# peterhpark/neuroclear

Hardware: AMD Instinct MI355X
Metric: voxels/sec (higher is better)
Workload: dtype f32

## Files before the change

include/nc_hip.h:

```cpp
#ifndef NC_HIP_H
#define NC_HIP_H

#include <stddef.h>
#include <stdint.h>

#ifdef __cplusplus
extern "C" {
#endif

#define NC_OK 0
#define NC_ERR_SHAPE (-1)
#define NC_ERR_WS (-2)
#define NC_ERR_HIP (-3)
#define NC_ERR_ARG (-4)

const char* nc_last_error(void);
int nc_version(void);
int nc_conv_fwd_path(int C, int K, int kd, int kh, int kw, int stride, int pad);
int nc_conv_wgrad_path(int C, int K, int kd, int kh, int kw, int stride, int pad);
void nc_prof_begin(double min_flop);
int nc_prof_end(int max, int* cls, double* flop, float* ms);
int nc_prof_end2(int max, int* cls, double* flop, float* ms, double* abytes);
void nc_set_force_direct(int on);
void nc_sconv_set_cfg(int cfg);
// ... 72 lines not shown

int nc_slice_fwd(const float* vol, float* out, int NC, int D, int H, int W, int axis, int index, void* stream);
int nc_slice_bwd(const float* dout, float* dvol, int NC, int D, int H, int W, int axis, int index, void* stream);
int nc_mip_fwd(const float* vol, float* out, int32_t* arg, int NC, int D, int H, int W, int axis, int start, int depth,
               void* stream);
int nc_mip_bwd(const float* dout, const int32_t* arg, float* dvol, int NC, int D, int H, int W, int axis,
               void* stream);

int nc_volume_slices(const float* src, float* dst, int N, int C, int D, int H, int W, int axis, int to_volume,
                     void* stream);

size_t nc_loss_ws_bytes(long n);
int nc_mse_const_fwd(const float* pred, long n, float target, float* out, void* ws, size_t ws_bytes, void* stream);
int nc_mse_const_bwd(const float* pred, long n, float target, const float* gscale, float* dpred, void* stream);
int nc_bce_logits_const_fwd(const float* pred, long n, float target, float* out, void* ws, size_t ws_bytes, void* stream);
int nc_bce_logits_const_bwd(const float* pred, long n, float target, const float* gscale, float* dpred, void* stream);
int nc_mean_fwd(const float* pred, long n, float* out, void* ws, size_t ws_bytes, void* stream);
int nc_mean_bwd(long n, const float* gscale, float* dpred, void* stream);
int nc_l1_fwd(const float* a, const float* b, long n, float* out, void* ws, size_t ws_bytes, void* stream);
int nc_l1_bwd(const float* a, const float* b, long n, const float* gscale, float* da, void* stream);

int nc_adam_step(float* p, const float* g, float* m, float* v, long n, float lr, float beta1, float beta2, float eps,
                 int step, void* stream);

int nc_dice_cut_cube(const void* vol, int is_u16, int L0, int L1, int L2, int roi, int overlap, int border, int index,
                     float* cube, void* stream);
int nc_rotate_crop(const void* vol, int is_u16, int D, int H, int W, int z0, int y0, int x0, int cz, int cy, int cx,
                   const double* inv_affine, float* out, void* stream);
int nc_assemble_scatter_add(const float* cube, float* acc, int P0, int P1, int P2, int roi, int overlap, int border,
                            int index, void* stream);
int nc_assemble_finalize(const float* acc, void* out, int out_is_u16, int P0, int P1, int P2, int L0, int L1, int L2,
                         int roi, int overlap, void* stream);
int nc_assemble_finalize_slab(const float* acc_slab, void* out, int out_is_u16, int P0, int P1, int P2, int L0, int L1, int L2, int roi,
                              int overlap, int z0, int nz, int za, void* stream);

int nc_assemble_merge(const float* acc, float* merged, int L0, int L1, int L2, int roi, int overlap, void* stream);
int nc_radix_hist(const float* x, long n, int pass, unsigned prefix, unsigned* hist4096, void* stream);
int nc_assemble_rescale_finalize(const float* merged, void* out, int out_is_u16, int L0, int L1, int L2, int roi,
                                 int overlap, float lo, float hi, float range, void* stream);

size_t nc_match_histograms_ws_bytes(long n);
int nc_match_histograms(const float* source, const float* tmpl, float* out, long n, void* ws, size_t ws_bytes,
                        void* stream);

int nc_spectral_norm_fwd(const float* w_orig, float* u, float* v, float* w_out, float* sigma, float* scratch_k, int K, int M,
                         int power_iteration, float eps, void* stream);
int nc_spectral_norm_bwd(const float* g, const float* w_sn, const float* u, const float* v, const float* sigma, float* dw_orig, int K,
                         int M, void* stream);

size_t nc_patchgan_param_floats(int n_layers, int ndf, int nd);
size_t nc_patchgan_saved_floats(int B, int D, int H, int W, int n_layers, int ndf, int nd);
size_t nc_patchgan_ws_bytes(int B, int D, int H, int W, int n_layers, int ndf, int nd);
int nc_patchgan_out_shape(int B, int D, int H, int W, int n_layers, int ndf, int nd, int* oD, int* oH, int* oW);
int nc_patchgan_fwd(const float* params, const float* x, float* y, float* saved, int B, int D, int H, int W,
                    int n_layers, int ndf, int nd, void* ws, size_t ws_bytes, void* stream);
int nc_patchgan_bwd(const float* params, const float* x, const float* saved, const float* dy, float* dx, float* dparams,
                    int B, int D, int H, int W, int n_layers, int ndf, int nd, void* ws, size_t ws_bytes, void* stream);
int nc_patchgan_fwd_part(const float* params, const float* x, float* y, float* saved, int Btot, int b0, int B, int D, int H,
                         int W, int n_layers, int ndf, int nd, void* ws, size_t ws_bytes, void* stream);
int nc_patchgan_bwd_part(const float* params, const float* x, const float* saved, const float* dy, float* dx, int Btot, int b0,
                         int B, int D, int H, int W, int n_layers, int ndf, int nd, void* ws, size_t ws_bytes, void* stream);
size_t nc_patchgan_gp_saved_floats(int B, int D, int H, int W, int n_layers, int ndf, int nd);
size_t nc_patchgan_gp_ws_bytes(int B, int D, int H, int W, int n_layers, int ndf, int nd);
int nc_patchgan_gp_fwd(const float* params, const float* x, float* g, float* pen, float* saved, int B, int D, int H, int W, int n_layers,
                       int ndf, int nd, float constant, float lambda_gp, void* ws, size_t ws_bytes, void* stream);
int nc_patchgan_gp_bwd(const float* params, const float* x, const float* saved, const float* g, const float* dpen, float* dparams, float* dx,
                       int B, int D, int H, int W, int n_layers, int ndf, int nd, float constant, float lambda_gp, void* ws, size_t ws_bytes,
                       void* stream);

size_t nc_unet_deconv_fwd_ws_bytes(int N, int S0, int S1, int S2);
int nc_unet_deconv_fwd(const float* params, const float* x, float* y, int N, int S0, int S1, int S2, void* ws,
                       size_t ws_bytes, void* stream);


size_t nc_unet_deconv_param_floats(void);
size_t nc_unet_deconv_saved_floats(int N, int S0, int S1, int S2);
size_t nc_unet_deconv_train_ws_bytes(int N, int S0, int S1, int S2);
int nc_unet_deconv_train_fwd(const float* params, const float* x, float* y, float* saved, int N, int S0, int S1, int S2,
                             void* ws, size_t ws_bytes, void* stream, unsigned* kept);
int nc_unet_deconv_bwd(const float* params, const float* x, const float* y, const float* saved, const float* dy, float* dx,
                       float* dparams, int N, int S0, int S1, int S2, void* ws, size_t ws_bytes, void* stream, unsigned kept);
void nc_set_unet_lean(int on);
int nc_get_unet_lean(void);
size_t nc_deep_linear_param_floats(void);
size_t nc_deep_linear_saved_floats(int N, int S0, int S1, int S2);
size_t nc_deep_linear_ws_bytes(int N, int S0, int S1, int S2);
int nc_deep_linear_fwd(const float* params, const float* x, float* y, float* saved , int N, int S0, int S1,
                       int S2, void* ws, size_t ws_bytes, void* stream, unsigned* kept );
void nc_set_dl_collapse(int on);
int nc_get_dl_collapse(void);
int nc_deep_linear_bwd(const float* params, const float* x, const float* saved, const float* dy, float* dx, float* dparams,
                       int N, int S0, int S1, int S2, void* ws, size_t ws_bytes, void* stream, unsigned kept);

int nc_conv_fwd_c8(const void* xh, const float* w, const float* bias, void* yh, int out_ctot, int out_c0, int N, int C, int D, int H,
                   int W, int K, int kd, int kh, int kw, int stride, int pad, int dtype, void* ws, size_t ws_bytes, void* stream);
int nc_conv_dgrad_c8(const void* dyh, const float* w, void* dxh, int N, int C, int D, int H, int W, int K, int kd, int kh, int kw,
                     int stride, int pad, int dtype, void* ws, size_t ws_bytes, void* stream);
size_t nc_conv_c1_c8_ws_bytes(int N, int D, int H, int W, int ks);
int nc_conv_c1_fwd_c8(const float* x, const float* w, const float* bias, void* yh, int out_ctot, int out_c0, int N, int D, int H, int W,
                      int ks, int dtype, void* ws, size_t ws_bytes, void* stream);
int nc_conv_c1_dgrad_c8(const void* dyh, const float* w, float* dx, int N, int D, int H, int W, int ks, void* ws, size_t ws_bytes,
                        void* stream);
size_t nc_conv_c1_wgrad_c8_ws_bytes(int N, int D, int H, int W, int ks);
int nc_conv_c1_wgrad_c8(const float* x, const void* dyh, float* dw, int N, int D, int H, int W, int ks, void* ws, size_t ws_bytes,
                        void* stream);
size_t nc_c8_instnorm_ws_bytes(int N, int C, long S);
int nc_c8_instnorm_stats(const void* xh, int N, int C, long S, float eps, float* mean, float* rstd, int dtype, void* ws,
                         size_t ws_bytes, void* stream);
int nc_c8_instnorm_act_fwd(const void* xh, const float* mean, const float* rstd, float slope, void* yh, int out_ctot, int out_c0,
                           int N, int C, long S, int dtype, void* stream);
int nc_c8_instnorm_act_bwd(const void* gh, int g_ctot, int g_c0, const void* xh, const float* mean, const float* rstd, float slope,
                           void* dxh, float* dbias , int N, int C, long S, int dtype, void* ws, size_t ws_bytes,
                           void* stream);
int nc_c8_maxpool2_fwd(const void* xh, int x_ctot, int x_c0, void* yh, int N, int C, int D, int H, int W, int dtype, void* stream);
int nc_c8_maxpool2_bwd_add(const void* dph, const void* xh, int x_ctot, int x_c0, const void* skiph, int s_ctot, int s_c0, void* dxh,
                           int N, int C, int D, int H, int W, int dtype, void* stream);
int nc_from_c8(const void* xh, int x_ctot, int x_c0, float* y, int N, int C, long S, int dtype, void* stream);
size_t nc_convT_c8_ws_bytes(int N, int C, int D, int H, int W, int K);
int nc_convT_k2s2_fwd_c8(const void* xh, const float* w, const float* bias, void* yh, int out_ctot, int out_c0, int N, int C, int D,
                         int H, int W, int K, int dtype, void* ws, size_t ws_bytes, void* stream);
int nc_convT_k2s2_dgrad_c8(const void* dyh, int dy_ctot, int dy_c0, const float* w, void* dxh, int N, int C, int D, int H, int W, int K,
                           void* ws, size_t ws_bytes, void* stream);
int nc_convT_k2s2_wgrad_c8(const void* xh, const void* dyh, int dy_ctot, int dy_c0, float* dw, float* dbias , int N,
                           int C, int D, int H, int W, int K, void* ws, size_t ws_bytes, void* stream);

int nc_unet_deconv_lp_supported(int N, int S0, int S1, int S2, int dtype);
size_t nc_unet_deconv_lp_saved_bytes(int N, int S0, int S1, int S2);
size_t nc_unet_deconv_lp_ws_bytes(int N, int S0, int S1, int S2);
int nc_unet_deconv_lp_fwd(const float* params, const float* x, float* y, void* saved, int N, int S0, int S1, int S2, int dtype,
                          void* ws, size_t ws_bytes, void* stream);
int nc_unet_deconv_lp_bwd(const float* params, const float* x, const float* y, const void* saved, const float* dy, float* dx,
                          float* dparams, int N, int S0, int S1, int S2, int dtype, void* ws, size_t ws_bytes, void* stream);
int nc_deep_linear_lp_supported(int N, int S0, int S1, int S2, int dtype);
size_t nc_deep_linear_lp_saved_bytes(int N, int S0, int S1, int S2);
size_t nc_deep_linear_lp_ws_bytes(int N, int S0, int S1, int S2);
int nc_deep_linear_lp_fwd(const float* params, const float* x, float* y, void* saved, int N, int S0, int S1, int S2, int dtype,
                          void* ws, size_t ws_bytes, void* stream, unsigned* kept);
int nc_deep_linear_lp_bwd(const float* params, const float* x, const void* saved, const float* dy, float* dx, float* dparams,
                          int N, int S0, int S1, int S2, int dtype, void* ws, size_t ws_bytes, void* stream, unsigned kept);

void nc_set_conv_split(int on);
int nc_get_conv_split(void);
void nc_set_split_terms(int terms);
int nc_get_split_terms(void);
void nc_set_p2d_terms(int mode);
int nc_get_p2d_terms(void);
void nc_set_h2_guard(int on);
int nc_get_h2_guard(void);
int nc_h2_guard_stats(unsigned long long* out4, int reset);
void nc_set_epi_stats(int on);
int nc_get_epi_stats(void);
void nc_set_s3x_w64(int on);
int nc_get_s3x_w64(void);
int nc_unet_deconv_fwd_terms(int S0, int S1, int S2);
void nc_set_c8x_mode(int mode);
int nc_get_c8x_mode(void);
int nc_conv_lp_uses_c8x(int what , int fp32_out, int N, int C, int D, int H, int W, int K, int ks);
void nc_set_s3_fusion(int on);
int nc_conv_split_supported(int what, int N, int C, int D, int H, int W, int K, int kd, int kh, int kw, int stride, int pad);
size_t nc_conv_split_ws_bytes(int N, int C, int D, int H, int W, int K, int ks);
size_t nc_s3_bytes(int N, int C, long S);
int nc_to_s3(const float* x, void* xs, int N, int C, long S, void* stream);
int nc_conv_fwd_split(const float* x, const void* xs, const float* w, const float* bias, float* y, int N, int C, int D, int H, int W,
                      int K, int ks , void* ws, size_t ws_bytes, void* stream);
int nc_conv_dgrad_split(const float* dy, const void* dys, const float* w, float* dx, int N, int C, int D, int H, int W, int K, int ks,
                        void* ws, size_t ws_bytes, void* stream);
// ... 30 lines not shown
```

neuroclear_amd/_lib.py:

```python
import ctypes
import os
import re

_HERE = os.path.dirname(os.path.abspath(__file__))
LIB_PATH = os.environ.get('NC_HIP_LIB') or os.path.join(_HERE, 'csrc', 'libnc_hip.so')
HEADER_PATH = os.path.join(os.path.dirname(_HERE), 'include', 'nc_hip.h')

_lib = None


class NcError(RuntimeError):
    pass


def header_symbols():
    src = open(HEADER_PATH).read()
    src = re.sub(r'/\*.*?\*/', '', src, flags=re.S)
    return sorted(set(re.findall(r'\b(nc_[a-zA-Z0-9_]+)\s*\(', src)))


def lib():
    global _lib
    if _lib is None:
        if not os.path.exists(LIB_PATH):
            raise NcError('libnc_hip.so is not built (%s): run `python -c "import __graft_entry__ as g; g.build()"` '
                          'or `make -C neuroclear_amd/csrc`; there is no CPU fallback' % LIB_PATH)
        L = ctypes.CDLL(LIB_PATH)
        for name in header_symbols():
            fn = getattr(L, name)
            if name.endswith('_bytes') or name.endswith('_floats'):
                fn.restype = ctypes.c_size_t
            elif name == 'nc_last_error':
                fn.restype = ctypes.c_char_p
            elif name in ('nc_set_force_direct', 'nc_prof_begin', 'nc_sconv_set_cfg', 'nc_sconv_set_tune', 'nc_set_conv_split', 'nc_set_s3_fusion', 'nc_set_c8x_mode', 'nc_set_split_terms', 'nc_set_h2_guard', 'nc_set_epi_stats', 'nc_set_dl_collapse', 'nc_set_p2d_terms', 'nc_set_s3x_w64', 'nc_set_unet_lean'):
                fn.restype = None
            else:
                fn.restype = ctypes.c_int
        _lib = L
    return _lib


def check(code, what=''):
    if code != 0:
        raise NcError('%s failed (%d): %s' % (what, code, lib().nc_last_error().decode()))


P = ctypes.c_void_p
I = ctypes.c_int
L_ = ctypes.c_long
F = ctypes.c_float
Z = ctypes.c_size_t
```

neuroclear_amd/csrc/api.hip:

```cpp
#include <cstdlib>
#include <cstring>
#include <vector>

#include <atomic>
#include <mutex>
#include <set>
#include <utility>

#include "common.hpp"

namespace nc {

static thread_local char g_err[512] = "";
int g_force_direct = 0;

void set_error(const char* fmt, ...) {
  va_list ap;
  va_start(ap, fmt);
  vsnprintf(g_err, sizeof(g_err), fmt, ap);
  va_end(ap);
}

int raise_dyn_lds(const void* kernel, int bytes, const char* who) {
  static std::mutex mu;
// ... 303 lines not shown
int nc_conv_dgrad_lp(const float* dy, const void* dyh, const float* w, float* dx, int N, int C, int D, int H, int W, int K,
                     int kd, int kh, int kw, int stride, int pad, int dtype, void* ws, size_t ws_bytes, void* stream) {
  ConvDims d;
  if (int e = lp_args("conv_dgrad_lp", d, dy, dyh, w, dx, N, C, D, H, W, K, kd, kh, kw, stride, pad, dtype)) return e;
  if (!h_dgrad_supported(d)) { set_error("conv_dgrad_lp: shape not covered by the 16-bit kernels"); return NC_ERR_SHAPE; }
  ProfScope ps(1, 1, d, 1, (hipStream_t)stream);
  return conv_dgrad_h(dy, dyh, w, dx, d, dtype, ws, ws_bytes, (hipStream_t)stream);
}

int nc_conv_wgrad_lp(const float* x, const void* xh, const float* dy, const void* dyh, float* dw, float* dbias, int N, int C,
                     int D, int H, int W, int K, int kd, int kh, int kw, int stride, int pad, int dtype, void* ws,
                     size_t ws_bytes, void* stream) {
  ConvDims d;
  if (int e = lp_args("conv_wgrad_lp", d, x, xh, dw, dw, N, C, D, H, W, K, kd, kh, kw, stride, pad, dtype)) return e;
  if (!dy && !dyh) { set_error("conv_wgrad_lp: null pointer"); return NC_ERR_ARG; }
  if (dbias && !dy) { set_error("conv_wgrad_lp: the bias gradient needs the fp32 dy"); return NC_ERR_ARG; }
  if (!h_wgrad_supported(d)) { set_error("conv_wgrad_lp: shape not covered by the 16-bit kernels"); return NC_ERR_SHAPE; }
  hipStream_t s = (hipStream_t)stream;
  {
    ProfScope ps(2, 1, d, 1, s);
    if (int e = conv_wgrad_h(x, xh, dy, dyh, dw, d, dtype, ws, ws_bytes, s)) return e;
  }
  if (dbias) return bias_grad(dy, dbias, d.N, d.K, (long)d.Do * d.Ho * d.Wo, ws, ws_bytes, s);
  return NC_OK;
}

int nc_conv_wgrad(const float* x, const float* dy, float* dw, float* dbias, int N, int C, int D, int H, int W, int K,
                  int kd, int kh, int kw, int stride, int pad, void* ws, size_t ws_bytes, void* stream) {
  ConvDims d;
  if (int e = conv_args("conv_wgrad", d, x, dy, dw, N, C, D, H, W, K, kd, kh, kw, stride, pad)) return e;
  hipStream_t s = (hipStream_t)stream;
  int e;
  {
  const int path = wgrad_path(d);
  ProfScope ps(2, path, d, 0, s);
  if (path == 9) e = conv_wgrad_s3(x, nullptr, dy, nullptr, dw, d, ws, ws_bytes, s);
  else if (path == 10) e = conv_wgrad_p2d(x, dy, dw, d, ws, ws_bytes, s);
  else if (!g_force_direct && mfma_wgrad_supported(d)) e = conv_wgrad_mfma(x, dy, dw, d, ws, ws_bytes, s);
  else if (!g_force_direct && wgrad_1x1_supported(d)) e = conv_wgrad_1x1(x, dy, dw, d, ws, ws_bytes, s);
  else if (!g_force_direct && c1_wgrad_supported(d)) e = conv_wgrad_c1(x, dy, dw, d, ws, ws_bytes, s);
  else if (!g_force_direct && k1_wgrad_supported(d)) e = conv_wgrad_k1(x, dy, dw, d, s);
  else if (!g_force_direct && wgrad_path(d) == 8) {
    e = conv_wgrad_pg1(x, dy, nullptr, 1.f, dw, dbias, d, ws, ws_bytes, s);
    dbias = nullptr;
  }
  else if (!g_force_direct && sconv_wgrad_on(d)) e = conv_wgrad_sconv(x, dy, dw, d, ws, ws_bytes, s);
  else if (!g_force_direct && gemm_wgrad_supported(d)) e = conv_wgrad_gemm(x, dy, dw, d, ws, ws_bytes, s);
  else e = conv_wgrad_direct(x, dy, dw, d, s);
  }
  if (e) return e;
  if (dbias) return bias_grad(dy, dbias, d.N, d.K, (long)d.Do * d.Ho * d.Wo, ws, ws_bytes, s);
  return NC_OK;
}

int nc_conv_bwd(const float* x, const float* dy, const float* w, float* dx, float* dw, float* dbias, int N, int C, int D, int H, int W,
                int K, int kd, int kh, int kw, int stride, int pad, void* ws, size_t ws_bytes, void* stream) {
  ConvDims d;
  if (int e = conv_args("conv_bwd", d, x, dy, dw, N, C, D, H, W, K, kd, kh, kw, stride, pad)) return e;
  if (!w) { set_error("conv_bwd: null pointer"); return NC_ERR_ARG; }
  hipStream_t s = (hipStream_t)stream;
  SwitchScope switches_;
  if (dx && dgrad_path(d) == 9 && wgrad_path(d) == 9 && ws && s3_bwd_ws_bytes(d) && ws_bytes >= s3_bwd_ws_bytes(d)) {
    {
      ProfScope ps(1, 9, d, 0, s);
      if (int e = conv_bwd_s3(x, dy, w, dx, dw, d, ws, ws_bytes, s, 0)) return e;
      if (int e = conv_bwd_s3(x, dy, w, dx, dw, d, ws, ws_bytes, s, 1)) return e;
    }
    {
      ProfScope ps(2, 9, d, 0, s);
      if (int e = conv_bwd_s3(x, dy, w, dx, dw, d, ws, ws_bytes, s, 2)) return e;
    }
    if (dbias) return bias_grad(dy, dbias, d.N, d.K, (long)d.Do * d.Ho * d.Wo, ws, ws_bytes, s);
    return NC_OK;
  }
  if (dx)
    if (int e = nc_conv_dgrad(dy, w, dx, N, C, D, H, W, K, kd, kh, kw, stride, pad, ws, ws_bytes, stream)) return e;
  return nc_conv_wgrad(x, dy, dw, dbias, N, C, D, H, W, K, kd, kh, kw, stride, pad, ws, ws_bytes, stream);
}

}

namespace nc {
int conv_fwd_keep(const float* x, const float* w, const float* bias, float* y, int N, int C, int D, int H, int W, int K, int ks,
                  void* ws, size_t ws_bytes, void* stream, void* xs_keep, bool* kept) {
  ConvDims d;
  *kept = false;
  if (xs_keep && make_dims(d, N, C, D, H, W, K, ks, ks, ks, 1, ks / 2) && fwd_path(d) == 9 && wgrad_path(d) == 9) {
    if (!x || !w || !y) { set_error("conv_fwd: null pointer"); return NC_ERR_ARG; }
    ProfScope ps(0, 9, d, 0, (hipStream_t)stream);
    *kept = true;
    return conv_fwd_s3(x, nullptr, w, bias, y, d, ws, ws_bytes, (hipStream_t)stream, xs_keep);
  }
  return nc_conv_fwd(x, w, bias, y, N, C, D, H, W, K, ks, ks, ks, 1, ks / 2, ws, ws_bytes, stream);
}

bool conv_keep_supported(int N, int C, int D, int H, int W, int K, int ks) {
  ConvDims d;
  return make_dims(d, N, C, D, H, W, K, ks, ks, ks, 1, ks / 2) && fwd_path(d) == 9 && wgrad_path(d) == 9;
}

int conv_fwd_pre(const void* xs, const float* w, const float* bias, float* y, int N, int C, int D, int H, int W, int K, int ks, void* ws,
                 size_t ws_bytes, void* stream, float* stats_part) {
  ConvDims d;
  if (!xs || !w || !y) { set_error("conv_fwd_pre: null pointer"); return NC_ERR_ARG; }
  if (!make_dims(d, N, C, D, H, W, K, ks, ks, ks, 1, ks / 2) || fwd_path(d) != 9) { set_error("conv_fwd_pre: layer not on the split-operand kernels"); return NC_ERR_SHAPE; }
  ProfScope ps(0, 9, d, 0, (hipStream_t)stream);
  if (stats_part && !(conv_layer_h2(d) && ks == 3)) { set_error("conv_fwd_pre: epilogue statistics exist for the two-term 3^3 layers only"); return NC_ERR_ARG; }
  return conv_fwd_s3(nullptr, xs, w, bias, y, d, ws, ws_bytes, (hipStream_t)stream, nullptr, stats_part);
}

bool conv_bwd_pre_supported(int N, int C, int D, int H, int W, int K, int ks, bool want_dx, size_t ws_bytes) {
  ConvDims d;
  return make_dims(d, N, C, D, H, W, K, ks, ks, ks, 1, ks / 2) && wgrad_path(d) == 9 && s3_bwd_ws_bytes(d) && ws_bytes >= s3_bwd_ws_bytes(d) &&
         (!want_dx || dgrad_path(d) == 9);
}
int conv_bwd_pre(const float* x, const void* xs, const float* w, float* dx, float* dw, int N, int C, int D, int H, int W, int K, int ks,
                 void* ws, size_t ws_bytes, void* stream, bool dy_guarded) {
  ConvDims d;
  hipStream_t s = (hipStream_t)stream;
  if (!conv_bwd_pre_supported(N, C, D, H, W, K, ks, dx != nullptr, ws_bytes) || !make_dims(d, N, C, D, H, W, K, ks, ks, ks, 1, ks / 2)) {
    set_error("conv_bwd_pre: layer not on the split-operand kernels");
    return NC_ERR_SHAPE;
  }
  if ((!x && !xs) || !w || !dw || !ws) { set_error("conv_bwd_pre: null pointer"); return NC_ERR_ARG; }
  if (dx) {
    ProfScope ps(1, 9, d, 0, s);
    if (int e = conv_bwd_s3(x, nullptr, w, dx, dw, d, ws, ws_bytes, s, 1, nullptr, dy_guarded)) return e;
  }
  ProfScope ps(2, 9, d, 0, s);
  return conv_bwd_s3(x, nullptr, w, dx, dw, d, ws, ws_bytes, s, 2, xs, dy_guarded);
}

int conv_bwd_keep(const float* x, const void* xs, const float* dy, const float* w, float* dx, float* dw, int N, int C, int D, int H,
                  int W, int K, int ks, void* ws, size_t ws_bytes, void* stream) {
  ConvDims d;
  hipStream_t s = (hipStream_t)stream;
  if (xs && make_dims(d, N, C, D, H, W, K, ks, ks, ks, 1, ks / 2) && wgrad_path(d) == 9 && ws && s3_bwd_ws_bytes(d) &&
      ws_bytes >= s3_bwd_ws_bytes(d) &&
      (!dx || dgrad_path(d) == 9)) {
    if (!x || !dy || !w || !dw) { set_error("conv_bwd: null pointer"); return NC_ERR_ARG; }
    {
      ProfScope ps(1, 9, d, 0, s);
      if (int e = conv_bwd_s3(x, dy, w, dx, dw, d, ws, ws_bytes, s, 0)) return e;
      if (dx)
        if (int e = conv_bwd_s3(x, dy, w, dx, dw, d, ws, ws_bytes, s, 1)) return e;
    }
    ProfScope ps(2, 9, d, 0, s);
    return conv_bwd_s3(x, dy, w, dx, dw, d, ws, ws_bytes, s, 2, xs);
  }
  return nc_conv_bwd(x, dy, w, dx, dw, nullptr, N, C, D, H, W, K, ks, ks, ks, 1, ks / 2, ws, ws_bytes, stream);
}
}

extern "C" {

namespace {
struct UnetOff {
  size_t w[14], b[14];
  size_t total;
};
UnetOff unet_offsets() {
  struct L { int id; size_t wn, bn; };
  const L order[14] = {{0, 64 * 1 * 27, 64},       {1, 64 * 64 * 27, 64},     {2, 128 * 64 * 27, 128},
                       {3, 128 * 128 * 27, 128},   {4, 256 * 128 * 27, 256},  {5, 256 * 256 * 27, 256},
                       {6, 256 * 256 * 27, 256},   {10, 256 * 128 * 8, 128},  {7, 128 * 256 * 27, 128},
                       {8, 128 * 128 * 27, 128},   {11, 128 * 64 * 8, 64},    {9, 64 * 128 * 27, 64},
                       {12, 64, 1},                {13, 1, 1}};
  UnetOff o{};
  size_t off = 0;
  for (const L& l : order) {
    o.w[l.id] = off; off += l.wn;
    o.b[l.id] = off; off += l.bn;
  }
  o.total = off;
  return o;
}
struct UnetWs {
  size_t raw, cat1, a1, p1, cat2, a2, a2b, p2, b1, b2, t1, t2, mean, rstd, in_ws, conv_ws, total;
  size_t s_a1, s_cat1, s_a2, s_cat2, s_b1, s_b2;
  size_t cells;
  size_t stats;
  size_t in_ws_bytes, conv_ws_bytes;
};
UnetWs unet_ws(int S0, int S1, int S2, int NB = 1) {
  const size_t S1v = (size_t)S0 * S1 * S2;
  const size_t S = S1v * NB, Sh = S / 8, Sq = S / 64;
  UnetWs u{};
  size_t off = 0;
  auto take = [&](size_t n) { size_t r = off; off += (n + 63) & ~(size_t)63; return r; };
  u.raw = take(64 * S); u.cat1 = take(128 * S); u.a1 = take(64 * S); u.p1 = take(64 * Sh); u.cat2 = take(256 * Sh);
  u.a2 = take(128 * Sh); u.a2b = take(128 * Sh); u.p2 = take(128 * Sq); u.b1 = take(256 * Sq); u.b2 = take(256 * Sq);
  u.t1 = take(S); u.t2 = take(S); u.mean = take(256 * (size_t)NB); u.rstd = take(256 * (size_t)NB);
  u.in_ws_bytes = nc_instnorm_ws_bytes(256, (long)S1v);
  u.in_ws = take(u.in_ws_bytes / 4);
  size_t cw = 0;
  auto upd = [&](int C, int D, int H, int W, int K) {
    size_t b = nc_conv_ws_bytes(1, C, D, H, W, K, 3, 3, 3, 1, 1);
    if (b > cw) cw = b;
  };
  upd(64, S0, S1, S2, 64); upd(128, S0, S1, S2, 64);
  upd(64, S0 / 2, S1 / 2, S2 / 2, 128); upd(128, S0 / 2, S1 / 2, S2 / 2, 128); upd(256, S0 / 2, S1 / 2, S2 / 2, 128);
  upd(128, S0 / 4, S1 / 4, S2 / 4, 256); upd(256, S0 / 4, S1 / 4, S2 / 4, 256);
  u.conv_ws_bytes = cw;
  u.conv_ws = take(cw / 4 + 64);
  auto take3 = [&](size_t elems) { return take((elems * 6 + 3) / 4); };
  u.s_a1 = take3(64 * S); u.s_cat1 = take3(128 * S); u.s_a2 = take3(128 * Sh); u.s_cat2 = take3(256 * Sh);
  u.s_b1 = take3(256 * Sq); u.s_b2 = take3(256 * Sq);
  u.cells = take(64);
  {
    size_t sb = 0;
// ... 260 lines not shown
```

neuroclear_amd/csrc/common.hpp:

```cpp
#pragma once
#include <hip/hip_runtime.h>

#include <cstdarg>
#include <cstdio>

#include "../../include/nc_hip.h"

namespace nc {

void set_error(const char* fmt, ...);

inline int check_launch(const char* what) {
  hipError_t e = hipGetLastError();
  if (e != hipSuccess) {
    set_error("%s: %s", what, hipGetErrorString(e));
    return NC_ERR_HIP;
  }
  return NC_OK;
}

inline long cdiv(long a, long b) { return (a + b - 1) / b; }

int raise_dyn_lds(const void* kernel, int bytes, const char* who);
template <typename K>
// ... 71 lines not shown
bool gemm_fwd_supported(const ConvDims& d);
bool gemm_dgrad_supported(const ConvDims& d);
bool gemm_wgrad_supported(const ConvDims& d);
size_t gemm_ws_bytes(const ConvDims& d);
int conv_fwd_gemm(const float* x, const float* w, const float* b, float* y, const ConvDims& d, void* ws, size_t wsb,
                  hipStream_t s);
int conv_dgrad_gemm(const float* dy, const float* w, float* dx, const ConvDims& d, void* ws, size_t wsb,
                    hipStream_t s);
int conv_wgrad_gemm(const float* x, const float* dy, float* dw, const ConvDims& d, void* ws, size_t wsb,
                    hipStream_t s);

bool sconv_fwd_supported(const ConvDims& d);
bool sconv_dgrad_supported(const ConvDims& d);
size_t sconv_ws_bytes(const ConvDims& d);
void p2d_set_terms(int m);
int p2d_get_terms();
bool p2d_fwd_supported(const ConvDims& d);
bool p2d_dgrad_supported(const ConvDims& d);
size_t p2d_ws_bytes(const ConvDims& d);
int conv_fwd_p2d(const float* x, const float* w, const float* bias, float* y, const ConvDims& d, void* ws, size_t wsb, hipStream_t s);
int conv_dgrad_p2d(const float* dy, const float* w, float* dx, const ConvDims& d, void* ws, size_t wsb, hipStream_t s);
bool p2d_wgrad_supported(const ConvDims& d);
size_t p2d_wgrad_ws_bytes(const ConvDims& d);
int conv_wgrad_p2d(const float* x, const float* dy, float* dw, const ConvDims& d, void* ws, size_t wsb, hipStream_t s);
int conv_fwd_sconv(const float* x, const float* w, const float* bias, float* y, const ConvDims& d, void* ws, size_t wsb, hipStream_t s);
int conv_dgrad_sconv(const float* dy, const float* w, float* dx, const ConvDims& d, void* ws, size_t wsb, hipStream_t s);
void sconv_set_cfg(int cfg);
void sconv_set_tune(int on);
bool sconv_wgrad_supported(const ConvDims& d);
size_t sconv_wgrad_ws_bytes(const ConvDims& d);
int conv_wgrad_sconv(const float* x, const float* dy, float* dw, const ConvDims& d, void* ws, size_t wsb, hipStream_t s);

bool pg1_supported(const ConvDims& d);
size_t pg1_ws_bytes(const ConvDims& d);
int conv_fwd_pg1(const float* x, const float* w, const float* bias, float* y, const ConvDims& d, float slope, hipStream_t s);
int conv_wgrad_pg1(const float* x, const float* g, const float* act, float slope, float* dw, float* db, const ConvDims& d,
                   void* ws, size_t wsb, hipStream_t s);
int conv_dgrad_pg1(const float* g, const float* act, float slope, const float* w, float* dx, const ConvDims& d, hipStream_t s);

bool wgrad_1x1_supported(const ConvDims& d);
size_t wgrad_1x1_ws_bytes(const ConvDims& d);
int conv_wgrad_1x1(const float* x, const float* dy, float* dw, const ConvDims& d, void* ws, size_t wsb, hipStream_t s);
bool flat_1x1_supported(const ConvDims& d);
int conv_fwd_1x1(const float* x, const float* w, const float* b, float* y, const ConvDims& d, void* ws, size_t wsb,
                 hipStream_t s);
int conv_dgrad_1x1(const float* dy, const float* w, float* dx, const ConvDims& d, void* ws, size_t wsb,
                   hipStream_t s);

size_t conv_fwd_to1_k3_ws_bytes(int N, int D, int H, int W);
int conv_fwd_to1_k3(const float* x, const float* w, float* y, int N, int C, int D, int H, int W, void* ws, size_t wsb, hipStream_t s);
bool to1_dgrad_supported(const ConvDims& d);
int conv_dgrad_to1(const float* dy, const float* w, float* dx, const ConvDims& d, hipStream_t s);
bool to1_mfma_supported(const ConvDims& d);
size_t to1_mfma_ws_bytes(const ConvDims& d);
int conv_dgrad_to1_mfma(const float* dy, const float* w, float* dx, const ConvDims& d, void* ws, size_t wsb,
                        hipStream_t s);
bool k1_fwd_supported(const ConvDims& d);
bool k1_wgrad_supported(const ConvDims& d);
int conv_fwd_k1(const float* x, const float* w, const float* b, float* y, const ConvDims& d, hipStream_t s);
int conv_wgrad_k1(const float* x, const float* dy, float* dw, const ConvDims& d, hipStream_t s);
bool c1_wgrad_supported(const ConvDims& d);
size_t c1_wgrad_ws_bytes(const ConvDims& d);
int conv_wgrad_c1(const float* x, const float* dy, float* dw, const ConvDims& d, void* ws, size_t wsb, hipStream_t s);

bool s3_fwd_supported(const ConvDims& d);
bool s3_dgrad_supported(const ConvDims& d);
size_t s3_ws_bytes(const ConvDims& d);
size_t s3_tensor_bytes(int N, int C, long S);
int split3_to(const float* x, void* xs, int N, int C, long S, hipStream_t s);
int split3_into(const float* x, long xstride, void* xs, int N, int C, long S, int ctot, int c0, hipStream_t s, const unsigned* guard = nullptr);
bool conv_layer_h2(const ConvDims& d);
struct ForceThreeTerm { ForceThreeTerm(); ~ForceThreeTerm(); };
struct NetworkScope { NetworkScope(); ~NetworkScope(); };
struct SwitchScope { SwitchScope(); ~SwitchScope(); };
struct ForceTwoTerm { ForceTwoTerm(); ~ForceTwoTerm(); int prev_terms, prev_depth; };
int frozen_terms();
int frozen_guard();
bool h2_guard_can_flip();
int operand_into(const ConvDims& d, const float* x, long xstride, void* xs, int N, int C, long S, int ctot, int c0, hipStream_t s);
int act_operand(const ConvDims& d, const float* x, const float* mean, const float* rstd, float slope, float* y, long ystride, void* ys, int N, int C,
                long S, int ctot, int c0, hipStream_t s);
int act_split3(const float* x, const float* mean, const float* rstd, float slope, float* y, long ystride, void* ys, int N, int C, long S,
               int ctot, int c0, hipStream_t s);
int conv_fwd_s3(const float* x, const void* xs, const float* w, const float* b, float* y, const ConvDims& d, void* ws, size_t wsb,
                hipStream_t s, void* xs_keep = nullptr, float* stats_part = nullptr);
bool epi_stats_on();
void epi_stats_set(int on);
int epi_stats_mode();
void s3x_w64_set(int on);
int s3x_w64_get();
int conv_dgrad_s3(const float* dy, const void* dys, const float* w, float* dx, const ConvDims& d, void* ws, size_t wsb, hipStream_t s);
size_t s3_bwd_ws_bytes(const ConvDims& d);
int conv_bwd_s3(const float* x, const float* dy, const float* w, float* dx, float* dw, const ConvDims& d, void* ws, size_t wsb,
                hipStream_t s, int phase, const void* xs = nullptr, bool dy_guarded = false);
int conv_fwd_keep(const float* x, const float* w, const float* bias, float* y, int N, int C, int D, int H, int W, int K, int ks,
                  void* ws, size_t ws_bytes, void* stream, void* xs_keep, bool* kept);
int conv_bwd_keep(const float* x, const void* xs, const float* dy, const float* w, float* dx, float* dw, int N, int C, int D, int H,
                  int W, int K, int ks, void* ws, size_t ws_bytes, void* stream);
bool s3x_supported(int N, int Cin, int D, int H, int W, int Kout, int KS);
size_t s3x_packed_bytes(int Cin, int Kout, int KS, int NT = 3);
void s3x_set_terms(int t);
int s3x_get_terms();
int conv_s3x_h2(const void* xs, const unsigned* cell_a, const unsigned* cell_b, int split_c, const float* w, const float* bias, float* y, int N,
                int Cin, int D, int H, int W, int Kout, int KS, long so, long si, int flip, unsigned* wcell, void* wp_ws, hipStream_t s,
                const unsigned* guard = nullptr, float* stats_part = nullptr);
size_t s3x_stats_bytes(int N, int D, int H, int W, int Kout, int KS);
int s3x_stats_finalize(const float* stats_part, const float* bias, int N, int D, int H, int W, int Kout, int KS, float eps, float* mean, float* rstd,
                       hipStream_t s);
bool c1k7_h2_supported(const ConvDims& d);
size_t c1k7_h2_ws_bytes(const ConvDims& d);
int conv_c1k7_h2(const float* x, const float* w, const float* bias, float* y, const ConvDims& d, void* ws, size_t wsb, hipStream_t s);
size_t c1k7_h2_dgrad_ws_bytes(const ConvDims& d);
bool dl_typed_supported(int N, int D, int H, int W);
size_t dl_typed_bytes(int N, int D, int H, int W);
const float* dl_typed_wp(const char* scratch, int N, int D, int H, int W);
float* dl_typed_dwsw(char* scratch, int N, int D, int H, int W);
int dl_typed_compose(const float* F, char* scratch, int N, int D, int H, int W, hipStream_t s);
int dl_typed_fwd_boundary(const float* act0, float* y, char* scratch, int N, int D, int H, int W, hipStream_t s);
int dl_typed_dgrad_boundary(const float* act0, const float* dy, float* g, char* scratch, int N, int D, int H, int W, hipStream_t s);
int dl_typed_p(const float* act0, const float* dy, float* Pq, char* scratch, int N, int D, int H, int W, hipStream_t s);
int conv_c1k7_h2_dgrad(const float* dy, const float* w, float* dx, const ConvDims& d, void* ws, size_t wsb, hipStream_t s);
inline size_t h2_cells_offset(size_t elems) { return (elems * 4 + 255) & ~(size_t)255; }
inline unsigned* h2_cells_of(const void* t, size_t elems) { return (unsigned*)((char*)const_cast<void*>(t) + h2_cells_offset(elems)); }
int instnorm_relu_tail_sigmoid(const float* x, const float* mean, const float* rstd, const float* w1, const float* b1, const float* w2,
                               const float* b2, float* y, int C, long S, hipStream_t s);
int instnorm_act_bwd_dbias_h2(const float* dy, const float* x, const float* mean, const float* rstd, float slope, void* dxs,
                              float* dbias, int N, int C, long S, void* ws, size_t ws_bytes, void* stream, unsigned* guard = nullptr);
int instnorm_act_bwd_dbias_h2_rank1(const float* dy1, const float* w1, const float* x, const float* mean, const float* rstd, float slope, void* dxs,
                                    float* dbias, int C, long S, void* ws, size_t ws_bytes, void* stream, unsigned* guard);
unsigned* conv_bwd_guard_words(void* ws, int N, int K, long S);
int maxpool2_h2(const void* in, void* out, int N, int C, int ctot, int D, int H, int W, hipStream_t s);
int h2_zero_cells(unsigned* cells, int n, hipStream_t s);
int h2_set_cell(unsigned* cell, float bound, hipStream_t s);
int h2_absmax(const float* x, long n, unsigned* cell, hipStream_t s, unsigned* cell2 = nullptr);
int split2h_into(const float* x, long xstride, void* xs, int N, int C, long S, int ctot, int c0, const unsigned* cell, hipStream_t s,
                 unsigned* guard = nullptr);
constexpr int kGuardLow = 0, kGuardAll = 1, kGuardFlag = 2;
constexpr unsigned kGuardDrop = 17u << 23;
constexpr unsigned long long kGuardShare = 64;
#if defined(__HIP_DEVICE_COMPILE__)
__device__ __forceinline__ bool guard_skip(const unsigned* guard, int want) {
  return guard && (int)(__builtin_nontemporal_load(guard + kGuardFlag) != 0) != want;
}
#else
__device__ bool guard_skip(const unsigned* guard, int want);
#endif
bool h2_guard_on();
int h2_guard_mode();
void h2_guard_set(int on);
int h2_guard_read(unsigned long long* out4, int reset);
int h2_guard_zero(unsigned* g, hipStream_t s, int nwords = 8);
int h2_guard_decide(unsigned* ga, unsigned* gb, unsigned* prior, unsigned* flag, bool can_flip, hipStream_t s, unsigned long long total_a = 0);
int h2_to_s3_if(const void* xh, void* xs, int N, int C, long S, const unsigned* cells, const unsigned* guard, hipStream_t s);
int act_split2h(const float* x, const float* mean, const float* rstd, float slope, float* y, long ystride, void* ys, int N, int C, long S, int ctot,
                int c0, float bound, unsigned* cell, unsigned* cell2, hipStream_t s);
int act_split2h_pool(const float* x, const float* mean, const float* rstd, float slope, void* ys, void* pooled, int N, int C, int D, int H, int W,
                     int ctot, int c0, float bound, unsigned* cell, hipStream_t s);
int conv_s3x(const void* xs, const float* w, const float* bias, float* y, int N, int Cin, int D, int H, int W, int Kout, int KS, long so,
             long si, int flip, void* wp_ws, hipStream_t s, const unsigned* guard = nullptr);
bool conv_keep_supported(int N, int C, int D, int H, int W, int K, int ks);
int conv_fwd_pre(const void* xs, const float* w, const float* bias, float* y, int N, int C, int D, int H, int W, int K, int ks, void* ws,
                 size_t ws_bytes, void* stream, float* stats_part = nullptr);
bool conv_bwd_pre_supported(int N, int C, int D, int H, int W, int K, int ks, bool want_dx, size_t ws_bytes);
int conv_bwd_pre(const float* x, const void* xs, const float* w, float* dx, float* dw, int N, int C, int D, int H, int W, int K, int ks,
                 void* ws, size_t ws_bytes, void* stream, bool dy_guarded = false);
bool instnorm_bwd_s3_supported(int N, int C, long S);
int instnorm_act_bwd_dbias_s3(const float* dy, const float* x, const float* mean, const float* rstd, float slope, void* dxs,
                              float* dbias, int N, int C, long S, void* ws, size_t ws_bytes, void* stream);
bool convT_fwd_s3_supported(int N, int C, int D, int H, int W, int K);
size_t c8x_packed_bytes(int Cin, int Kout, int KS);
void c8x_set_mode(int m);
int c8x_get_mode();
bool c8x_supported(int N, int Cin, int D, int H, int W, int Kout, int KS, bool fp32_out);
int conv_c8x(const void* xh, const float* w, const float* bias, float* y, void* yh, int ctot, int c0, int N, int Cin, int D, int H, int W,
             int Kout, int KS, long so, long si, int flip, int diffuse, int dt, void* wp_ws, hipStream_t s);
bool convT_s3x_supported(int N, int C, int D, int H, int W, int K);
size_t convT_s3x_ws_bytes(int C, int K);
int convT_fwd_s3x(const void* xs, const float* w, const float* bias, float* y, void* ys, int ctot, int c0, int N, int C, int D, int H, int W,
                  int K, void* ws, size_t wsb, hipStream_t s, const unsigned* h2cell = nullptr, const unsigned* xcell = nullptr);
int convT_h2_bound(const float* w, const float* bias, int C, int K, float in_bound, unsigned* cell, hipStream_t s);
int convT_fwd_split_h2(const float* x, const float* w, const float* bias, float* y, void* ys, int ys_ctot, int ys_c0, int N, int C, int D, int H,
                       int W, int K, const unsigned* out_cell, void* ws, size_t ws_bytes, hipStream_t s);
int convT_fwd_s3(const float* x, const float* w, const float* bias, float* y, void* ys, int ctot, int c0, int N, int C, int D, int H,
                 int W, int K, void* stream);
bool s3_wgrad_supported(const ConvDims& d);
bool c8x_wgrad_supported(const ConvDims& d);
size_t c8x_wgrad_part_bytes(const ConvDims& d);
int conv_wgrad_c8x(const void* xh, const void* dyh, float* dw, const ConvDims& d, int dtype, void* ws, size_t wsb, hipStream_t s);
size_t s3_wgrad_ws_bytes(const ConvDims& d);
int conv_wgrad_s3(const float* x, const void* xs, const float* dy, const void* dys, float* dw, const ConvDims& d, void* ws, size_t wsb,
                  hipStream_t s);
bool s3x_k32_supported(int N, int D, int H, int W);
bool conv_fwd_h2_k32_supported(const ConvDims& d);
int conv_fwd_h2_k32_keep(const float* x, const float* w, float* y, const ConvDims& d, void* ws, size_t wsb, hipStream_t s, void* xs_keep);
bool conv_fwd_h2_c32_supported(const ConvDims& d);
size_t conv_fwd_h2_c32_ws_bytes(const ConvDims& d);
int conv_fwd_h2_c32(const float* x, const float* w, float* y, const ConvDims& d, void* ws, size_t wsb, hipStream_t s);
bool wgrad_h2_supported(const ConvDims& d);
int conv_wgrad_h2(const float* x, const void* xs, const float* dy, const void* dys, float* dw, const ConvDims& d, void* ws, size_t wsb, hipStream_t s);
bool h_fwd_supported(const ConvDims& d);
bool h_dgrad_supported(const ConvDims& d);
bool h_wgrad_supported(const ConvDims& d);
size_t h_ws_bytes(const ConvDims& d);
int to_c8(const float* x, void* xh, int N, int C, long S, int dt, hipStream_t s);
int conv_fwd_h(const float* x, const void* xh, const float* w, const float* b, float* y, const ConvDims& d, int dt,
               void* ws, size_t wsb, hipStream_t s);
int conv_dgrad_h(const float* dy, const void* dyh, const float* w, float* dx, const ConvDims& d, int dt, void* ws,
                 size_t wsb, hipStream_t s);
int conv_wgrad_h(const float* x, const void* xh, const float* dy, const void* dyh, float* dw, const ConvDims& d, int dt,
                 void* ws, size_t wsb, hipStream_t s);
int conv_fwd_h_c8(const void* xh, const float* w, const float* b, void* yh, int ctot, int c0, const ConvDims& d, int dt,
                  void* ws, size_t wsb, hipStream_t s);
int conv_fwd_h_na1(const void* xh, const float* w, float* y, const ConvDims& d, int dt, void* ws, size_t wsb, hipStream_t s);
int conv_dgrad_h_c8(const void* dyh, const float* w, void* dxh, int ctot, int c0, const ConvDims& d, int dt, void* ws,
                    size_t wsb, hipStream_t s);
bool dl_collapse_on();
size_t dl_tail_bytes();
const float* dl_tail_E(const char* tail);
const float* dl_tail_Ef(const char* tail);
float* dl_tail_q(char* tail);
int dl_tail_compose(const float* w2, const float* w3, const float* w4, const float* w5, char* tail, hipStream_t s);
int dl_tail_grads(const float* w2, const float* w3, const float* w4, const float* w5, char* tail, float* dw2, float* dw3, float* dw4, float* dw5,
                  hipStream_t s);
float* dl_tail_P(char* tail);
const float* dl_w1_fold(char* tail, const float* w1, hipStream_t s);
int dl_w1_contract(const char* tail, float* dw1, hipStream_t s);
int dl_q_from_p(char* tail, const float* w1, hipStream_t s);
const float* dl_fold_fwd64(char* tail, const float* w1, hipStream_t s);
int dl_combine27(const float* Z, float* y, int N, int D, int H, int W, int zch, hipStream_t s);
bool c1_h_supported(int D, int H, int W, int KS);
size_t c1_h_ws_bytes(int N, int D, int H, int W, int KS);
int conv_c1_fwd_h(const float* x, const float* w, const float* bias, void* yh, int ctot, int c0, int N, int D, int H, int W, int KS,
                  int dt, void* ws, size_t wsb, hipStream_t s);
int conv_c1_dgrad_h(const void* dyh, const float* w, float* dx, int N, int D, int H, int W, int KS, void* ws, size_t wsb,
                    hipStream_t s);

void h_set_weight_diffusion(int on);

bool c1_wgrad_h_supported(int N, int D, int H, int W, int KS);
size_t c1_wgrad_h_ws_bytes(int N, int D, int H, int W, int KS);
int conv_c1_wgrad_h(const float* x, const void* dyh, float* dw, int N, int D, int H, int W, int KS, void* ws, size_t wsb,
                    hipStream_t s);

static constexpr size_t kPackSlackBytes = 128 * 1024;

extern int g_force_direct;

struct ProfScope {
// ... 8 lines not shown
```

neuroclear_amd/csrc/conv_s3x.hip:

```cpp
#include <atomic>
#include <cstdlib>
#include <type_traits>

#include "common.hpp"
#include "s3_common.hpp"

namespace nc {
namespace {

typedef float f32x4 __attribute__((ext_vector_type(4)));
typedef __bf16 bf16x8 __attribute__((ext_vector_type(8)));
typedef _Float16 f16x8 __attribute__((ext_vector_type(8)));
typedef unsigned u32x4 __attribute__((ext_vector_type(4)));
typedef unsigned long long u64x2 __attribute__((ext_vector_type(2)));
typedef const __attribute__((address_space(1))) void* gptr_t;
typedef __attribute__((address_space(3))) void* lptr_t;
typedef const volatile __attribute__((address_space(3))) unsigned long long* lds64_t;

constexpr int kWaves = 8;
constexpr int kThreads = kWaves * 64;
constexpr int kLdsMax = 160 * 1024;
#ifndef NC_S3X_DMAW
#define NC_S3X_DMAW 4
#endif
#ifndef NC_S3X_BDEPTH
#define NC_S3X_BDEPTH 1
#endif
constexpr int kDmaWaves = NC_S3X_DMAW;
constexpr int kMaxPieces = 56;

__device__ __forceinline__ unsigned fdiv(unsigned n, unsigned m) { return __umulhi(n, m); }
unsigned magic(unsigned d) { return (unsigned)(((1ull << 32) + d - 1) / d); }

__device__ __forceinline__ void split3(float v, unsigned short (&t)[3]) { s3_split(v, t); }

template <int NT>
__global__ void __launch_bounds__(256) k_pack_w_s3x(const float* __restrict__ w, unsigned short* __restrict__ wp, int NCH, int KS, int NS,
                                                    long so, long si, int flip, long total, const unsigned* __restrict__ amax, int split_c,
                                                    const unsigned* __restrict__ cell_a, const unsigned* __restrict__ cell_b) {
  const long i = (long)blockIdx.x * 256 + threadIdx.x;
  if (i >= total) return;
  const int T2 = KS * KS, T3 = T2 * KS, NB = NCH * KS;
  const int j = (int)(i & 7);
  long q = i >> 3;
  const int lane = (int)(q & 63); q >>= 6;
  const int f = (int)(q % (2 * NT)); q /= 2 * NT;
  const int s = (int)(q % NS); q /= NS;
  const int half = (int)(q & 1);
  const int cot = (int)(q >> 1);
  const int rb = f / NT, term = f % NT;
  const int g = lane >> 4, m = lane & 15;
  const int T = 4 * s + g;
  const int bi = T / T2, tp = T % T2;
  unsigned short t[3] = {0, 0, 0};
  if (bi < NB) {
    const int chunk = bi / KS, dz = bi % KS;
#ifdef NC_S3X_B128
    const int jj = j;
#else
    const int jj = (g & 1) ? ((j + 4) & 7) : j;
#endif
    const long co = cot * 64 + half * 32 + rb * 16 + m, ci = chunk * 8 + jj;
    const int tap = dz * T2 + tp;
    const float v = w[co * so + ci * si + (flip ? T3 - 1 - tap : tap)];
    if constexpr (NT == 3) split3(v, t);
    else h2_split(v * (ci >= split_c ? h2_group_factor(*cell_a, *cell_b) : 1.f) * h2_scale(*amax), t);
  }
  wp[i] = t[term];
}

__global__ void __launch_bounds__(256) k_absmax_w(const float* __restrict__ w, long n, int T3, int C, int split_c, const unsigned* __restrict__ cell_a,
                                                  const unsigned* __restrict__ cell_b, unsigned* __restrict__ out) {
  unsigned m = 0;
  const float gf = split_c < C ? h2_group_factor(*cell_a, *cell_b) : 1.f;
  for (long i = (long)blockIdx.x * 256 + threadIdx.x; i < n; i += (long)gridDim.x * 256) {
    const int ci = (int)((i / T3) % C);
    const unsigned b = __float_as_uint(w[i] * (ci >= split_c ? gf : 1.f)) & 0x7fffffffu;
    if (b < 0x7f800000u && b > m) m = b;
  }
#pragma unroll
  for (int o = 32; o > 0; o >>= 1) {
    const unsigned q = (unsigned)__shfl_xor((int)m, o);
    m = q > m ? q : m;
  }
  __shared__ unsigned wm[4];
  if ((threadIdx.x & 63) == 0) wm[threadIdx.x >> 6] = m;
  __syncthreads();
  if (threadIdx.x == 0) {
    unsigned b = wm[0];
    for (int k = 1; k < 4; ++k) b = wm[k] > b ? wm[k] : b;
    if (b) atomicMax(out, b);
  }
}

__global__ void __launch_bounds__(256) k_pack_w_c1k7(const float* __restrict__ w, unsigned short* __restrict__ wp, int NS, long total,
                                                     const unsigned* __restrict__ amax) {
  const long i = (long)blockIdx.x * 256 + threadIdx.x;
  if (i >= total) return;
  const int j = (int)(i & 7);
  long q = i >> 3;
  const int lane = (int)(q & 63); q >>= 6;
  const int f = (int)(q & 3); q >>= 2;
  const int s = (int)(q % NS); q /= NS;
  const int half = (int)(q & 1);
  const int rb = f >> 1, term = f & 1;
  const int g = lane >> 4, m = lane & 15;
  const int T = 4 * s + g;
  unsigned short t[3] = {0, 0, 0};
  const int jj = (g & 1) ? ((j + 4) & 7) : j;
  const int dz = T >> 3, dy = T & 7;
  if (dz < 7 && dy < 7 && jj < 7) {
    const int co = half * 32 + rb * 16 + m;
    h2_split(w[(long)co * 343 + (dz * 7 + dy) * 7 + jj] * h2_scale(*amax), t);
  }
  wp[i] = t[term];
}

__global__ void __launch_bounds__(256) k_build_x8_h2(const float* __restrict__ x, uint4* __restrict__ out, long S, int W, const unsigned* __restrict__ cell,
                                                     unsigned* __restrict__ guard) {
  const unsigned cb_bits = *cell;
  const float sc = h2_scale(cb_bits);
  const int n = blockIdx.y;
  unsigned n_all = 0, n_low = 0;
  for (long v0 = (long)blockIdx.x * 256; v0 < S; v0 += (long)gridDim.x * 256) {
    const long v = v0 + threadIdx.x;
    unsigned m = 0;
    if (v < S) {
      const int xx = (int)(v % W);
      const float* row = x + (long)n * S + (v - xx);
      unsigned short e[8][3];
#pragma unroll
      for (int j = 0; j < 8; ++j) {
        const int xs = xx + j - 3;
        const float f = (j < 7 && (unsigned)xs < (unsigned)W) ? row[xs] : 0.f;
        if (j == 3) { const unsigned b = __float_as_uint(f) & 0x7fffffffu; if (b < 0x7f800000u) m = b; }
        h2_split(f * sc, e[j]);
      }
#pragma unroll
      for (int t = 0; t < 2; ++t) out[((long)n * 2 + t) * S + v] = s3_unit(e, t);
    }
    if (guard) {
      const unsigned thr = cb_bits > kGuardDrop ? cb_bits - kGuardDrop : 0u;
      const bool any_hi = __builtin_amdgcn_ballot_w64(m >= thr && m != 0) != 0;
      const bool any_nz = __builtin_amdgcn_ballot_w64(m != 0) != 0;
      if (any_nz) {
        ++n_all;
        if (!any_hi) ++n_low;
      }
    }
  }
  if (!guard) return;
  __shared__ unsigned cnt[2];
  if (threadIdx.x < 2) cnt[threadIdx.x] = 0;
  __syncthreads();
  if ((threadIdx.x & 63) == 0) {
    if (n_all) atomicAdd(&cnt[kGuardAll], n_all);
    if (n_low) atomicAdd(&cnt[kGuardLow], n_low);
  }
  __syncthreads();
  if (threadIdx.x < 2 && cnt[threadIdx.x]) atomicAdd(guard + threadIdx.x, cnt[threadIdx.x]);
}

__global__ void __launch_bounds__(256) k_pack_w_c1k7d(const float* __restrict__ w, unsigned short* __restrict__ wp, int NS, long total,
                                                      const unsigned* __restrict__ amax) {
  const long i = (long)blockIdx.x * 256 + threadIdx.x;
  if (i >= total) return;
  const int j = (int)(i & 7);
  long q = i >> 3;
  const int lane = (int)(q & 63); q >>= 6;
  const int f = (int)(q & 3); q >>= 2;
  const int s = (int)(q % NS); q /= NS;
  const int half = (int)(q & 1);
  const int rb = f >> 1, term = f & 1;
  const int g = lane >> 4, m = lane & 15;
  const int T = 4 * s + g;
// ... 918 lines not shown
__global__ void __launch_bounds__(256) k_s3x_stats_partial(const float2* __restrict__ part, XStatsPlan pl, double2* __restrict__ chunk_sums) {
  const int slice = blockIdx.x, n = blockIdx.y, ch = blockIdx.z;
  const int cot = slice >> 1, half = slice & 1;
  const int l = threadIdx.x & 31, grp = threadIdx.x >> 5;
  const long per_n = (long)pl.TPP * pl.D;
  double s = 0.0, q = 0.0;
  const long nrec = per_n * 4, per = (nrec + kStatChunks - 1) / kStatChunks;
  const long r1 = (ch + 1) * per < nrec ? (ch + 1) * per : nrec;
#pragma unroll 4
  for (long r = ch * per + grp; r < r1; r += 8) {
    const long u = r >> 2;
    const int pg = (int)(r & 3);
    const long t = ((long)n * per_n + u) * pl.KT + cot;
    if (t < pl.main_count) {
      const float2 v = part[((t * kWaves) + pg * 2 + half) * 32 + l];
      s += (double)v.x; q += (double)v.y;
    } else {
      const int full_g = (pl.TPP / kXGroup) * kXGroup * pl.D;
      int tp;
      if (u < full_g) { const long g4 = u / (kXGroup * pl.D), rem = u - g4 * (kXGroup * pl.D); tp = (int)(g4 * kXGroup + (rem % kXGroup)); }
      else { const int L = pl.TPP % kXGroup; const long v2 = u - full_g; tp = (pl.TPP / kXGroup) * kXGroup + (int)(v2 % L); }
      for (int sub = 0; sub < pl.fsub; ++sub) {
        if ((long)(tp * pl.fsub + sub) * pl.PTsub >= pl.HP) continue;
        const long ti = pl.main_count + (t - pl.full) * pl.fsub + sub;
        const float2 v = part[((ti * kWaves) + pg * 2 + half) * 32 + l];
        s += (double)v.x; q += (double)v.y;
      }
    }
  }
  __shared__ double rs[8][32], rq[8][32];
  rs[grp][l] = s; rq[grp][l] = q;
  __syncthreads();
  if (grp == 0) {
    for (int g = 1; g < 8; ++g) { s += rs[g][l]; q += rq[g][l]; }
    chunk_sums[(((long)n * gridDim.x + slice) * kStatChunks + ch) * 32 + l] = make_double2(s, q);
  }
}
__global__ void __launch_bounds__(256) k_s3x_stats_final(const double2* __restrict__ chunk_sums, int K, const float* __restrict__ bias, long S, float eps,
                                                         float* __restrict__ mean, float* __restrict__ rstd) {
  const int i = blockIdx.x * 256 + threadIdx.x, n = blockIdx.y;
  if (i >= K) return;
  const int slice = i >> 5, l = i & 31;
  double s = 0.0, q = 0.0;
  for (int ch = 0; ch < kStatChunks; ++ch) {
    const double2 v = chunk_sums[(((long)n * (K / 32) + slice) * kStatChunks + ch) * 32 + l];
    s += v.x; q += v.y;
  }
  const int g4 = l >> 3, m = l & 7;
  const int c = (slice >> 1) * 64 + (slice & 1) * 32 + 4 * g4 + 16 * (m >> 2) + (m & 3);
  const double m0 = s / (double)S;
  double var = q / (double)S - m0 * m0;
  if (var < 0.0) var = 0.0;
  mean[(long)n * K + c] = (float)(m0 + (bias ? (double)bias[c] : 0.0));
  rstd[(long)n * K + c] = (float)(1.0 / sqrt(var + (double)eps));
}

}

static std::atomic<int> g_epi_stats{getenv("NC_EPI_STATS") ? atoi(getenv("NC_EPI_STATS")) : 1};
bool epi_stats_on() { return g_epi_stats.load(std::memory_order_relaxed) != 0; }
int epi_stats_mode() { return g_epi_stats.load(std::memory_order_relaxed); }
void epi_stats_set(int on) { g_epi_stats.store(on < 0 ? 0 : on > 2 ? 2 : on, std::memory_order_relaxed); }

int s3x_ksteps(int Cin, int KS) { return (KS * KS * KS * (Cin / 8) / 4 + 1) & ~1; }
size_t s3x_packed_bytes(int Cin, int Kout, int KS, int NT) {
  const int NS = s3x_ksteps(Cin, KS);
  return (size_t)(Kout / 32) * NS * 2 * NT * 1024;
}

static std::atomic<int> g_terms{getenv("NC_SPLIT_TERMS") ? atoi(getenv("NC_SPLIT_TERMS")) : 2};
void s3x_set_terms(int t) { g_terms = (t == 0 || t == 3) ? t : 2; }
int s3x_get_terms() { const int f = frozen_terms(); return f >= 0 ? f : g_terms.load(); }

bool s3x_k32_supported(int N, int D, int H, int W) { return x_plan(N, D, H, W, 1, 5, 2, true).ok && (long)32 * D * H * W * 4 < (1l << 31); }
bool s3x_supported(int N, int Cin, int D, int H, int W, int Kout, int KS) {
  if (KS != 3 && KS != 5) return false;
  if (Cin % 64 || Kout % 64) return false;
  if ((long)Kout * D * H * W * 4 >= (1l << 31)) return false;
  if ((long)D * H * W * 48 >= (1l << 31)) return false;
  if ((long)H * (W + KS - 1) + 4096 >= (1l << 31)) return false;
  return x_plan(N, D, H, W, Kout / 64, KS).ok;
}

int conv_s3x_h2(const void* xs, const unsigned* cell_a, const unsigned* cell_b, int split_c, const float* w, const float* bias, float* y, int N,
                int Cin, int D, int H, int W, int Kout, int KS, long so, long si, int flip, unsigned* wcell, void* wp_ws, hipStream_t s,
                const unsigned* guard, float* stats_part) {
  const bool k32 = Kout == 32;
  if (k32 && (KS != 5 || stats_part || guard)) { set_error("conv_s3x_h2: 32 output channels for unguarded 5^3 launches only"); return NC_ERR_SHAPE; }
  const XPlan pl = x_plan(N, D, H, W, k32 ? 1 : Kout / 64, KS, 2, k32);
  if (!pl.ok) { set_error("conv_s3x_h2: shape not covered"); return NC_ERR_SHAPE; }
  if (split_c < Cin && (flip || !cell_b || split_c % 8)) { set_error("conv_s3x_h2: scale groups only for the forward weight layout"); return NC_ERR_ARG; }
  if (stats_part && KS != 3) { set_error("conv_s3x_h2: epilogue statistics exist for the 3^3 layers only (the layers in front of an InstanceNorm)"); return NC_ERR_ARG; }
  const int NCH = Cin / 8, NS = s3x_ksteps(Cin, KS), T3 = KS * KS * KS;
  if (Cin % 32) { set_error("conv_s3x_h2: channels must be a multiple of 32"); return NC_ERR_SHAPE; }
  if (int e = h2_zero_cells(wcell, 1, s)) return e;
  const long nw = (long)Kout * Cin * T3;
  if (!cell_b) cell_b = cell_a;
  hipLaunchKernelGGL(k_absmax_w, dim3((unsigned)(cdiv(nw, 256 * 8) < 256 ? cdiv(nw, 256 * 8) : 256)), dim3(256), 0, s, w, nw, T3, Cin,
                     flip ? Cin : split_c, cell_a, cell_b, wcell);
  const long total = (long)(s3x_packed_bytes(Cin, Kout, KS, 2) / 2);
  hipLaunchKernelGGL(k_pack_w_s3x<2>, dim3((unsigned)cdiv(total, 256)), dim3(256), 0, s, w, (unsigned short*)wp_ws, NCH, KS, NS, so, si, flip, total,
                     (const unsigned*)wcell, flip ? Cin : split_c, cell_a, cell_b);
  if (int e = check_launch("conv_s3x_h2 pack")) return e;
  XParams p{};
  p.xs = (const uint4*)xs; p.wp = (const uint4*)wp_ws; p.bias = bias; p.y = y; p.amax_x = cell_a; p.amax_w = wcell; p.guard = guard;
  p.N = N; p.NCH = NCH; p.D = D; p.H = H; p.W = W; p.K = Kout;
  p.P = pl.P; p.HP = pl.HP; p.TPP = pl.TPP; p.KT = k32 ? 1 : Kout / 64;
  p.NS = NS; p.mP = magic(pl.P);
  static const int flush = getenv("NC_S3X_FLUSH") ? atoi(getenv("NC_S3X_FLUSH")) : 4;
  p.flush = flush >= 4 ? flush : flush > 0 ? 4 : 1 << 30;
  if (KS == 3 && !k32 && s3x_w64_get()) p.flush = 1 << 30;
  const bool one = pl.rem && pl.fsub == 1;
  if (pl.full || one) {
    p.fsub = 1; p.UB = pl.UB; p.npb = pl.npb; p.mUB = magic(pl.UB);
    p.t_begin = 0; p.t_count = (int)(pl.full + (one ? pl.rem : 0)); p.tiles_per_xcd = (int)cdiv(p.t_count, 8);
    p.stats = (float2*)stats_part;
    const int e = !k32 && w64_applies(KS, pl.NCB, NS, pl.lds) ? (stats_part ? launch_w64<true>(p, pl.lds, s) : launch_w64<false>(p, pl.lds, s))
                  : k32 ? (pl.NCB == 4 ? launch_x<5, 4, 2, false, true>(p, pl.lds + kOffTab, s) : launch_x<5, 2, 2, false, true>(p, pl.lds + kOffTab, s))
                  : stats_part ? (KS == 3 ? launch_x_ncb<3, 2, true>(pl.NCB, p, pl.lds + kOffTab, s) : launch_x_ncb<5, 2>(pl.NCB, p, pl.lds + kOffTab, s))
                             : (KS == 3 ? launch_x_ncb<3, 2>(pl.NCB, p, pl.lds + kOffTab, s) : launch_x_ncb<5, 2>(pl.NCB, p, pl.lds + kOffTab, s));
    if (e) return e;
  }
  if (pl.rem && !one) {
    p.fsub = pl.fsub; p.UB = pl.UBt; p.npb = pl.npbt; p.mUB = magic(pl.UBt);
    p.t_begin = (int)pl.full; p.t_count = (int)(pl.rem * pl.fsub); p.tiles_per_xcd = (int)cdiv(p.t_count, 8);
    p.stats = stats_part ? (float2*)stats_part + pl.full * kWaves * 32 : nullptr;
    const int e = k32 ? (pl.NCB / pl.fsub == 4 ? launch_x<5, 4, 2, false, true>(p, pl.ldst + kOffTab, s) : launch_x<5, 2, 2, false, true>(p, pl.ldst + kOffTab, s))
                  : stats_part ? (KS == 3 ? launch_x_ncb<3, 2, true>(pl.NCB / pl.fsub, p, pl.ldst + kOffTab, s)
                                        : launch_x_ncb<5, 2>(pl.NCB / pl.fsub, p, pl.ldst + kOffTab, s))
                             : (KS == 3 ? launch_x_ncb<3, 2>(pl.NCB / pl.fsub, p, pl.ldst + kOffTab, s)
                                        : launch_x_ncb<5, 2>(pl.NCB / pl.fsub, p, pl.ldst + kOffTab, s));
    if (e) return e;
  }
  return NC_OK;
}

static size_t c1k7_al(size_t b) { return (b + 255) & ~(size_t)255; }
static constexpr int kC1k7Steps = 14;
static size_t c1k7_packed_bytes() { return (size_t)2 * kC1k7Steps * 4 * 1024; }
bool c1k7_h2_supported(const ConvDims& d) {
  static const int on = getenv("NC_C1K7_H2") ? atoi(getenv("NC_C1K7_H2")) : 1;
  if (!on || s3x_get_terms() != 2) return false;
  if (d.C != 1 || d.K != 64 || d.kd != 7 || d.kh != 7 || d.kw != 7 || d.sd != 1 || d.sh != 1 || d.sw != 1 || d.pd != 3 || d.ph != 3 || d.pw != 3) return false;
  const long S = (long)d.D * d.H * d.W;
  if (d.W < 4 || (long)64 * S * 4 >= (1l << 31) || S * 32 >= (1l << 31)) return false;
  return x_plan(d.N, d.D, d.H, d.W, 1, 7, 2, false, true).ok;
}
size_t c1k7_h2_ws_bytes(const ConvDims& d) {
  if (!c1k7_h2_supported(d)) return 0;
  return 512 + c1k7_al((size_t)d.N * d.D * d.H * d.W * 32) + c1k7_al(c1k7_packed_bytes());
}
template <int NCB>
static int launch_pc(const XParams& p, int lds, hipStream_t s) { return launch_x<7, NCB, 2, false, false, 1>(p, lds, s); }
static int launch_pc_ncb(int NCB, const XParams& p, int lds, hipStream_t s) {
  if (NCB == 8) return launch_pc<8>(p, lds, s);
  if (NCB == 7) return launch_pc<7>(p, lds, s);
  if (NCB == 6) return launch_pc<6>(p, lds, s);
  if (NCB == 4) return launch_pc<4>(p, lds, s);
  return launch_pc<2>(p, lds, s);
}
int conv_c1k7_h2(const float* x, const float* w, const float* bias, float* y, const ConvDims& d, void* ws, size_t wsb, hipStream_t s) {
  if (!c1k7_h2_supported(d)) { set_error("conv_c1k7_h2: shape not covered"); return NC_ERR_SHAPE; }
  if (!ws || wsb < c1k7_h2_ws_bytes(d)) { set_error("conv_c1k7_h2: workspace too small"); return NC_ERR_WS; }
  const XPlan pl = x_plan(d.N, d.D, d.H, d.W, 1, 7, 2, false, true);
  const long S = (long)d.D * d.H * d.W;
  unsigned* cells = (unsigned*)ws;
  unsigned* gw = (unsigned*)((char*)ws + 256);
  uint4* x8 = (uint4*)((char*)ws + 512);
  void* wp = (char*)x8 + c1k7_al((size_t)d.N * S * 32);
  if (int e = h2_zero_cells(cells, 2, s)) return e;
  if (int e = h2_absmax(x, (long)d.N * S, cells, s)) return e;
  if (int e = h2_absmax(w, (long)64 * 343, cells + 1, s)) return e;
  const bool guard = h2_guard_on();
  if (guard) if (int e = h2_guard_zero(gw, s, 4)) return e;
  {
    long bx = cdiv(S, 256);
    if (guard && bx * d.N > 4096) bx = cdiv(4096, d.N);
    hipLaunchKernelGGL(k_build_x8_h2, dim3((unsigned)bx, (unsigned)d.N), dim3(256), 0, s, x, x8, S, d.W, (const unsigned*)cells, guard ? gw : nullptr);
  }
  if (guard) if (int e = h2_guard_decide(gw, nullptr, nullptr, gw + kGuardFlag, false, s)) return e;
  const long total = (long)(c1k7_packed_bytes() / 2);
  hipLaunchKernelGGL(k_pack_w_c1k7, dim3((unsigned)cdiv(total, 256)), dim3(256), 0, s, w, (unsigned short*)wp, kC1k7Steps, total, (const unsigned*)(cells + 1));
  if (int e = check_launch("conv_c1k7_h2 prep")) return e;
  XParams p{};
  p.xs = x8; p.wp = (const uint4*)wp; p.bias = bias; p.y = y; p.amax_x = cells; p.amax_w = cells + 1; p.guard = nullptr;
  p.N = d.N; p.NCH = 1; p.D = d.D; p.H = d.H; p.W = d.W; p.K = 64;
// ... 138 lines not shown
```

neuroclear_amd/csrc/conv_split.hip:

```cpp
#include <cstdlib>
#include <type_traits>

#include "common.hpp"
#include "s3_common.hpp"

namespace nc {
NC_ZERO_PAGE()
namespace {

typedef float f32x16 __attribute__((ext_vector_type(16)));
typedef __bf16 bf16x8 __attribute__((ext_vector_type(8)));
typedef int i32x4 __attribute__((ext_vector_type(4)));
typedef const __attribute__((address_space(1))) void* gptr_t;
typedef __attribute__((address_space(3))) void* lptr_t;

constexpr int kWaves = 8;
constexpr int kThreads = kWaves * 64;
constexpr int kLdsMax = 160 * 1024;
#ifndef NC_S3_ABLATE
#define NC_S3_ABLATE 0
#endif
template <int KS> struct Sub;
template <> struct Sub<3> { static constexpr int NP = 5, NSUB = 1, MAXP = 5; static constexpr int q0[2] = {0, 5}; };
template <> struct Sub<5> { static constexpr int NP = 13, NSUB = 4, MAXP = 4; static constexpr int q0[5] = {0, 4, 7, 10, 13}; };
// ... 332 lines not shown
      for (int v = 0; v < VB; ++v) {
        const unsigned f = (unsigned)(cur.q0 + qb + v * 32);
        const unsigned yy = fdiv(f, p.mP);
        const unsigned xx = f - yy * p.P;
        yo[v] = ((int)yy < p.H && (int)xx < p.W) ? (long)yy * p.W + xx : -1;
      }
#pragma unroll
      for (int a = 0; a < 2; ++a) {
        float bv[16];
#pragma unroll
        for (int e = 0; e < 16; ++e) bv[e] = p.bias ? p.bias[cob + a * 32 + (e & 3) + 8 * (e >> 2) + 4 * h] : 0.f;
#pragma unroll
        for (int v = 0; v < VB; ++v)
          if (yo[v] >= 0) {
            float* yv = yn + yo[v];
#pragma unroll
            for (int e = 0; e < 16; ++e) yv[(long)(a * 32 + (e & 3) + 8 * (e >> 2)) * S] = acc[a][v][e] + bv[e];
          }
      }
    }
    if (!more_tiles) break;
    cur = nxt;
    tcur = tnext;
    lo = dz_lo(cur);
    nv = dz_hi(cur) - lo + 1;
  }
}

struct SPlan {
  int PT, VB, P, R, RP, TPP, npb, lds;
  bool ok;
};

SPlan s_plan(int H, int W, int KS) {
  SPlan pl{};
  pl.P = W + KS - 1;
  const long plane = (long)H * pl.P;
  const int wbytes = (KS == 3 ? Sub<3>::MAXP : Sub<5>::MAXP) * kPairPieces * 1024;
  double best = 0;
  for (int VB : {2, 1}) {
    const int PT = VB * 256;
    const int rows = (pl.P - 1 + PT - 1) / pl.P + 1;
    const int R = rows + KS - 1;
    const int RP = R * pl.P;
    const int npb = (3 * RP + 4 + 63) / 64;
    const int lds = 2 * npb * 1024 + 2 * wbytes;
    if (npb > 8 * 7 || lds > kLdsMax) continue;
    const int TPP = (int)((plane + PT - 1) / PT);
    const double eff = (double)H * W / ((double)TPP * PT) * (VB == 2 ? 1.0 : 0.85);
    if (eff > best) {
      best = eff;
      pl.PT = PT; pl.VB = VB; pl.R = R; pl.RP = RP; pl.npb = npb; pl.lds = lds; pl.TPP = TPP;
      pl.ok = true;
    }
  }
  return pl;
}

bool s_shape_ok(const ConvDims& d, int Cin, int Kout) {
  if (d.kd != d.kh || d.kd != d.kw || (d.kd != 3 && d.kd != 5)) return false;
  if (d.sd != 1 || d.sh != 1 || d.sw != 1 || d.pd != d.kd / 2 || d.ph != d.pd || d.pw != d.pd) return false;
  if (Cin % 8 || Kout % 64) return false;
  if ((long)d.D * d.H * d.W * 3 >= (1l << 31)) return false;
  return s_plan(d.H, d.W, d.kd).ok;
}

size_t s_packed_bytes(int Cin, int Kout, int KS) {
  return (size_t)(Kout / 64) * (Cin / 8) * KS * ((KS * KS + 1) / 2) * kPairPieces * 1024;
}
size_t align256(size_t b) { return (b + 255) & ~(size_t)255; }

template <int KS, int VB>
int launch_s3(const SParams& p, int lds, hipStream_t s) {
  auto kern = k_conv_s3<KS, VB>;
  if (int e = raise_dyn_lds(kern, kLdsMax, "conv_s3")) return e;
  hipLaunchKernelGGL(kern, dim3(256), dim3(kThreads), lds, s, p);
  return check_launch("conv_s3");
}

bool s3_layer_h2(const ConvDims& d);

int run_s3(const float* x, const void* xs_pre, const float* w, const float* bias, float* y, const ConvDims& d, int Cin, int Kout,
           long so, long si, int flip, void* ws, size_t wsb, hipStream_t s, void* xs_keep = nullptr, bool h2 = false, unsigned* guard_pre = nullptr,
           float* stats_part = nullptr) {
  const int KS = d.kd;
  const SPlan pl = s_plan(d.H, d.W, KS);
  const long S = (long)d.D * d.H * d.W;
  if (h2) {
    const size_t ex = (size_t)d.N * Cin * S;
    const bool internal = !xs_pre && !xs_keep;
    const size_t p2 = s3x_packed_bytes(Cin, Kout, KS, 2), p3 = s3x_packed_bytes(Cin, Kout, KS, 3);
    const size_t xb6 = align256(ex * 6), xb4 = h2_cells_offset(ex) + 256;
    bool dual = guard_pre || (internal && x && h2_guard_can_flip() && wsb >= xb6 + 256 + p3 + 256);
    if (guard_pre && wsb < 256 + p3 + 256) { set_error("conv_s3 (two-term, guarded operand): workspace too small"); return NC_ERR_WS; }
    const size_t xb = !internal ? 0 : dual ? xb6 : xb4;
    if (!ws || wsb < xb + 256 + p2 + 256) { set_error("conv_s3 (two-term): workspace too small"); return NC_ERR_WS; }
    void* xs = xs_pre ? const_cast<void*>(xs_pre) : xs_keep ? xs_keep : ws;
    unsigned* cells = h2_cells_of(xs, ex);
    unsigned* gw = (unsigned*)((char*)ws + xb);
    unsigned* guard = guard_pre ? guard_pre : gw;
    if (!xs_pre) {
      if (int e = h2_guard_zero(gw, s)) return e;
      if (int e = h2_zero_cells(cells, 2, s)) return e;
      if (int e = h2_absmax(x, (long)ex, cells, s, cells + 1)) return e;
      if (int e = split2h_into(x, (long)Cin * S, xs, d.N, Cin, S, Cin, 0, cells, s, gw)) return e;
      if (int e = h2_guard_decide(gw, nullptr, nullptr, gw + kGuardFlag, dual, s)) return e;
      if (dual)
        if (int e = split3_into(x, (long)Cin * S, xs, d.N, Cin, S, Cin, 0, s, gw)) return e;
    }
    if (stats_part && dual) { set_error("conv_s3 (two-term): epilogue statistics need an operand that cannot fall back"); return NC_ERR_ARG; }
    if (int e = conv_s3x_h2(xs, cells, cells + 1, flip ? Cin : Cin / 2, w, bias, y, d.N, Cin, d.D, d.H, d.W, Kout, KS, so, si, flip, gw + 16,
                            (char*)ws + xb + 256, s, dual ? guard : nullptr, stats_part)) return e;
    if (dual) return conv_s3x(xs, w, bias, y, d.N, Cin, d.D, d.H, d.W, Kout, KS, so, si, flip, (char*)ws + xb + 256, s, guard);
    return NC_OK;
  }
  const size_t xb = (xs_pre || xs_keep) ? 0 : align256((size_t)d.N * Cin * S * 6);
  const size_t wb = align256(s_packed_bytes(Cin, Kout, KS));
  if (!ws || wsb < xb + wb + 256) { set_error("conv_s3: workspace too small"); return NC_ERR_WS; }
  uint4* xs = xs_pre ? (uint4*)xs_pre : xs_keep ? (uint4*)xs_keep : (uint4*)ws;
  unsigned short* wp = (unsigned short*)((char*)ws + xb);
  const uint4* zeros = reinterpret_cast<const uint4*>(nc_zero_page());
  if (!zeros) { set_error("conv_s3: no zero page"); return NC_ERR_HIP; }
  if (!xs_pre) {
    hipLaunchKernelGGL(k_split3, dim3((unsigned)cdiv(S, 256), (unsigned)(d.N * Cin / 8)), dim3(256), 0, s, x, xs, S, Cin / 8, Cin / 8, 0,
                       (long)Cin * S, (const unsigned*)nullptr);
    if (int e = check_launch("split3")) return e;
  }
  static const int use_x = getenv("NC_S3X") ? atoi(getenv("NC_S3X")) : 1;
  if (use_x && s3x_supported(d.N, Cin, d.D, d.H, d.W, Kout, KS) && s3x_packed_bytes(Cin, Kout, KS) <= wb)
    return conv_s3x(xs, w, bias, y, d.N, Cin, d.D, d.H, d.W, Kout, KS, so, si, flip, wp, s);
  const long total = (long)(s_packed_bytes(Cin, Kout, KS) / 2);
  hipLaunchKernelGGL(k_pack_w_s3, dim3((unsigned)cdiv(total, 256)), dim3(256), 0, s, w, wp, Cin / 8, KS, so, si, flip, total);
  if (int e = check_launch("pack_w_s3")) return e;
  SParams p{};
  p.xs = xs; p.wp = (const uint4*)wp; p.bias = bias; p.y = y; p.zeros = zeros;
  p.N = d.N; p.NCH = Cin / 8; p.D = d.D; p.H = d.H; p.W = d.W; p.K = Kout;
  p.P = pl.P; p.R = pl.R; p.RP = pl.RP; p.PT = pl.PT; p.TPP = pl.TPP; p.KT = Kout / 64;
  p.mP = magic(pl.P); p.mRP = magic(pl.RP);
  p.npb = pl.npb;
  p.ntiles = (long)d.N * d.D * pl.TPP * p.KT;
  p.tiles_per_xcd = (int)cdiv(p.ntiles, 8);
  static const int flush = 1;
  p.flush = flush;
  if (KS == 3) return pl.VB == 2 ? launch_s3<3, 2>(p, pl.lds, s) : launch_s3<3, 1>(p, pl.lds, s);
  return pl.VB == 2 ? launch_s3<5, 2>(p, pl.lds, s) : launch_s3<5, 1>(p, pl.lds, s);
}

typedef short s16x4 __attribute__((ext_vector_type(4)));
typedef __attribute__((address_space(3))) s16x4* ltr_t;

struct WsParams {
  const uint4* xs;
  const uint4* dys;
  float* part;
  const uint4* zeros;
  int N, C, K, D, H, W;
  int Ty, Tx, YB, XB;
  int F, NF;
  int Xp, XU, XUp;
  int PT, PTp, NK;
  int npx, npd;
  int xslot, dybuf;
  int nct;
  int npairs, nwp;
  long steps;
  unsigned mTx, mXp, mXUp, mPTp;
  const unsigned* guard;
};

__device__ __forceinline__ i32x4 tr_frag(const unsigned char* lds, unsigned a0, unsigned a1) {
  const s16x4 lo = __builtin_amdgcn_ds_read_tr16_b64_v4i16((ltr_t)(lds + a0));
  const s16x4 hi = __builtin_amdgcn_ds_read_tr16_b64_v4i16((ltr_t)(lds + a1));
  return __builtin_bit_cast(i32x4, __builtin_shufflevector(lo, hi, 0, 1, 2, 3, 4, 5, 6, 7));
}

template <int KS>
__global__ void __launch_bounds__(kThreads, 1) k_wgrad_s3(const WsParams p) {
  extern __shared__ __attribute__((aligned(1024))) unsigned char lds_raw[];
  if (guard_skip(p.guard, 1)) return;
  constexpr int PAD = KS / 2, T2 = KS * KS;
  constexpr int ZR = KS == 3 ? 3 : 1, NS = ZR + 1, NDG = KS / ZR, TW = ZR * T2;
  constexpr int TG = (TW + 3) / 4;
  const int tid = threadIdx.x, lane = tid & 63;
  const int wave = __builtin_amdgcn_readfirstlane(tid >> 6);
  const int mt = wave & 1, tg = wave >> 1;
  const int t0 = tg * (TW / 4) + (tg < TW % 4 ? tg : TW % 4);
  const int ntap = TW / 4 + (tg < TW % 4 ? 1 : 0);
  const long HW = (long)p.H * p.W, S = (long)p.D * HW;

  const int G = gridDim.x, xcd = blockIdx.x & 7;
  const int wg = (G >> 3) * xcd + ((G & 7) < xcd ? (G & 7) : xcd) + (blockIdx.x >> 3);
  const int pair = wg % p.npairs, wi = wg / p.npairs;
  if (wi >= p.nwp) return;
  const int dzg = pair % NDG, kc = pair / NDG;
  const int kt = kc / p.nct, ct = kc % p.nct;
// ... 739 lines not shown
}

bool c8x_wgrad_supported(const ConvDims& d) {
  static const int on = getenv("NC_HX_WGRAD") ? atoi(getenv("NC_HX_WGRAD")) : 1;
  return on && wsx_shape_ok(d);
}
size_t c8x_wgrad_part_bytes(const ConvDims& d) {
  const int T3 = d.kd * d.kh * d.kw, TW = d.kd == 3 ? 27 : 25;
  const int npairs = (d.K / 64) * (d.C / 32) * (T3 / TW);
  return (size_t)npairs * ws_nwp(d, ws_plan(d, 1), npairs) * TW * 64 * 32 * 4;
}
int conv_wgrad_c8x(const void* xh, const void* dyh, float* dw, const ConvDims& d, int dtype, void* ws, size_t wsb, hipStream_t s) {
  return dtype == NC_DT_F16 ? run_wsx<NC_DT_F16>(xh, dyh, dw, d, ws, wsb, s) : run_wsx<NC_DT_BF16>(xh, dyh, dw, d, ws, wsb, s);
}

bool s3_fwd_supported(const ConvDims& d) { return s_shape_ok(d, d.C, d.K); }
bool s3_dgrad_supported(const ConvDims& d) { return s_shape_ok(d, d.K, d.C); }
size_t s3_ws_bytes(const ConvDims& d) {
  const long S = (long)d.D * d.H * d.W;
  const int cmax = d.C > d.K ? d.C : d.K;
  const int c64 = (d.C + 63) / 64 * 64, k64 = (d.K + 63) / 64 * 64;
  size_t pk = align256(s_packed_bytes(c64, k64, d.kd));
  const size_t p3 = align256(s3x_packed_bytes(c64, k64, d.kd, 3));
  if (p3 > pk) pk = p3;
  return align256((size_t)d.N * cmax * S * 6) + pk + 768;
}
size_t s3_tensor_bytes(int N, int C, long S) { return (size_t)N * C * S * 6; }
bool s3_wgrad_supported(const ConvDims& d) { return ws_shape_ok(d); }
size_t s3_wgrad_ws_bytes(const ConvDims& d) {
  if (!ws_shape_ok(d)) return 0;
  const long S = (long)d.D * d.H * d.W;
  size_t pb = ws_part_bytes(d, 3);
  if (ws_kv(d, 2) == 32 && ws_plan(d, 2).ok) { const size_t p2 = ws_part_bytes(d, 2); if (p2 > pb) pb = p2; }
  return align256((size_t)d.N * d.C * S * 6) + align256((size_t)d.N * d.K * S * 6) + pb + 768;
}
int conv_wgrad_s3(const float* x, const void* xs, const float* dy, const void* dys, float* dw, const ConvDims& d, void* ws, size_t wsb,
                  hipStream_t s) {
  return run_ws(x, xs, dy, dys, dw, d, ws, wsb, s);
}
bool conv_fwd_h2_c32_supported(const ConvDims& d) {
  if (s3x_get_terms() != 2 || d.C % 32 || d.K % 64 || d.kd != d.kh || d.kd != d.kw || (d.kd != 3 && d.kd != 5)) return false;
  if (d.sd != 1 || d.sh != 1 || d.sw != 1 || d.pd != d.kd / 2 || d.ph != d.pd || d.pw != d.pd) return false;
  return s3x_supported(d.N, 64, d.D, d.H, d.W, d.K, d.kd);
}
size_t conv_fwd_h2_c32_ws_bytes(const ConvDims& d) {
  const size_t ex = (size_t)d.N * d.C * d.D * d.H * d.W;
  return align256(ex * 6) + 256 + s3x_packed_bytes(d.C, d.K, d.kd, 3) + 512;
}
int conv_fwd_h2_c32(const float* x, const float* w, float* y, const ConvDims& d, void* ws, size_t wsb, hipStream_t s) {
  if (!conv_fwd_h2_c32_supported(d)) { set_error("conv_fwd_h2_c32: shape not covered"); return NC_ERR_SHAPE; }
  const int T3 = d.kd * d.kh * d.kw;
  return run_s3(x, nullptr, w, nullptr, y, d, d.C, d.K, (long)d.C * T3, T3, 0, ws, wsb, s, nullptr, true);
}
bool conv_fwd_h2_k32_supported(const ConvDims& d) {
  if (s3x_get_terms() != 2 || d.C % 64 || d.K != 32 || d.kd != 5 || d.kh != 5 || d.kw != 5 || d.sd != 1 || d.sh != 1 || d.sw != 1 || d.pd != 2 || d.ph != 2 || d.pw != 2)
    return false;
  return s3x_k32_supported(d.N, d.D, d.H, d.W);
}
int conv_fwd_h2_k32_keep(const float* x, const float* w, float* y, const ConvDims& d, void* ws, size_t wsb, hipStream_t s, void* xs_keep) {
  if (!conv_fwd_h2_k32_supported(d) || !xs_keep) { set_error("conv_fwd_h2_k32_keep: shape not covered"); return NC_ERR_SHAPE; }
  return run_s3(x, nullptr, w, nullptr, y, d, d.C, d.K, (long)d.C * 125, 125, 0, ws, wsb, s, xs_keep, true);
}
bool wgrad_h2_supported(const ConvDims& d) { return s3x_get_terms() == 2 && ws_shape_ok(d) && ws_kv(d, 2) == 32 && ws_plan(d, 2).ok && ws_part_bytes(d, 2) != 0; }
int conv_wgrad_h2(const float* x, const void* xs, const float* dy, const void* dys, float* dw, const ConvDims& d, void* ws, size_t wsb, hipStream_t s) {
  if (!wgrad_h2_supported(d)) { set_error("conv_wgrad_h2: shape not covered"); return NC_ERR_SHAPE; }
  return run_ws_h2(x, xs, dy, dys, dw, d, ws, wsb, s, nullptr);
}
size_t s3_bwd_ws_bytes(const ConvDims& d) {
  if (!ws_shape_ok(d)) return 0;
  const long S = (long)d.D * d.H * d.W;
  const size_t A = align256((size_t)d.N * d.K * S * 6) + 256;
  size_t dg = 0;
  if (s_shape_ok(d, d.K, d.C)) {
    dg = align256(s_packed_bytes(d.K, d.C, d.kd));
    const size_t p3 = align256(s3x_packed_bytes(d.K, d.C, d.kd, 3));
    if (p3 > dg) dg = p3;
    dg += 768;
  }
  const size_t wg = s3_wgrad_ws_bytes(d) - align256((size_t)d.N * d.K * S * 6);
  return A + (dg > wg ? dg : wg);
}
unsigned* conv_bwd_guard_words(void* ws, int N, int K, long S) { return (unsigned*)((char*)ws + align256((size_t)N * K * S * 6)); }
int conv_bwd_s3(const float* x, const float* dy, const float* w, float* dx, float* dw, const ConvDims& d, void* ws, size_t wsb,
                hipStream_t s, int phase, const void* xs, bool dy_guarded) {
  const long S = (long)d.D * d.H * d.W;
  const size_t A = align256((size_t)d.N * d.K * S * 6) + 256;
  if (!ws || wsb < s3_bwd_ws_bytes(d)) { set_error("conv_bwd_s3: workspace too small"); return NC_ERR_WS; }
  unsigned* yg = (unsigned*)((char*)ws + A - 256);
  const bool h2 = s3_layer_h2(d);
  const bool guarded = h2 && h2_guard_can_flip() && (dy || dy_guarded);
  if (phase == 0) {
    if (h2) {
      const size_t ey = (size_t)d.N * d.K * S;
      unsigned* yc = h2_cells_of(ws, ey);
      if (int e = h2_guard_zero(yg, s)) return e;
      if (int e = h2_zero_cells(yc, 2, s)) return e;
      if (int e = h2_absmax(dy, (long)ey, yc, s, yc + 1)) return e;
      if (int e = split2h_into(dy, (long)d.K * S, ws, d.N, d.K, S, d.K, 0, yc, s, yg)) return e;
      if (!guarded) return h2_guard_decide(yg, nullptr, nullptr, yg + kGuardFlag, false, s);
      if (int e = h2_guard_decide(yg, nullptr, nullptr, yg + kGuardFlag, true, s)) return e;
      return split3_into(dy, (long)d.K * S, ws, d.N, d.K, S, d.K, 0, s, yg);
    }
    return split3_to(dy, ws, d.N, d.K, S, s);
  }
  if (phase == 1) {
    ConvDims t = d;
    t.C = d.K; t.K = d.C;
    const int T3 = d.kd * d.kh * d.kw;
    return run_s3(dy, ws, w, nullptr, dx, t, d.K, d.C, T3, (long)d.C * T3, 1, (char*)ws + A, wsb - A, s, nullptr, h2, guarded ? yg : nullptr);
  }
  return run_ws(x, xs, dy, ws, dw, d, (char*)ws + A, wsb - A, s, guarded ? yg : nullptr);
}

int split3_to(const float* x, void* xs, int N, int C, long S, hipStream_t s) { return split3_into(x, (long)C * S, xs, N, C, S, C, 0, s); }

int split3_into(const float* x, long xstride, void* xs, int N, int C, long S, int ctot, int c0, hipStream_t s, const unsigned* guard) {
  if (C % 8 || ctot % 8 || c0 % 8) { set_error("split3: channels must be multiples of 8"); return NC_ERR_SHAPE; }
  long bx = cdiv(S, 256);
  const long ny = (long)N * C / 8;
  if (guard && bx * ny > 2048) bx = cdiv(2048, ny) < bx ? cdiv(2048, ny) : bx;
  hipLaunchKernelGGL(k_split3, dim3((unsigned)bx, (unsigned)ny), dim3(256), 0, s, x, (uint4*)xs, S, C / 8, ctot / 8, c0 / 8,
                     xstride, guard);
  return check_launch("split3");
}

int act_split3(const float* x, const float* mean, const float* rstd, float slope, float* y, long ystride, void* ys, int N, int C, long S,
               int ctot, int c0, hipStream_t s) {
  if (C % 8 || ctot % 8 || c0 % 8) { set_error("act_split3: channels must be multiples of 8"); return NC_ERR_SHAPE; }
  hipLaunchKernelGGL(k_act_split3, dim3((unsigned)cdiv(S, 256), (unsigned)(N * C / 8)), dim3(256), 0, s, x, mean, rstd, slope, y, ystride,
                     (uint4*)ys, S, C / 8, ctot / 8, c0 / 8);
  return check_launch("act_split3");
}

int operand_into(const ConvDims& d, const float* x, long xstride, void* xs, int N, int C, long S, int ctot, int c0, hipStream_t s) {
  if (!s3_layer_h2(d)) return split3_into(x, xstride, xs, N, C, S, ctot, c0, s);
  if (C != ctot && 2 * C != ctot) { set_error("operand_into: a part must be the whole tensor or a half"); return NC_ERR_SHAPE; }
  unsigned* cells = h2_cells_of(xs, (size_t)N * ctot * S);
  unsigned* mine = cells + (c0 ? 1 : 0);
  if (int e = h2_zero_cells(mine, C == ctot ? 2 : 1, s)) return e;
  for (int n = 0; n < N; ++n)
    if (int e = h2_absmax(x + (long)n * xstride, (long)C * S, mine, s, C == ctot ? cells + 1 : nullptr)) return e;
  unsigned* g = cells + (c0 ? 16 : 8);
  if (int e = h2_guard_zero(g, s)) return e;
  if (int e = split2h_into(x, xstride, xs, N, C, S, ctot, c0, mine, s, g)) return e;
  return h2_guard_decide(g, nullptr, nullptr, g + kGuardFlag, false, s);
}
int act_operand(const ConvDims& d, const float* x, const float* mean, const float* rstd, float slope, float* y, long ystride, void* ys, int N, int C,
                long S, int ctot, int c0, hipStream_t s) {
  if (!s3_layer_h2(d)) return act_split3(x, mean, rstd, slope, y, ystride, ys, N, C, S, ctot, c0, s);
  if (C != ctot && 2 * C != ctot) { set_error("act_operand: a part must be the whole tensor or a half"); return NC_ERR_SHAPE; }
  unsigned* cells = h2_cells_of(ys, (size_t)N * ctot * S);
  unsigned* mine = cells + (c0 ? 1 : 0);
  return act_split2h(x, mean, rstd, slope, y, ystride, ys, N, C, S, ctot, c0, sqrtf((float)S), mine, C == ctot ? cells + 1 : nullptr, s);
}
bool conv_layer_h2(const ConvDims& d) { return s3_layer_h2(d); }
static thread_local int tl_net_depth = 0;
static thread_local int tl_sw_depth = 0, tl_sw_terms = -1, tl_sw_guard = -1;
SwitchScope::SwitchScope() {
  if (tl_sw_depth++ == 0) { tl_sw_terms = s3x_get_terms(); tl_sw_guard = h2_guard_mode(); }
}
SwitchScope::~SwitchScope() {
  if (--tl_sw_depth == 0) { tl_sw_terms = -1; tl_sw_guard = -1; }
}
ForceTwoTerm::ForceTwoTerm() : prev_terms(tl_sw_terms), prev_depth(tl_sw_depth) { tl_sw_terms = 2; ++tl_sw_depth; }
ForceTwoTerm::~ForceTwoTerm() { tl_sw_terms = prev_terms; --tl_sw_depth; if (tl_sw_depth == 0) { tl_sw_terms = -1; tl_sw_guard = -1; } }
int frozen_terms() { return tl_sw_terms; }
int frozen_guard() { return tl_sw_guard; }
NetworkScope::NetworkScope() { ++tl_net_depth; if (tl_sw_depth++ == 0) { tl_sw_terms = s3x_get_terms(); tl_sw_guard = h2_guard_mode(); } }
NetworkScope::~NetworkScope() { --tl_net_depth; if (--tl_sw_depth == 0) { tl_sw_terms = -1; tl_sw_guard = -1; } }
bool h2_guard_can_flip() { return h2_guard_mode() == 2 || (h2_guard_mode() == 1 && tl_net_depth == 0); }
ForceThreeTerm::ForceThreeTerm() { ++tl_force3; }
ForceThreeTerm::~ForceThreeTerm() { --tl_force3; }

int conv_fwd_s3(const float* x, const void* xs, const float* w, const float* b, float* y, const ConvDims& d, void* ws, size_t wsb,
                hipStream_t s, void* xs_keep, float* stats_part) {
  const int T3 = d.kd * d.kh * d.kw;
  return run_s3(x, xs, w, b, y, d, d.C, d.K, (long)d.C * T3, T3, 0, ws, wsb, s, xs_keep, s3_layer_h2(d), nullptr, stats_part);
}

int conv_dgrad_s3(const float* dy, const void* dys, const float* w, float* dx, const ConvDims& d, void* ws, size_t wsb, hipStream_t s) {
  ConvDims t = d;
  t.C = d.K; t.K = d.C;
  const int T3 = d.kd * d.kh * d.kw;
  return run_s3(dy, dys, w, nullptr, dx, t, d.K, d.C, T3, (long)d.C * T3, 1, ws, wsb, s, nullptr, s3_layer_h2(d));
}

}
```

neuroclear_amd/csrc/convt_s3.hip:

```cpp
#include <cstdlib>

#include "common.hpp"
#include "s3_common.hpp"

namespace nc {
namespace {

typedef float f32x4 __attribute__((ext_vector_type(4)));
typedef __bf16 bf16x8 __attribute__((ext_vector_type(8)));
typedef _Float16 f16x8 __attribute__((ext_vector_type(8)));
typedef int i32x4 __attribute__((ext_vector_type(4)));

constexpr int kTWaves = 8;
constexpr int kTThreads = kTWaves * 64;
constexpr int kTCB = 4;

template <int NT>
__global__ void __launch_bounds__(256) k_pack_wT_s3(const float* __restrict__ w, unsigned short* __restrict__ wp, int C, int K, int QN, long total,
                                                    const unsigned* __restrict__ wcell) {
  const long i = (long)blockIdx.x * 256 + threadIdx.x;
  if (i >= total) return;
  const int j = (int)(i & 7);
  long r = i >> 3;
  const int lane = (int)(r & 63); r >>= 6;
  const int term = (int)(r % NT); r /= NT;
  const int ql = (int)(r % QN); r /= QN;
  const int NS = C / 32;
  const int s = (int)(r % NS); r /= NS;
  const int nqg = 8 / QN;
  const int qg = (int)(r % nqg);
  const int kg = (int)(r / nqg);
  const int m = lane & 15, g = lane >> 4;
  const int ci = (4 * s + g) * 8 + j, k = kg * 16 + m, q = qg * QN + ql;
  unsigned short t[3];
  if constexpr (NT == 3) s3_split(w[((long)ci * K + k) * 8 + q], t);
  else h2_split(w[((long)ci * K + k) * 8 + q] * h2_scale(*wcell), t);
  wp[i] = t[term];
}

struct TParams3 {
  const uint4* xs;
  const uint4* wp;
  const float* bias;
  float* y;
  uint2* ys;
  int N, C, K, D, H, W;
  int oblocks, ob0;
  const unsigned *xcell, *wcell;
  const unsigned* h2cell;
  int ngroups;
  long ntiles;
};

template <int QN, int NT = 3>
__global__ void __launch_bounds__(kTThreads, 1) k_convT_s3(const TParams3 p) {
  extern __shared__ __attribute__((aligned(1024))) unsigned char lds_raw[];
  const int tid = threadIdx.x, lane = tid & 63;
  const int wave = __builtin_amdgcn_readfirstlane(tid >> 6);
  const int m16 = lane & 15, g = lane >> 4;
  const long S = (long)p.D * p.H * p.W;
  const int NS = p.C / 32;
  constexpr int NQG = 8 / QN;
  const int xcd = blockIdx.x & 7, jx = blockIdx.x >> 3;
  const int grp = jx % p.ngroups;
  const long slot = (long)(jx / p.ngroups) * 8 + xcd;
  const long nslots = (long)(gridDim.x / (8 * p.ngroups)) * 8;
  const int kg = grp / NQG, qg = grp % NQG;

  {
    const uint4* src = p.wp + (long)grp * NS * QN * NT * 64;
    uint4* dst = reinterpret_cast<uint4*>(lds_raw);
    for (int i = tid; i < NS * QN * NT * 64; i += kTThreads) dst[i] = src[i];
  }
  __syncthreads();
  const i32x4* const wl = reinterpret_cast<const i32x4*>(lds_raw) + lane;

  const long tiles_per_n = (S + 511) / 512;
  const int H2 = 2 * p.H, W2 = 2 * p.W;
  const long S2 = 8 * S;
  float bb[4];
#pragma unroll
  for (int e = 0; e < 4; ++e) bb[e] = p.bias ? p.bias[kg * 16 + 4 * g + e] : 0.f;
  float oscx = 1.f, oscw = 1.f;
  if constexpr (NT == 2) { const float2 f = h2_unscale2(*p.xcell, *p.wcell); oscx = f.x; oscw = f.y; }

  for (long tile = slot; tile < p.ntiles; tile += nslots) {
// ... 15 lines not shown
    i32x4 B[kTCB][NT];
    auto load_b = [&](int s) __attribute__((always_inline)) {
      const uint4* xc = xn + (long)(4 * s + g) * NT * S;
#pragma unroll
      for (int cb = 0; cb < kTCB; ++cb)
#pragma unroll
        for (int t = 0; t < NT; ++t) B[cb][t] = __builtin_bit_cast(i32x4, xc[(long)t * S + vv[cb]]);
    };
    load_b(0);
#pragma unroll 1
    for (int s = 0; s < NS; ++s) {
      i32x4 Bc[kTCB][NT];
#pragma unroll
      for (int cb = 0; cb < kTCB; ++cb)
#pragma unroll
        for (int t = 0; t < NT; ++t) Bc[cb][t] = B[cb][t];
      if (s + 1 < NS) load_b(s + 1);
      const i32x4* ws = wl + (long)s * QN * NT * 64;
#pragma unroll
      for (int q = 0; q < QN; ++q) {
        i32x4 A[NT];
#pragma unroll
        for (int t = 0; t < NT; ++t) A[t] = ws[(q * NT + t) * 64];
        constexpr int NP = NT == 3 ? 6 : 3;
        constexpr int TA[6] = {NT - 1, NT == 3 ? 1 : 0, 0, 1, 0, 0};
        constexpr int TB[6] = {0, 1, NT == 3 ? 2 : 0, 0, 1, 0};
#pragma unroll
        for (int m = 0; m < NP; ++m)
#pragma unroll
          for (int cb = 0; cb < kTCB; ++cb) {
            if constexpr (NT == 3)
              acc[q][cb] = __builtin_amdgcn_mfma_f32_16x16x32_bf16(__builtin_bit_cast(bf16x8, A[TA[m]]), __builtin_bit_cast(bf16x8, Bc[cb][TB[m]]),
                                                                   acc[q][cb], 0, 0, 0);
            else
              acc[q][cb] = __builtin_amdgcn_mfma_f32_16x16x32_f16(__builtin_bit_cast(f16x8, A[TA[m]]), __builtin_bit_cast(f16x8, Bc[cb][TB[m]]),
                                                                  acc[q][cb], 0, 0, 0);
          }
      }
    }
#pragma unroll
    for (int cb = 0; cb < kTCB; ++cb) {
      const long v = v0 + cb * 16 + m16;
      if (v >= S) continue;
      const int ix = (int)(v % p.W), iy = (int)((v / p.W) % p.H), iz = (int)(v / ((long)p.W * p.H));
#pragma unroll
      for (int q = 0; q < QN; ++q) {
        const int qq = qg * QN + q;
        const long o = ((long)(2 * iz + (qq >> 2)) * H2 + (2 * iy + ((qq >> 1) & 1))) * W2 + 2 * ix + (qq & 1);
        float val[4];
#pragma unroll
        for (int e = 0; e < 4; ++e) val[e] = NT == 2 ? acc[q][cb][e] * oscx * oscw + bb[e] : acc[q][cb][e] + bb[e];
        if (p.y) {
          float* yk = p.y + ((long)n * p.K + kg * 16 + 4 * g) * S2 + o;
#pragma unroll
          for (int e = 0; e < 4; ++e) yk[(long)e * S2] = val[e];
        }
        if (p.ys && p.h2cell) {
          unsigned short t3[4][3];
          const float sc = h2_scale(*p.h2cell);
#pragma unroll
          for (int e = 0; e < 4; ++e) h2_split(val[e] * sc, t3[e]);
          const long blk = ((long)n * p.oblocks + p.ob0 + kg * 2 + (g >> 1)) * 2;
#pragma unroll
          for (int t = 0; t < 2; ++t)
            p.ys[((blk + t) * S2 + o) * 2 + (g & 1)] = make_uint2(t3[0][t] | ((unsigned)t3[1][t] << 16), t3[2][t] | ((unsigned)t3[3][t] << 16));
        } else if (p.ys) {
          unsigned short t3[4][3];
#pragma unroll
          for (int e = 0; e < 4; ++e) s3_split(val[e], t3[e]);
          const long blk = ((long)n * p.oblocks + p.ob0 + kg * 2 + (g >> 1)) * 3;
#pragma unroll
          for (int t = 0; t < 3; ++t)
            p.ys[((blk + t) * S2 + o) * 2 + (g & 1)] = make_uint2(t3[0][t] | ((unsigned)t3[1][t] << 16), t3[2][t] | ((unsigned)t3[3][t] << 16));
        }
      }
    }
  }
}

__global__ void __launch_bounds__(256) k_convT_bound(const float* __restrict__ w, const float* __restrict__ bias, int C, int K, float in_bound,
                                                     unsigned* __restrict__ cell) {
  __shared__ float part[4][64];
  __shared__ float red[64];
  const int col = threadIdx.x & 63, sl = threadIdx.x >> 6;
  const int kq = blockIdx.x * 64 + col;
  float sabs = 0.f;
  if (kq < K * 8) {
#pragma unroll 8
    for (int ci = sl; ci < C; ci += 4) sabs += fabsf(w[(long)ci * K * 8 + kq]);
  }
  part[sl][col] = sabs;
  __syncthreads();
  if (sl == 0) {
    const float t = (part[0][col] + part[1][col]) + (part[2][col] + part[3][col]);
    red[col] = kq < K * 8 ? t * in_bound + (bias ? fabsf(bias[kq >> 3]) : 0.f) : 0.f;
  }
  __syncthreads();
  for (int o = 32; o > 0; o >>= 1) {
    if ((int)threadIdx.x < o) red[threadIdx.x] = red[threadIdx.x + o] > red[threadIdx.x] ? red[threadIdx.x + o] : red[threadIdx.x];
    __syncthreads();
  }
  if (threadIdx.x == 0) atomicMax(cell, __float_as_uint(red[0] * 1.001f) & 0x7fffffffu);
}

int qn_for(int C) { return (C / 32) * 8 * 3 * 1024 <= 128 * 1024 ? 8 : 4; }

}

bool convT_s3x_supported(int N, int C, int D, int H, int W, int K) {
  static const bool on = !(getenv("NC_CONVT_S3X") && atoi(getenv("NC_CONVT_S3X")) == 0);
  const long S = (long)D * H * W;
  if (!on || C % 32 || K % 16 || C > 256 || N < 1) return false;
  if ((C / 32) * qn_for(C) * 3 * 1024 > 128 * 1024) return false;
  return (long)N * K * 8 * S < (1L << 40) && S * 16 * 3 * (C / 8) < (1L << 40);
}
size_t convT_s3x_ws_bytes(int C, int K) { return (size_t)C * K * 8 * 3 * 2 + 256; }

int convT_h2_bound(const float* w, const float* bias, int C, int K, float in_bound, unsigned* cell, hipStream_t s) {
  hipLaunchKernelGGL(k_convT_bound, dim3((unsigned)cdiv((long)K * 8, 64)), dim3(256), 0, s, w, bias, C, K, in_bound, cell);
  return check_launch("convT_h2_bound");
}

int convT_fwd_s3x(const void* xs, const float* w, const float* bias, float* y, void* ys, int ctot, int c0, int N, int C, int D, int H, int W,
                  int K, void* ws, size_t wsb, hipStream_t s, const unsigned* h2cell, const unsigned* xcell) {
  if (!xs || !w || (!y && !ys) || !ws) { set_error("convT_fwd_s3x: null pointer"); return NC_ERR_ARG; }
  if (!convT_s3x_supported(N, C, D, H, W, K) || ctot % 8 || c0 % 8) { set_error("convT_fwd_s3x: shape not covered"); return NC_ERR_SHAPE; }
  if (wsb < convT_s3x_ws_bytes(C, K)) { set_error("convT_fwd_s3x: workspace too small"); return NC_ERR_WS; }
  const int QN = qn_for(C);
  const int NT = xcell ? 2 : 3;
  const long total = (long)C * K * 8 * NT;
  unsigned* wcell = (unsigned*)((char*)ws + (size_t)C * K * 8 * 3 * 2);
  if (NT == 2) {
    if (int e = h2_zero_cells(wcell, 1, s)) return e;
    if (int e = h2_absmax(w, (long)C * K * 8, wcell, s)) return e;
    hipLaunchKernelGGL(k_pack_wT_s3<2>, dim3((unsigned)cdiv(total, 256)), dim3(256), 0, s, w, (unsigned short*)ws, C, K, QN, total, (const unsigned*)wcell);
  } else {
    hipLaunchKernelGGL(k_pack_wT_s3<3>, dim3((unsigned)cdiv(total, 256)), dim3(256), 0, s, w, (unsigned short*)ws, C, K, QN, total, (const unsigned*)nullptr);
  }
  if (int e = check_launch("pack_wT_s3")) return e;
  const long S = (long)D * H * W;
  TParams3 p{};
  p.xs = (const uint4*)xs; p.wp = (const uint4*)ws; p.bias = bias; p.y = y; p.ys = (uint2*)ys;
  p.N = N; p.C = C; p.K = K; p.D = D; p.H = H; p.W = W;
  p.oblocks = ctot / 8; p.ob0 = c0 / 8; p.h2cell = ys ? h2cell : nullptr; p.xcell = xcell; p.wcell = wcell;
  p.ngroups = (K / 16) * (8 / QN);
  p.ntiles = (long)N * cdiv(S, 512);
  int per_xcd = 32 / p.ngroups;
  if (per_xcd < 1) per_xcd = 1;
  const unsigned grid = (unsigned)(8 * p.ngroups * per_xcd);
  const size_t lds = (size_t)(C / 32) * QN * NT * 1024;
  auto launch = [&](auto kern) -> int {
    if (int e = raise_dyn_lds(kern, 160 * 1024, "convT_fwd_s3x")) return e;
    hipLaunchKernelGGL(kern, dim3(grid), dim3(kTThreads), lds, s, p);
    return check_launch("convT_s3");
  };
  if (NT == 2) return QN == 8 ? launch(k_convT_s3<8, 2>) : launch(k_convT_s3<4, 2>);
  return QN == 8 ? launch(k_convT_s3<8, 3>) : launch(k_convT_s3<4, 3>);
}

}
```

neuroclear_amd/csrc/gen_nets.hip:

```cpp

#include <atomic>
#include <cstdlib>

#include "common.hpp"

using namespace nc;

#define NC_TRY(expr) do { int e_ = (expr); if (e_) return e_; } while (0)

namespace {

size_t up64(size_t n) { return (n + 63) & ~(size_t)63; }

size_t s3_floats(size_t elems) { return up64((elems * 6 + 3) / 4); }
size_t align256(size_t b) { return (b + 255) & ~(size_t)255; }

std::atomic<int> g_unet_lean{getenv("NC_UNET_LEAN") ? (atoi(getenv("NC_UNET_LEAN")) != 0) : 1};
constexpr int kLeanBit0 = 10;
constexpr int kLeanBlocks[5] = {1, 3, 5, 6, 8};
int lean_index(int consumer) {
  for (int j = 0; j < 5; ++j) if (kLeanBlocks[j] == consumer) return j;
  return -1;
}

struct UBlock { int C, K, lvl; };
const UBlock kUB[10] = {{1, 64, 0},    {64, 64, 0},    {64, 128, 1},  {128, 128, 1}, {128, 256, 2},
                        {256, 256, 2}, {256, 256, 2}, {256, 128, 1}, {128, 128, 1}, {128, 64, 0}};

struct UPlan {
  int N, d[3][3];
  long S[3];
  size_t a1, cat1, p1, a2, cat2, p2, b1, b2, b3, e2a, e2b, e1, t1, raw[10], mean[10], rstd[10], saved;
  size_t xs3[10];
  size_t G1, G2, G3, H1, H2, H3, Q1, Q2, s1, s2, T, grads;
  size_t conv_ws, in_ws, convT_ws;
};

bool u_plan(UPlan& p, int N, int S0, int S1, int S2) {
  if (N < 1 || S0 < 4 || S1 < 4 || S2 < 4 || (S0 & 3) || (S1 & 3) || (S2 & 3)) return false;
  p = UPlan{};
  p.N = N;
  for (int l = 0; l < 3; ++l) {
    p.d[l][0] = S0 >> l; p.d[l][1] = S1 >> l; p.d[l][2] = S2 >> l;
    p.S[l] = (long)p.d[l][0] * p.d[l][1] * p.d[l][2];
  }
  const size_t n = (size_t)N, S = (size_t)p.S[0], Sh = (size_t)p.S[1], Sq = (size_t)p.S[2];
  size_t off = 0;
  auto take = [&](size_t k) { size_t r = off; off += up64(k); return r; };
  p.a1 = take(n * 64 * S); p.cat1 = take(n * 128 * S); p.p1 = take(n * 64 * Sh); p.a2 = take(n * 128 * Sh);
  p.cat2 = take(n * 256 * Sh); p.p2 = take(n * 128 * Sq); p.b1 = take(n * 256 * Sq); p.b2 = take(n * 256 * Sq);
  p.b3 = take(n * 256 * Sq); p.e2a = take(n * 128 * Sh); p.e2b = take(n * 128 * Sh); p.e1 = take(n * 64 * S);
  p.t1 = take(n * S);
  for (int i = 0; i < 10; ++i) {
    p.raw[i] = take(n * kUB[i].K * (size_t)p.S[kUB[i].lvl]);
    p.mean[i] = take(n * kUB[i].K);
    p.rstd[i] = take(n * kUB[i].K);
  }
  for (int i = 1; i < 10; ++i) { p.xs3[i] = off; off += s3_floats(n * kUB[i].C * (size_t)p.S[kUB[i].lvl]); }
  p.saved = off;
  off = 0;
  p.G1 = take(n * 64 * S); p.G2 = take(n * 64 * S); p.G3 = take(n * 128 * S);
  p.H1 = take(n * 128 * Sh); p.H2 = take(n * 128 * Sh); p.H3 = take(n * 256 * Sh);
  p.Q1 = take(n * 256 * Sq); p.Q2 = take(n * 256 * Sq); p.s1 = take(n * S); p.s2 = take(n * S);
  p.T = take(n * 64 * S);
  p.grads = off;
  auto upd = [&](int C, int K, int l, int k) {
    const size_t b = nc_conv_ws_bytes(N, C, p.d[l][0], p.d[l][1], p.d[l][2], K, k, k, k, 1, k / 2);
    if (b > p.conv_ws) p.conv_ws = b;
  };
  for (int i = 0; i < 10; ++i) upd(kUB[i].C, kUB[i].K, kUB[i].lvl, 3);
  upd(64, 1, 0, 1); upd(1, 1, 0, 1);
  p.in_ws = nc_instnorm_bwd_dbias_ws_bytes(N * 256, (long)S);
  for (int i = 1; i < 10; ++i) {
    const size_t b = s3x_stats_bytes(N, p.d[kUB[i].lvl][0], p.d[kUB[i].lvl][1], p.d[kUB[i].lvl][2], kUB[i].K, 3);
    if (b > p.in_ws) p.in_ws = b;
  }
  p.convT_ws = nc_convT_ws_bytes(N, 256, p.d[2][0], p.d[2][1], p.d[2][2], 128);
  const size_t c2 = nc_convT_ws_bytes(N, 128, p.d[1][0], p.d[1][1], p.d[1][2], 64);
  if (c2 > p.convT_ws) p.convT_ws = c2;
  return true;
}

struct UOff { size_t w[14], b[14], total; };
UOff u_offsets() {
  struct L { int id; size_t wn, bn; };
  const L order[14] = {{0, 64 * 1 * 27, 64},     {1, 64 * 64 * 27, 64},    {2, 128 * 64 * 27, 128},  {3, 128 * 128 * 27, 128},
                       {4, 256 * 128 * 27, 256}, {5, 256 * 256 * 27, 256}, {6, 256 * 256 * 27, 256}, {10, 256 * 128 * 8, 128},
                       {7, 128 * 256 * 27, 128}, {8, 128 * 128 * 27, 128}, {11, 128 * 64 * 8, 64},   {9, 64 * 128 * 27, 64},
                       {12, 64, 1},              {13, 1, 1}};
  UOff o{};
  size_t off = 0;
  for (const L& l : order) {
    o.w[l.id] = off; off += l.wn;
    o.b[l.id] = off; off += l.bn;
  }
  o.total = off;
  return o;
}

int gather_half(const float* src, float* dst, int N, int Ctot, int c0, int C, long S, hipStream_t s) {
  if (hipMemcpy2DAsync(dst, (size_t)C * S * 4, src + (size_t)c0 * S, (size_t)Ctot * S * 4, (size_t)C * S * 4, N,
                       hipMemcpyDeviceToDevice, s) != hipSuccess) {
    set_error("gather_half: hipMemcpy2DAsync failed");
    return NC_ERR_HIP;
  }
  return NC_OK;
}

size_t u_ws_bytes(const UPlan& p, bool bwd) {
  return align256(p.conv_ws) + align256(p.in_ws) + align256(p.convT_ws) + (bwd ? p.grads * sizeof(float) : 0) + 256;
}

}

extern "C" {

void nc_set_unet_lean(int on) { g_unet_lean.store(on != 0, std::memory_order_relaxed); }
int nc_get_unet_lean(void) { return g_unet_lean.load(std::memory_order_relaxed); }

size_t nc_unet_deconv_param_floats(void) { return u_offsets().total; }

size_t nc_unet_deconv_saved_floats(int N, int S0, int S1, int S2) {
  UPlan p;
  return u_plan(p, N, S0, S1, S2) ? p.saved : 0;
}

size_t nc_unet_deconv_train_ws_bytes(int N, int S0, int S1, int S2) {
  UPlan p;
  return u_plan(p, N, S0, S1, S2) ? u_ws_bytes(p, true) : 0;
}

int nc_unet_deconv_train_fwd(const float* params, const float* x, float* y, float* saved, int N, int S0, int S1, int S2,
                             void* ws, size_t ws_bytes, void* stream, unsigned* kept) {
  NetworkScope net_scope;
  if (!params || !x || !y || !saved) { set_error("unet_deconv_train_fwd: null pointer"); return NC_ERR_ARG; }
  UPlan p;
  if (!u_plan(p, N, S0, S1, S2)) {
    set_error("unet_deconv_train_fwd: every edge must be a positive multiple of 4 (got %d,%d,%d)", S0, S1, S2);
    return NC_ERR_SHAPE;
  }
  if (!ws || ws_bytes < u_ws_bytes(p, false)) { set_error("unet_deconv_train_fwd: workspace too small"); return NC_ERR_WS; }
  const UOff o = u_offsets();
  void* cws = ws;
  void* iws = (char*)ws + align256(p.conv_ws);
  float* V = saved;
  const float* P = params;
  if (kept) *kept = 0;
  hipStream_t hs = (hipStream_t)stream;
  static const bool fuse_on = !(getenv("NC_S3_TRAIN_FUSE") && atoi(getenv("NC_S3_TRAIN_FUSE")) == 0);
  const bool lean = g_unet_lean.load(std::memory_order_relaxed) != 0;
  bool use[10], pre[10], h2l[10];
  ConvDims cd[10];
  for (int i = 0; i < 10; ++i) {
    const UBlock& b = kUB[i];
    const int* d = p.d[b.lvl];
    use[i] = fuse_on && i >= 1 && conv_keep_supported(N, b.C, d[0], d[1], d[2], b.K, 3);
    pre[i] = false;
    h2l[i] = make_dims(cd[i], N, b.C, d[0], d[1], d[2], b.K, 3, 3, 3, 1, 1) && use[i] && conv_layer_h2(cd[i]);
  }
  unsigned kept_mask = 0;
  auto block = [&](int i, const float* in, float* out, size_t out_stride, int to, int to_ctot) -> int {
    const UBlock& b = kUB[i];
    const int* d = p.d[b.lvl];
    const long S = p.S[b.lvl];
    const bool epi = pre[i] && h2l[i] && epi_stats_mode() == 2 && s3x_stats_bytes(N, d[0], d[1], d[2], b.K, 3) && s3x_stats_bytes(N, d[0], d[1], d[2], b.K, 3) <= p.in_ws;
    if (pre[i]) {
      NC_TRY(conv_fwd_pre(V + p.xs3[i], P + o.w[i], P + o.b[i], V + p.raw[i], N, b.C, d[0], d[1], d[2], b.K, 3, cws, p.conv_ws, stream,
                          epi ? (float*)iws : nullptr));
      kept_mask |= 1u << i;
      if (h2l[i]) kept_mask |= 1u << (16 + i);
    } else {
      bool kept1 = false;
      NC_TRY(conv_fwd_keep(in, P + o.w[i], P + o.b[i], V + p.raw[i], N, b.C, d[0], d[1], d[2], b.K, 3, cws, p.conv_ws, stream,
                           i >= 1 ? (void*)(V + p.xs3[i]) : nullptr, &kept1));
      if (kept1) kept_mask |= 1u << i;
      if (kept1 && i >= 1 && conv_layer_h2(cd[i])) kept_mask |= 1u << (16 + i);
    }
    if (epi) NC_TRY(s3x_stats_finalize((const float*)iws, P + o.b[i], N, d[0], d[1], d[2], b.K, 3, 1e-5f, V + p.mean[i], V + p.rstd[i], hs));
    else NC_TRY(nc_instnorm_stats(V + p.raw[i], N * b.K, S, 1e-5f, V + p.mean[i], V + p.rstd[i], iws, p.in_ws, stream));
    if (to >= 0 && use[to]) {
      const int lj = lean && h2l[to] && to_ctot == b.K ? lean_index(to) : -1;
      if (lj >= 0) { out = nullptr; kept_mask |= 1u << (kLeanBit0 + lj); }
      NC_TRY(act_operand(cd[to], V + p.raw[i], V + p.mean[i], V + p.rstd[i], 0.f, out, (long)out_stride, V + p.xs3[to], N, b.K, S, to_ctot, 0, hs));
      if (to_ctot == b.K) pre[to] = true;
      return NC_OK;
    }
    if (out_stride == (size_t)b.K * S || N == 1)
      return nc_instnorm_act_fwd(V + p.raw[i], V + p.mean[i], V + p.rstd[i], 0.f, out, N * b.K, S, stream);
    for (int n = 0; n < N; ++n)
      NC_TRY(nc_instnorm_act_fwd(V + p.raw[i] + (size_t)n * b.K * S, V + p.mean[i] + n * b.K, V + p.rstd[i] + n * b.K, 0.f,
                                 out + n * out_stride, b.K, S, stream));
    return NC_OK;
  };
  const long S = p.S[0], Sh = p.S[1], Sq = p.S[2];
  const int *d0 = p.d[0], *d1 = p.d[1], *d2 = p.d[2];
  NC_TRY(block(0, x, V + p.a1, (size_t)64 * S, 1, 64));
  NC_TRY(block(1, V + p.a1, V + p.cat1, (size_t)128 * S, 9, 128));
  for (int n = 0; n < N; ++n)
    NC_TRY(nc_maxpool2_fwd(V + p.cat1 + (size_t)n * 128 * S, V + p.p1 + (size_t)n * 64 * Sh, 64, d0[0], d0[1], d0[2], stream));
  NC_TRY(block(2, V + p.p1, V + p.a2, (size_t)128 * Sh, 3, 128));
  NC_TRY(block(3, V + p.a2, V + p.cat2, (size_t)256 * Sh, 7, 256));
  for (int n = 0; n < N; ++n)
    NC_TRY(nc_maxpool2_fwd(V + p.cat2 + (size_t)n * 256 * Sh, V + p.p2 + (size_t)n * 128 * Sq, 128, d1[0], d1[1], d1[2], stream));
  NC_TRY(block(4, V + p.p2, V + p.b1, (size_t)256 * Sq, 5, 256));
  NC_TRY(block(5, V + p.b1, V + p.b2, (size_t)256 * Sq, 6, 256));
  NC_TRY(block(6, V + p.b2, V + p.b3, (size_t)256 * Sq, -1, 0));
  const bool ct2 = nc_convT_k2s2_split_active(1, 256, d2[0], d2[1], d2[2], 128) &&
                   p.conv_ws >= nc_convT_k2s2_split_ws_bytes(1, 256, d2[0], d2[1], d2[2], 128);
  static const bool ct_h2 = !(getenv("NC_CONVT_H2") && atoi(getenv("NC_CONVT_H2")) == 0);
  const bool ct2h = ct2 && h2l[7] && ct_h2;
  unsigned* cell7 = h2_cells_of(V + p.xs3[7], (size_t)N * 256 * Sh) + 1;
  if (ct2h) {
    NC_TRY(h2_zero_cells(cell7, 1, hs));
    NC_TRY(convT_h2_bound(P + o.w[10], P + o.b[10], 256, 128, sqrtf((float)Sq), cell7, hs));
  }
  for (int n = 0; n < N; ++n) {
    if (ct2h)
      NC_TRY(convT_fwd_split_h2(V + p.b3 + (size_t)n * 256 * Sq, P + o.w[10], P + o.b[10], V + p.cat2 + ((size_t)n * 256 + 128) * Sh,
                                (char*)(V + p.xs3[7]) + (size_t)n * 256 * Sh * 4, 256, 128, 1, 256, d2[0], d2[1], d2[2], 128, cell7, cws, p.conv_ws, hs));
    else if (ct2)
      NC_TRY(nc_convT_k2s2_fwd_split(V + p.b3 + (size_t)n * 256 * Sq, nullptr, P + o.w[10], P + o.b[10], V + p.cat2 + ((size_t)n * 256 + 128) * Sh,
                                     use[7] && !h2l[7] ? (char*)(V + p.xs3[7]) + (size_t)n * 256 * Sh * 6 : nullptr, 256, 128, 1, 256, d2[0], d2[1], d2[2], 128, cws,
                                     p.conv_ws, stream));
    else
      NC_TRY(nc_convT_k2s2_fwd(V + p.b3 + (size_t)n * 256 * Sq, P + o.w[10], P + o.b[10], V + p.cat2 + ((size_t)n * 256 + 128) * Sh,
                               1, 256, d2[0], d2[1], d2[2], 128, stream));
  }
  if (use[7]) {
    if (!ct2 || (h2l[7] && !ct2h)) NC_TRY(operand_into(cd[7], V + p.cat2 + (size_t)128 * Sh, (long)256 * Sh, V + p.xs3[7], N, 128, Sh, 256, 128, hs));
    pre[7] = true;
  }
  NC_TRY(block(7, V + p.cat2, V + p.e2a, (size_t)128 * Sh, 8, 128));
  NC_TRY(block(8, V + p.e2a, V + p.e2b, (size_t)128 * Sh, -1, 0));
  const bool ct1 = nc_convT_k2s2_split_active(1, 128, d1[0], d1[1], d1[2], 64) &&
                   p.conv_ws >= nc_convT_k2s2_split_ws_bytes(1, 128, d1[0], d1[1], d1[2], 64);
  const bool ct_s3 = use[9] && !h2l[9] && (ct1 || convT_fwd_s3_supported(1, 128, d1[0], d1[1], d1[2], 64));
  const bool ct1h = ct1 && h2l[9] && ct_h2;
  unsigned* cell9 = h2_cells_of(V + p.xs3[9], (size_t)N * 128 * S) + 1;
  if (ct1h) {
    NC_TRY(h2_zero_cells(cell9, 1, hs));
    NC_TRY(convT_h2_bound(P + o.w[11], P + o.b[11], 128, 64, sqrtf((float)Sh), cell9, hs));
  }
  for (int n = 0; n < N; ++n) {
    if (ct1h)
      NC_TRY(convT_fwd_split_h2(V + p.e2b + (size_t)n * 128 * Sh, P + o.w[11], P + o.b[11], V + p.cat1 + ((size_t)n * 128 + 64) * S,
                                (char*)(V + p.xs3[9]) + (size_t)n * 128 * S * 4, 128, 64, 1, 128, d1[0], d1[1], d1[2], 64, cell9, cws, p.conv_ws, hs));
    else if (ct1)
      NC_TRY(nc_convT_k2s2_fwd_split(V + p.e2b + (size_t)n * 128 * Sh, nullptr, P + o.w[11], P + o.b[11], V + p.cat1 + ((size_t)n * 128 + 64) * S,
                                     use[9] && !h2l[9] ? (char*)(V + p.xs3[9]) + (size_t)n * 128 * S * 6 : nullptr, 128, 64, 1, 128, d1[0], d1[1], d1[2], 64, cws,
                                     p.conv_ws, stream));
    else if (ct_s3)
      NC_TRY(convT_fwd_s3(V + p.e2b + (size_t)n * 128 * Sh, P + o.w[11], P + o.b[11], V + p.cat1 + ((size_t)n * 128 + 64) * S,
                          (char*)(V + p.xs3[9]) + (size_t)n * 128 * S * 6, 128, 64, 1, 128, d1[0], d1[1], d1[2], 64, stream));
    else
      NC_TRY(nc_convT_k2s2_fwd(V + p.e2b + (size_t)n * 128 * Sh, P + o.w[11], P + o.b[11], V + p.cat1 + ((size_t)n * 128 + 64) * S,
                               1, 128, d1[0], d1[1], d1[2], 64, stream));
  }
  if (use[9]) {
    if (!ct_s3 && !ct1h) NC_TRY(operand_into(cd[9], V + p.cat1 + (size_t)64 * S, (long)128 * S, V + p.xs3[9], N, 64, S, 128, 64, hs));
    pre[9] = true;
  }
  NC_TRY(block(9, V + p.cat1, V + p.e1, (size_t)64 * S, -1, 0));
  NC_TRY(nc_conv_fwd(V + p.e1, P + o.w[12], P + o.b[12], V + p.t1, N, 64, d0[0], d0[1], d0[2], 1, 1, 1, 1, 1, 0, cws, p.conv_ws, stream));
  NC_TRY(nc_conv_fwd(V + p.t1, P + o.w[13], P + o.b[13], y, N, 1, d0[0], d0[1], d0[2], 1, 1, 1, 1, 1, 0, cws, p.conv_ws, stream));
  if (kept) *kept = kept_mask;
  return nc_sigmoid_fwd(y, y, (long)N * S, stream);
}

int nc_unet_deconv_bwd(const float* params, const float* x, const float* y, const float* saved, const float* dy, float* dx,
                       float* dparams, int N, int S0, int S1, int S2, void* ws, size_t ws_bytes, void* stream, unsigned kept) {
  NetworkScope net_scope;
  if (!params || !x || !y || !saved || !dy || !dparams) { set_error("unet_deconv_bwd: null pointer"); return NC_ERR_ARG; }
  UPlan p;
  if (!u_plan(p, N, S0, S1, S2)) { set_error("unet_deconv_bwd: bad shape"); return NC_ERR_SHAPE; }
  if (!ws || ws_bytes < u_ws_bytes(p, true)) { set_error("unet_deconv_bwd: workspace too small"); return NC_ERR_WS; }
  const UOff o = u_offsets();
  hipStream_t hs = (hipStream_t)stream;
  void* cws = ws;
  void* iws = (char*)ws + align256(p.conv_ws);
  void* tws = (char*)iws + align256(p.in_ws);
  float* G = (float*)((char*)tws + align256(p.convT_ws));
  const float* V = saved;
  const float* P = params;
  float* DP = dparams;
  const long S = p.S[0], Sh = p.S[1], Sq = p.S[2];
  const int *d0 = p.d[0], *d1 = p.d[1], *d2 = p.d[2];
  const unsigned kept_mask = kept;
  static const bool fuse_bwd = !(getenv("NC_S3_TRAIN_FUSE") && atoi(getenv("NC_S3_TRAIN_FUSE")) == 0) &&
                               true;
  auto block_bwd = [&](int i, const float* g, const float* in, float* draw, float* gin, bool r1 = false) -> int {
    const UBlock& b = kUB[i];
    const int* d = p.d[b.lvl];
    const long Sl = p.S[b.lvl];
    ConvDims cdk;
    const bool now_h2 = make_dims(cdk, N, b.C, d[0], d[1], d[2], b.K, 3, 3, 3, 1, 1) && conv_layer_h2(cdk);
    const void* xs = ((kept_mask >> i) & 1) && (((kept_mask >> (16 + i)) & 1) != 0) == now_h2 ? (const void*)(V + p.xs3[i]) : nullptr;
    const int lj = lean_index(i);
    if (lj >= 0 && ((kept_mask >> (kLeanBit0 + lj)) & 1) &&
        !(xs && !h2_guard_can_flip() && conv_bwd_pre_supported(N, b.C, d[0], d[1], d[2], b.K, 3, gin != nullptr, p.conv_ws))) {
      NC_TRY(nc_instnorm_act_fwd(V + p.raw[i - 1], V + p.mean[i - 1], V + p.rstd[i - 1], 0.f, G + p.T, N * b.C, Sl, stream));
      in = G + p.T;
    }
    if (r1) {
      NC_TRY(instnorm_act_bwd_dbias_h2_rank1(g, P + o.w[12], V + p.raw[i], V + p.mean[i], V + p.rstd[i], 0.f, cws, DP + o.b[i], b.K, Sl, iws, p.in_ws,
                                             stream, conv_bwd_guard_words(cws, N, b.K, Sl)));
      return conv_bwd_pre(in, xs, P + o.w[i], gin, DP + o.w[i], N, b.C, d[0], d[1], d[2], b.K, 3, cws, p.conv_ws, stream, h2_guard_can_flip());
    }
    if (fuse_bwd && i >= 1 && conv_bwd_pre_supported(N, b.C, d[0], d[1], d[2], b.K, 3, gin != nullptr, p.conv_ws) &&
        instnorm_bwd_s3_supported(N, b.K, Sl)) {
      if (now_h2)
        NC_TRY(instnorm_act_bwd_dbias_h2(g, V + p.raw[i], V + p.mean[i], V + p.rstd[i], 0.f, cws, DP + o.b[i], N, b.K, Sl, iws, p.in_ws, stream,
                                         conv_bwd_guard_words(cws, N, b.K, Sl)));
      else
        NC_TRY(instnorm_act_bwd_dbias_s3(g, V + p.raw[i], V + p.mean[i], V + p.rstd[i], 0.f, cws, DP + o.b[i], N, b.K, Sl, iws, p.in_ws, stream));
      return conv_bwd_pre(in, xs, P + o.w[i], gin, DP + o.w[i], N, b.C, d[0], d[1], d[2], b.K, 3, cws, p.conv_ws, stream, now_h2 && h2_guard_can_flip());
    }
    NC_TRY(nc_instnorm_act_bwd_dbias(g, V + p.raw[i], V + p.mean[i], V + p.rstd[i], 0.f, draw, DP + o.b[i], N, b.K, Sl, iws,
                                     p.in_ws, stream));
    return conv_bwd_keep(in, xs, draw, P + o.w[i], gin, DP + o.w[i], N, b.C, d[0], d[1], d[2], b.K, 3, cws, p.conv_ws, stream);
  };
  auto upper_half = [&](const float* dcat, int Ctot, long Sl, const float** out) -> int {
    const int C = Ctot / 2;
    if (N == 1) { *out = dcat + (size_t)C * Sl; return NC_OK; }
    NC_TRY(gather_half(dcat, G + p.T, N, Ctot, C, C, Sl, hs));
    *out = G + p.T;
    return NC_OK;
  };
  NC_TRY(nc_sigmoid_bwd(dy, y, G + p.s1, (long)N * S, stream));
  NC_TRY(nc_conv_wgrad(V + p.t1, G + p.s1, DP + o.w[13], DP + o.b[13], N, 1, d0[0], d0[1], d0[2], 1, 1, 1, 1, 1, 0, cws, p.conv_ws, stream));
  NC_TRY(nc_conv_dgrad(G + p.s1, P + o.w[13], G + p.s2, N, 1, d0[0], d0[1], d0[2], 1, 1, 1, 1, 1, 0, cws, p.conv_ws, stream));
  ConvDims cd9;
  const bool r1 = g_unet_lean.load(std::memory_order_relaxed) != 0 && N == 1 && fuse_bwd &&
                  make_dims(cd9, N, 128, d0[0], d0[1], d0[2], 64, 3, 3, 3, 1, 1) && conv_layer_h2(cd9) &&
                  conv_bwd_pre_supported(N, 128, d0[0], d0[1], d0[2], 64, 3, true, p.conv_ws) && instnorm_bwd_s3_supported(N, 64, S);
  NC_TRY(nc_conv_wgrad(V + p.e1, G + p.s2, DP + o.w[12], DP + o.b[12], N, 64, d0[0], d0[1], d0[2], 1, 1, 1, 1, 1, 0, cws, p.conv_ws, stream));
  if (!r1) {
    NC_TRY(nc_conv_dgrad(G + p.s2, P + o.w[12], G + p.G1, N, 64, d0[0], d0[1], d0[2], 1, 1, 1, 1, 1, 0, cws, p.conv_ws, stream));
  }
  NC_TRY(block_bwd(9, r1 ? G + p.s2 : G + p.G1, V + p.cat1, G + p.G2, G + p.G3, r1));
  const float* g;
  NC_TRY(upper_half(G + p.G3, 128, S, &g));
  NC_TRY(nc_convT_k2s2_dgrad(g, P + o.w[11], G + p.H1, N, 128, d1[0], d1[1], d1[2], 64, tws, p.convT_ws, stream));
  NC_TRY(nc_convT_k2s2_wgrad(V + p.e2b, g, DP + o.w[11], DP + o.b[11], N, 128, d1[0], d1[1], d1[2], 64, tws, p.convT_ws, stream));
  NC_TRY(block_bwd(8, G + p.H1, V + p.e2a, G + p.H2, G + p.H1));
  NC_TRY(block_bwd(7, G + p.H1, V + p.cat2, G + p.H2, G + p.H3));
  NC_TRY(upper_half(G + p.H3, 256, Sh, &g));
  NC_TRY(nc_convT_k2s2_dgrad(g, P + o.w[10], G + p.Q1, N, 256, d2[0], d2[1], d2[2], 128, tws, p.convT_ws, stream));
  NC_TRY(nc_convT_k2s2_wgrad(V + p.b3, g, DP + o.w[10], DP + o.b[10], N, 256, d2[0], d2[1], d2[2], 128, tws, p.convT_ws, stream));
  NC_TRY(block_bwd(6, G + p.Q1, V + p.b2, G + p.Q2, G + p.Q1));
  NC_TRY(block_bwd(5, G + p.Q1, V + p.b1, G + p.Q2, G + p.Q1));
  NC_TRY(block_bwd(4, G + p.Q1, V + p.p2, G + p.Q2, G + p.Q1));
  for (int n = 0; n < N; ++n)
    NC_TRY(nc_maxpool2_bwd_add(G + p.Q1 + (size_t)n * 128 * Sq, V + p.cat2 + (size_t)n * 256 * Sh, G + p.H3 + (size_t)n * 256 * Sh,
                               G + p.H1 + (size_t)n * 128 * Sh, 128, d1[0], d1[1], d1[2], stream));
  NC_TRY(block_bwd(3, G + p.H1, V + p.a2, G + p.H2, G + p.H1));
  NC_TRY(block_bwd(2, G + p.H1, V + p.p1, G + p.H2, G + p.H1));
  for (int n = 0; n < N; ++n)
    NC_TRY(nc_maxpool2_bwd_add(G + p.H1 + (size_t)n * 64 * Sh, V + p.cat1 + (size_t)n * 128 * S, G + p.G3 + (size_t)n * 128 * S,
                               G + p.G1 + (size_t)n * 64 * S, 64, d0[0], d0[1], d0[2], stream));
  NC_TRY(block_bwd(1, G + p.G1, V + p.a1, G + p.G2, G + p.G1));
  return block_bwd(0, G + p.G1, x, G + p.G2, dx);
}

}

namespace {

struct LLayer { int C, K, k; };
const LLayer kLL[6] = {{1, 64, 7}, {64, 64, 5}, {64, 64, 3}, {64, 32, 1}, {32, 16, 1}, {16, 1, 1}};

struct LPlan {
  int N, d[3];
  long S;
  size_t w[6], params;
  size_t act[5], saved;
  size_t xs3[6];
  size_t g[2], grads;
  size_t conv_ws;
};

struct LTail {
  static constexpr size_t a = 0, e = 32 * 8, r = e + 64 * 8, E = r + 64 * 8, Ef = E + 1728 * 4, q = Ef + 1728 * 4, P = q + 1728 * 4 + 256,
                          Wf = P + (size_t)64 * 32 * 125 * 4 + 256, bytes = Wf + (size_t)64 * 32 * 125 * 4 + 256;
};

__global__ void __launch_bounds__(256) k_dl_shift27(const float* __restrict__ dy, float* __restrict__ dsh, int D, int H, int W) {
  const long S = (long)D * H * W;
  const int a = blockIdx.y, n = blockIdx.z;
  float* out = dsh + ((long)n * 32 + a) * S;
  const float* in = dy + (long)n * S;
  const int az = a / 9 - 1, ay = (a / 3) % 3 - 1, ax = a % 3 - 1;
  for (long v = (long)blockIdx.x * 256 + threadIdx.x; v < S; v += (long)gridDim.x * 256) {
    float r = 0.f;
    if (a < 27) {
      const int x = (int)(v % W), y = (int)((v / W) % H), z = (int)(v / ((long)W * H));
      const int sx = x - ax, sy = y - ay, sz = z - az;
      if ((unsigned)sx < (unsigned)W && (unsigned)sy < (unsigned)H && (unsigned)sz < (unsigned)D) r = in[((long)sz * H + sy) * W + sx];
    }
// ... 419 lines not shown
```

neuroclear_amd/ops.py:

```python
import ctypes
import os

import torch

from . import _lib
from ._lib import F, I, L_, P, Z, check, lib

_ws_cache = {}

prof = None


def prof_start(min_flop=0.0):
    global prof
    prof = []
    lib().nc_prof_begin(ctypes.c_double(min_flop))


_PATH = {0: 'direct', 1: 'mfma', 2: 'gemm', 3: 'flat', 4: 'taps', 5: 'k1', 6: 'to1', 7: 'img', 8: 'pg1', 9: 'split', 10: 'split2d', 11: 'split',
         12: 'lk'}


def prof_stop():
    global prof
# ... 794 lines not shown
        dp = torch.empty_like(pred)
        check(lib().nc_bce_logits_const_bwd(_ptr(pred), L_(pred.numel()), F(ctx.target), _ptr(g), _ptr(dp), _stream()),
              'nc_bce_logits_const_bwd')
        return dp, None


def bce_logits_const(pred, target):
    return _BceLogitsConst.apply(pred, float(target))


class _Mean(torch.autograd.Function):
    @staticmethod
    def forward(ctx, pred):
        pred = pred.contiguous()
        _chk(pred)
        _f32(pred)
        out = torch.empty((), dtype=torch.float32, device=pred.device)
        ws = workspace(lib().nc_loss_ws_bytes(L_(pred.numel())), pred.device, 'loss')
        check(lib().nc_mean_fwd(_ptr(pred), L_(pred.numel()), _ptr(out), _ptr(ws), Z(ws.numel()), _stream()), 'nc_mean_fwd')
        ctx.shape = pred.shape
        return out

    @staticmethod
    def backward(ctx, g):
        g = g.contiguous()
        dp = torch.empty(ctx.shape, dtype=torch.float32, device=g.device)
        check(lib().nc_mean_bwd(L_(dp.numel()), _ptr(g), _ptr(dp), _stream()), 'nc_mean_bwd')
        return dp


def mean(pred):
    return _Mean.apply(pred)


class _L1(torch.autograd.Function):
    @staticmethod
    def forward(ctx, a, b):
        a, b = a.contiguous(), b.contiguous()
        _chk(a, b)
        _f32(a, b)
        out = torch.empty((), dtype=torch.float32, device=a.device)
        ws = workspace(lib().nc_loss_ws_bytes(L_(a.numel())), a.device, 'loss')
        check(lib().nc_l1_fwd(_ptr(a), _ptr(b), L_(a.numel()), _ptr(out), _ptr(ws), Z(ws.numel()), _stream()),
              'nc_l1_fwd')
        ctx.save_for_backward(a, b)
        return out

    @staticmethod
    def backward(ctx, g):
        a, b = ctx.saved_tensors
        g = g.contiguous()
        da = torch.empty_like(a)
        check(lib().nc_l1_bwd(_ptr(a), _ptr(b), L_(a.numel()), _ptr(g), _ptr(da), _stream()), 'nc_l1_bwd')
        return da, None


def l1_loss(a, b):
    return _L1.apply(a, b)


def adam_step(p, g, m, v, lr, beta1, beta2, eps, step):
    _chk(p, g, m, v)
    _f32(p, g, m, v)
    check(lib().nc_adam_step(_ptr(p), _ptr(g), _ptr(m), _ptr(v), L_(p.numel()), F(lr), F(beta1), F(beta2), F(eps),
                             I(step), _stream()), 'nc_adam_step')


def set_force_direct(on):
    lib().nc_set_force_direct(I(1 if on else 0))


_param_gen = {}


def bump_param_generation(t):
    k = t.untyped_storage().data_ptr()
    _param_gen[k] = _param_gen.get(k, 0) + 1


def _param_generation(t):
    return _param_gen.get(t.untyped_storage().data_ptr(), 0)


_flat_grads = {}


def register_flat_grad(flat, grad):
    _flat_grads[flat.untyped_storage().data_ptr()] = [grad, set()]


def flat_grad_step_begin(flat):
    ent = _flat_grads.get(flat.untyped_storage().data_ptr())
    if ent is not None:
        ent[1].clear()


def _grad_destination(packed):
    ent = _flat_grads.get(packed.untyped_storage().data_ptr())
    if ent is not None and os.environ.get('NC_DIRECT_GRADS', '1') != '0':
        grad, written = ent
        off, n = packed.storage_offset(), packed.numel()
        if off + n <= grad.numel() and not any(a < off + n and off < b for a, b in written):
            written.add((off, off + n))
            return grad[off:off + n]
    return torch.empty_like(packed)


def _pack_params(params):
    p0 = params[0]
    off = p0.storage_offset()
    same = True
    for p in params:
        if (not p.is_contiguous()) or p.untyped_storage().data_ptr() != p0.untyped_storage().data_ptr() or \
                p.storage_offset() != off:
            same = False
            break
        off += p.numel()
    total = sum(p.numel() for p in params)
    if same:
        return p0.detach().as_strided((total,), (1,), p0.storage_offset())
    return torch.cat([p.detach().reshape(-1) for p in params])


class _PatchGAN(torch.autograd.Function):
    @staticmethod
    def forward(ctx, x, cfg, *params):
        n_layers, ndf, nd = cfg
        x = x.contiguous()
        _chk(x, *params)
        _f32(x, *params)
        if x.shape[1] != 1:
            raise _lib.NcError('fused PatchGAN expects one input channel')
        B = x.shape[0]
        D, H, W = (1, x.shape[2], x.shape[3]) if nd == 2 else tuple(x.shape[2:])
        L = lib()
        packed = _pack_params(params)
        if packed.numel() != L.nc_patchgan_param_floats(I(n_layers), I(ndf), I(nd)):
            raise _lib.NcError('fused PatchGAN: parameter count does not match (n_layers=%d, ndf=%d)' % (n_layers, ndf))
        od, oh, ow = I(0), I(0), I(0)
        import ctypes
        check(L.nc_patchgan_out_shape(I(B), I(D), I(H), I(W), I(n_layers), I(ndf), I(nd), ctypes.byref(od),
                                      ctypes.byref(oh), ctypes.byref(ow)), 'nc_patchgan_out_shape')
        oshape = (B, 1, oh.value, ow.value) if nd == 2 else (B, 1, od.value, oh.value, ow.value)
        y = torch.empty(oshape, dtype=torch.float32, device=x.device)
        saved = torch.empty(L.nc_patchgan_saved_floats(I(B), I(D), I(H), I(W), I(n_layers), I(ndf), I(nd)),
                            dtype=torch.float32, device=x.device)
        ws = workspace(L.nc_patchgan_ws_bytes(I(B), I(D), I(H), I(W), I(n_layers), I(ndf), I(nd)), x.device, 'patchgan')
        check(L.nc_patchgan_fwd(_ptr(packed), _ptr(x), _ptr(y), _ptr(saved), I(B), I(D), I(H), I(W), I(n_layers), I(ndf),
                                I(nd), _ptr(ws), Z(ws.numel()), _stream()), 'nc_patchgan_fwd')
        ctx.save_for_backward(x, saved)
        ctx.packed = packed
        ctx.packed_gen = _param_generation(packed)
        ctx.cfg = (cfg, (B, D, H, W), [tuple(p.shape) for p in params])
        return y

    @staticmethod
    def backward(ctx, dy):
        x, saved = ctx.saved_tensors
        (n_layers, ndf, nd), (B, D, H, W), shapes = ctx.cfg
        if _param_generation(ctx.packed) != ctx.packed_gen:
            raise _lib.NcError('fused PatchGAN: the parameters were updated (optimizer step / checkpoint load) between '
                               'this forward and its backward; the saved activations no longer match them')
        dy = dy.contiguous()
        want_x = ctx.needs_input_grad[0]
        want_p = any(ctx.needs_input_grad[2:])
        dx = torch.empty_like(x) if want_x else None
        dpar = _grad_target(ctx, 2) if want_p else None
        L = lib()
        ws = workspace(L.nc_patchgan_ws_bytes(I(B), I(D), I(H), I(W), I(n_layers), I(ndf), I(nd)), x.device, 'patchgan')
        check(L.nc_patchgan_bwd(_ptr(ctx.packed), _ptr(x), _ptr(saved), _ptr(dy), _ptr(dx), _ptr(dpar), I(B), I(D), I(H),
                                I(W), I(n_layers), I(ndf), I(nd), _ptr(ws), Z(ws.numel()), _stream()), 'nc_patchgan_bwd')
# ... 250 lines not shown
        check(L.nc_kgan_out_shape(I(B), I(D), I(H), I(W), I(ndf), I(nd), ctypes.byref(od), ctypes.byref(oh), ctypes.byref(ow)),
              'nc_kgan_out_shape')
        oshape = (B, 1, oh.value, ow.value) if nd == 2 else (B, 1, od.value, oh.value, ow.value)
        y = torch.empty(oshape, dtype=torch.float32, device=x.device)
        saved = torch.empty(L.nc_kgan_saved_floats(I(B), I(D), I(H), I(W), I(ndf), I(nd)), dtype=torch.float32, device=x.device)
        ws = workspace(L.nc_kgan_ws_bytes(I(B), I(D), I(H), I(W), I(ndf), I(nd)), x.device, 'kgan')
        check(L.nc_kgan_fwd(_ptr(packed), _ptr(x), _ptr(y), _ptr(saved), I(B), I(D), I(H), I(W), I(ndf), I(nd), _ptr(ws),
                            Z(ws.numel()), _stream()), 'nc_kgan_fwd')
        ctx.save_for_backward(x, saved)
        ctx.packed = packed
        ctx.packed_gen = _param_generation(packed)
        ctx.cfg = (cfg, (B, D, H, W), [tuple(p.shape) for p in params])
        return y

    @staticmethod
    def backward(ctx, dy):
        x, saved = ctx.saved_tensors
        (ndf, nd), (B, D, H, W), shapes = ctx.cfg
        if _param_generation(ctx.packed) != ctx.packed_gen:
            raise _lib.NcError('fused KernelGAN discriminator: the parameters were updated (optimizer step / checkpoint load) between '
                               'this forward and its backward; the saved activations no longer match them')
        dy = dy.contiguous()
        want_p = any(ctx.needs_input_grad[2:])
        dx = torch.empty_like(x) if ctx.needs_input_grad[0] else None
        dpar = _grad_target(ctx, 2) if want_p else None
        L = lib()
        ws = workspace(L.nc_kgan_ws_bytes(I(B), I(D), I(H), I(W), I(ndf), I(nd)), x.device, 'kgan')
        check(L.nc_kgan_bwd(_ptr(ctx.packed), _ptr(x), _ptr(saved), _ptr(dy), _ptr(dx), _ptr(dpar), I(B), I(D), I(H), I(W), I(ndf),
                            I(nd), _ptr(ws), Z(ws.numel()), _stream()), 'nc_kgan_bwd')
        grads = _param_grads(ctx, dpar, shapes, 2) if want_p else [None] * len(shapes)
        return (dx, None) + tuple(grads)


def kernelgan(x, params, nd, ndf=64):
    return _KernelGAN.apply(x, (int(ndf), int(nd)), *params)


def _grad_target(ctx, first):
    if all(ctx.needs_input_grad[first:]):
        return _grad_destination(ctx.packed)
    return torch.empty_like(ctx.packed)


def _param_grads(ctx, dpar, shapes, first):
    grads = [None] * len(shapes)
    off = 0
    for i, shp in enumerate(shapes):
        n = 1
        for s in shp:
            n *= s
        if ctx.needs_input_grad[first + i]:
            grads[i] = dpar[off:off + n].view(shp)
        off += n
    return grads


class _UnetDeconvTrain(torch.autograd.Function):
    @staticmethod
    def forward(ctx, x, *params):
        x = x.contiguous()
        _chk(x, *params)
        _f32(x, *params)
        N, _, S0, S1, S2 = x.shape
        L = lib()
        packed = _pack_params(params)
        if packed.numel() != L.nc_unet_deconv_param_floats():
            raise _lib.NcError('fused Unet_deconv: parameter count does not match')
        nsv = L.nc_unet_deconv_saved_floats(I(N), I(S0), I(S1), I(S2))
        if nsv == 0:
            raise _lib.NcError('fused Unet_deconv: every edge must be a positive multiple of 4, got %s' % ((S0, S1, S2),))
        saved = torch.empty(nsv, dtype=torch.float32, device=x.device)
        ws = workspace(L.nc_unet_deconv_train_ws_bytes(I(N), I(S0), I(S1), I(S2)), x.device, 'unet_train')
        y = torch.empty_like(x)
        e0 = _prof_begin()
        kept = ctypes.c_uint(0)
        check(L.nc_unet_deconv_train_fwd(_ptr(packed), _ptr(x), _ptr(y), _ptr(saved), I(N), I(S0), I(S1), I(S2), _ptr(ws),
                                         Z(ws.numel()), _stream(), ctypes.byref(kept)), 'nc_unet_deconv_train_fwd')
        ctx.kept = kept.value
        if e0 is not None:
            _prof_end(e0, 'unet_fwd', 2.0 * 663809 * x.numel())
        ctx.save_for_backward(x, y, saved)
        ctx.packed = packed
        ctx.packed_gen = _param_generation(packed)
        ctx.shapes = [tuple(p.shape) for p in params]
        return y

    @staticmethod
    def backward(ctx, dy):
        x, y, saved = ctx.saved_tensors
        if _param_generation(ctx.packed) != ctx.packed_gen:
            raise _lib.NcError('fused Unet_deconv: the parameters were updated between this forward and its backward')
        dy = dy.contiguous()
        N, _, S0, S1, S2 = x.shape
        L = lib()
        dx = torch.empty_like(x) if ctx.needs_input_grad[0] else None
        dpar = _grad_target(ctx, 1)
        ws = workspace(L.nc_unet_deconv_train_ws_bytes(I(N), I(S0), I(S1), I(S2)), x.device, 'unet_train')
        e0 = _prof_begin()
        check(L.nc_unet_deconv_bwd(_ptr(ctx.packed), _ptr(x), _ptr(y), _ptr(saved), _ptr(dy), _ptr(dx), _ptr(dpar), I(N),
                                   I(S0), I(S1), I(S2), _ptr(ws), Z(ws.numel()), _stream(), ctypes.c_uint(ctx.kept)), 'nc_unet_deconv_bwd')
        if e0 is not None:
            _prof_end(e0, 'unet_bwd', 2.0 * (2 * 663809 - 1728) * x.numel())
        return (dx,) + tuple(_param_grads(ctx, dpar, ctx.shapes, 1))


def unet_deconv_train(x, params):
    return _UnetDeconvTrain.apply(x, *params)


class _DeepLinear(torch.autograd.Function):
    @staticmethod
    def forward(ctx, x, *params):
        x = x.contiguous()
        _chk(x, *params)
        _f32(x, *params)
        N, _, S0, S1, S2 = x.shape
        L = lib()
        packed = _pack_params(params)
        if packed.numel() != L.nc_deep_linear_param_floats():
            raise _lib.NcError('fused DeepLinearGenerator: parameter count does not match')
        need = any(ctx.needs_input_grad)
        saved = torch.empty(L.nc_deep_linear_saved_floats(I(N), I(S0), I(S1), I(S2)), dtype=torch.float32,
                            device=x.device) if need else None
        ws = workspace(L.nc_deep_linear_ws_bytes(I(N), I(S0), I(S1), I(S2)), x.device, 'deep_linear')
        y = torch.empty_like(x)
        e0 = _prof_begin()
        kept = ctypes.c_uint(0)
        check(L.nc_deep_linear_fwd(_ptr(packed), _ptr(x), _ptr(y), _ptr(saved), I(N), I(S0), I(S1), I(S2), _ptr(ws),
                                   Z(ws.numel()), _stream(), ctypes.byref(kept)), 'nc_deep_linear_fwd')
        ctx.kept = kept.value
        if e0 is not None:
            _prof_end(e0, 'deep_linear_fwd', 2.0 * 647120 * x.numel())
        if need:
            ctx.save_for_backward(x, saved)
            ctx.packed = packed
            ctx.packed_gen = _param_generation(packed)
            ctx.shapes = [tuple(p.shape) for p in params]
        return y

    @staticmethod
    def backward(ctx, dy):
        x, saved = ctx.saved_tensors
        if _param_generation(ctx.packed) != ctx.packed_gen:
            raise _lib.NcError('fused DeepLinearGenerator: the parameters were updated between this forward and its backward')
        dy = dy.contiguous()
        N, _, S0, S1, S2 = x.shape
        L = lib()
        dx = torch.empty_like(x) if ctx.needs_input_grad[0] else None
        dpar = _grad_target(ctx, 1)
        ws = workspace(L.nc_deep_linear_ws_bytes(I(N), I(S0), I(S1), I(S2)), x.device, 'deep_linear')
        e0 = _prof_begin()
        check(L.nc_deep_linear_bwd(_ptr(ctx.packed), _ptr(x), _ptr(saved), _ptr(dy), _ptr(dx), _ptr(dpar), I(N), I(S0), I(S1),
                                   I(S2), _ptr(ws), Z(ws.numel()), _stream(), ctypes.c_uint(ctx.kept)), 'nc_deep_linear_bwd')
        if e0 is not None:
            _prof_end(e0, 'deep_linear_bwd', 2.0 * (2 * 647120 - (0 if dx is not None else 21952)) * x.numel())
        return (dx,) + tuple(_param_grads(ctx, dpar, ctx.shapes, 1))


def deep_linear(x, params):
    return _DeepLinear.apply(x, *params)


def gen_lp_supported(kind, shape):
    if conv_precision != 'bf16' or len(shape) != 5 or shape[1] != 1:
        return False
    N, _, S0, S1, S2 = shape
    fn = lib().nc_unet_deconv_lp_supported if kind == 'unet' else lib().nc_deep_linear_lp_supported
    return bool(fn(I(N), I(S0), I(S1), I(S2), I(_DT['bf16'])))


class _GenLp(torch.autograd.Function):

    @staticmethod
# ... 102 lines not shown
```

Measured before the change: 54.31 million.

## Batch UNet weight packing into one prep pass reused by forward and backward

After: 54.93 million (median of 6 runs). 1.1% higher.

```diff
diff --git a/include/nc_hip.h b/include/nc_hip.h
--- a/include/nc_hip.h
+++ b/include/nc_hip.h
@@ -178,6 +178,13 @@
                        float* dparams, int N, int S0, int S1, int S2, void* ws, size_t ws_bytes, void* stream, unsigned kept);
 void nc_set_unet_lean(int on);
 int nc_get_unet_lean(void);
+void nc_set_unet_wprep(int on);
+int nc_get_unet_wprep(void);
+int nc_unet_wprep_layout(int N, int S0, int S1, int S2, int block, int form, size_t* pack_off, size_t* pack_bytes, size_t* cell_off,
+                         size_t* bound_off);
+int nc_s3x_pack_h2_debug(const float* w, int C, int K, int form, const unsigned* cell_a, const unsigned* cell_b, void* wp, unsigned* wcell,
+                         void* stream);
+int nc_convT_h2_bound_debug(const float* w, const float* bias, int C, int K, float in_bound, unsigned* cell, void* stream);
 size_t nc_deep_linear_param_floats(void);
 size_t nc_deep_linear_saved_floats(int N, int S0, int S1, int S2);
 size_t nc_deep_linear_ws_bytes(int N, int S0, int S1, int S2);
diff --git a/neuroclear_amd/_lib.py b/neuroclear_amd/_lib.py
--- a/neuroclear_amd/_lib.py
+++ b/neuroclear_amd/_lib.py
@@ -32,7 +32,7 @@
                 fn.restype = ctypes.c_size_t
             elif name == 'nc_last_error':
                 fn.restype = ctypes.c_char_p
-            elif name in ('nc_set_force_direct', 'nc_prof_begin', 'nc_sconv_set_cfg', 'nc_sconv_set_tune', 'nc_set_conv_split', 'nc_set_s3_fusion', 'nc_set_c8x_mode', 'nc_set_split_terms', 'nc_set_h2_guard', 'nc_set_epi_stats', 'nc_set_dl_collapse', 'nc_set_p2d_terms', 'nc_set_s3x_w64', 'nc_set_unet_lean'):
+            elif name in ('nc_set_force_direct', 'nc_prof_begin', 'nc_sconv_set_cfg', 'nc_sconv_set_tune', 'nc_set_conv_split', 'nc_set_s3_fusion', 'nc_set_c8x_mode', 'nc_set_split_terms', 'nc_set_h2_guard', 'nc_set_epi_stats', 'nc_set_dl_collapse', 'nc_set_p2d_terms', 'nc_set_s3x_w64', 'nc_set_unet_lean', 'nc_set_unet_wprep'):
                 fn.restype = None
             else:
                 fn.restype = ctypes.c_int
diff --git a/neuroclear_amd/csrc/api.hip b/neuroclear_amd/csrc/api.hip
--- a/neuroclear_amd/csrc/api.hip
+++ b/neuroclear_amd/csrc/api.hip
@@ -409,14 +409,14 @@
 
 namespace nc {
 int conv_fwd_keep(const float* x, const float* w, const float* bias, float* y, int N, int C, int D, int H, int W, int K, int ks,
-                  void* ws, size_t ws_bytes, void* stream, void* xs_keep, bool* kept) {
+                  void* ws, size_t ws_bytes, void* stream, void* xs_keep, bool* kept, const S3xPrepared* prep) {
   ConvDims d;
   *kept = false;
   if (xs_keep && make_dims(d, N, C, D, H, W, K, ks, ks, ks, 1, ks / 2) && fwd_path(d) == 9 && wgrad_path(d) == 9) {
     if (!x || !w || !y) { set_error("conv_fwd: null pointer"); return NC_ERR_ARG; }
     ProfScope ps(0, 9, d, 0, (hipStream_t)stream);
     *kept = true;
-    return conv_fwd_s3(x, nullptr, w, bias, y, d, ws, ws_bytes, (hipStream_t)stream, xs_keep);
+    return conv_fwd_s3(x, nullptr, w, bias, y, d, ws, ws_bytes, (hipStream_t)stream, xs_keep, nullptr, prep);
   }
   return nc_conv_fwd(x, w, bias, y, N, C, D, H, W, K, ks, ks, ks, 1, ks / 2, ws, ws_bytes, stream);
 }
@@ -427,13 +427,13 @@
 }
 
 int conv_fwd_pre(const void* xs, const float* w, const float* bias, float* y, int N, int C, int D, int H, int W, int K, int ks, void* ws,
-                 size_t ws_bytes, void* stream, float* stats_part) {
+                 size_t ws_bytes, void* stream, float* stats_part, const S3xPrepared* prep) {
   ConvDims d;
   if (!xs || !w || !y) { set_error("conv_fwd_pre: null pointer"); return NC_ERR_ARG; }
   if (!make_dims(d, N, C, D, H, W, K, ks, ks, ks, 1, ks / 2) || fwd_path(d) != 9) { set_error("conv_fwd_pre: layer not on the split-operand kernels"); return NC_ERR_SHAPE; }
   ProfScope ps(0, 9, d, 0, (hipStream_t)stream);
   if (stats_part && !(conv_layer_h2(d) && ks == 3)) { set_error("conv_fwd_pre: epilogue statistics exist for the two-term 3^3 layers only"); return NC_ERR_ARG; }
-  return conv_fwd_s3(nullptr, xs, w, bias, y, d, ws, ws_bytes, (hipStream_t)stream, nullptr, stats_part);
+  return conv_fwd_s3(nullptr, xs, w, bias, y, d, ws, ws_bytes, (hipStream_t)stream, nullptr, stats_part, prep);
 }
 
 bool conv_bwd_pre_supported(int N, int C, int D, int H, int W, int K, int ks, bool want_dx, size_t ws_bytes) {
@@ -442,7 +442,7 @@
          (!want_dx || dgrad_path(d) == 9);
 }
 int conv_bwd_pre(const float* x, const void* xs, const float* w, float* dx, float* dw, int N, int C, int D, int H, int W, int K, int ks,
-                 void* ws, size_t ws_bytes, void* stream, bool dy_guarded) {
+                 void* ws, size_t ws_bytes, void* stream, bool dy_guarded, const S3xPrepared* prep) {
   ConvDims d;
   hipStream_t s = (hipStream_t)stream;
   if (!conv_bwd_pre_supported(N, C, D, H, W, K, ks, dx != nullptr, ws_bytes) || !make_dims(d, N, C, D, H, W, K, ks, ks, ks, 1, ks / 2)) {
@@ -452,7 +452,7 @@
   if ((!x && !xs) || !w || !dw || !ws) { set_error("conv_bwd_pre: null pointer"); return NC_ERR_ARG; }
   if (dx) {
     ProfScope ps(1, 9, d, 0, s);
-    if (int e = conv_bwd_s3(x, nullptr, w, dx, dw, d, ws, ws_bytes, s, 1, nullptr, dy_guarded)) return e;
+    if (int e = conv_bwd_s3(x, nullptr, w, dx, dw, d, ws, ws_bytes, s, 1, nullptr, dy_guarded, prep)) return e;
   }
   ProfScope ps(2, 9, d, 0, s);
   return conv_bwd_s3(x, nullptr, w, dx, dw, d, ws, ws_bytes, s, 2, xs, dy_guarded);
diff --git a/neuroclear_amd/csrc/common.hpp b/neuroclear_amd/csrc/common.hpp
--- a/neuroclear_amd/csrc/common.hpp
+++ b/neuroclear_amd/csrc/common.hpp
@@ -177,8 +177,9 @@
                 long S, int ctot, int c0, hipStream_t s);
 int act_split3(const float* x, const float* mean, const float* rstd, float slope, float* y, long ystride, void* ys, int N, int C, long S,
                int ctot, int c0, hipStream_t s);
+struct S3xPrepared { const void* wp; const unsigned* wcell; };
 int conv_fwd_s3(const float* x, const void* xs, const float* w, const float* b, float* y, const ConvDims& d, void* ws, size_t wsb,
-                hipStream_t s, void* xs_keep = nullptr, float* stats_part = nullptr);
+                hipStream_t s, void* xs_keep = nullptr, float* stats_part = nullptr, const S3xPrepared* prep = nullptr);
 bool epi_stats_on();
 void epi_stats_set(int on);
 int epi_stats_mode();
@@ -187,18 +188,26 @@
 int conv_dgrad_s3(const float* dy, const void* dys, const float* w, float* dx, const ConvDims& d, void* ws, size_t wsb, hipStream_t s);
 size_t s3_bwd_ws_bytes(const ConvDims& d);
 int conv_bwd_s3(const float* x, const float* dy, const float* w, float* dx, float* dw, const ConvDims& d, void* ws, size_t wsb,
-                hipStream_t s, int phase, const void* xs = nullptr, bool dy_guarded = false);
+                hipStream_t s, int phase, const void* xs = nullptr, bool dy_guarded = false, const S3xPrepared* prep = nullptr);
 int conv_fwd_keep(const float* x, const float* w, const float* bias, float* y, int N, int C, int D, int H, int W, int K, int ks,
-                  void* ws, size_t ws_bytes, void* stream, void* xs_keep, bool* kept);
+                  void* ws, size_t ws_bytes, void* stream, void* xs_keep, bool* kept, const S3xPrepared* prep = nullptr);
 int conv_bwd_keep(const float* x, const void* xs, const float* dy, const float* w, float* dx, float* dw, int N, int C, int D, int H,
                   int W, int K, int ks, void* ws, size_t ws_bytes, void* stream);
 bool s3x_supported(int N, int Cin, int D, int H, int W, int Kout, int KS);
 size_t s3x_packed_bytes(int Cin, int Kout, int KS, int NT = 3);
+int s3x_ksteps(int Cin, int KS);
+constexpr int kWPrepMaxSegs = 18, kWPrepMaxBounds = 2, kWPrepBoundCell0 = kWPrepMaxSegs, kWPrepCellBytes = 256;
+struct WPrepSeg { const float* w; int Cin, Kout, flip; unsigned a_bits; int b_cell; unsigned* ext_cell; };
+struct WPrepBound { const float* w; const float* bias; int C, K; float in_bound; int cell; };
+size_t wprep_bytes(const WPrepSeg* segs, int n);
+int wprep_run(const WPrepSeg* segs, int n, const WPrepBound* bounds, int nb, void* region, S3xPrepared* out, hipStream_t s);
+int s3x_pack_h2(const float* w, int Cin, int Kout, int KS, long so, long si, int flip, int split_c, const unsigned* cell_a, const unsigned* cell_b,
+                unsigned* wcell, void* wp_ws, hipStream_t s);
 void s3x_set_terms(int t);
 int s3x_get_terms();
 int conv_s3x_h2(const void* xs, const unsigned* cell_a, const unsigned* cell_b, int split_c, const float* w, const float* bias, float* y, int N,
                 int Cin, int D, int H, int W, int Kout, int KS, long so, long si, int flip, unsigned* wcell, void* wp_ws, hipStream_t s,
-                const unsigned* guard = nullptr, float* stats_part = nullptr);
+                const unsigned* guard = nullptr, float* stats_part = nullptr, const S3xPrepared* prep = nullptr);
 size_t s3x_stats_bytes(int N, int D, int H, int W, int Kout, int KS);
 int s3x_stats_finalize(const float* stats_part, const float* bias, int N, int D, int H, int W, int Kout, int KS, float eps, float* mean, float* rstd,
                        hipStream_t s);
@@ -255,10 +264,10 @@
              long si, int flip, void* wp_ws, hipStream_t s, const unsigned* guard = nullptr);
 bool conv_keep_supported(int N, int C, int D, int H, int W, int K, int ks);
 int conv_fwd_pre(const void* xs, const float* w, const float* bias, float* y, int N, int C, int D, int H, int W, int K, int ks, void* ws,
-                 size_t ws_bytes, void* stream, float* stats_part = nullptr);
+                 size_t ws_bytes, void* stream, float* stats_part = nullptr, const S3xPrepared* prep = nullptr);
 bool conv_bwd_pre_supported(int N, int C, int D, int H, int W, int K, int ks, bool want_dx, size_t ws_bytes);
 int conv_bwd_pre(const float* x, const void* xs, const float* w, float* dx, float* dw, int N, int C, int D, int H, int W, int K, int ks,
-                 void* ws, size_t ws_bytes, void* stream, bool dy_guarded = false);
+                 void* ws, size_t ws_bytes, void* stream, bool dy_guarded = false, const S3xPrepared* prep = nullptr);
 bool instnorm_bwd_s3_supported(int N, int C, long S);
 int instnorm_act_bwd_dbias_s3(const float* dy, const float* x, const float* mean, const float* rstd, float slope, void* dxs,
                               float* dbias, int N, int C, long S, void* ws, size_t ws_bytes, void* stream);
diff --git a/neuroclear_amd/csrc/conv_s3x.hip b/neuroclear_amd/csrc/conv_s3x.hip
--- a/neuroclear_amd/csrc/conv_s3x.hip
+++ b/neuroclear_amd/csrc/conv_s3x.hip
@@ -4,6 +4,7 @@
 
 #include "common.hpp"
 #include "s3_common.hpp"
+#include "w_prep.hpp"
 
 namespace nc {
 namespace {
@@ -40,57 +41,14 @@
                                                     const unsigned* __restrict__ cell_a, const unsigned* __restrict__ cell_b) {
   const long i = (long)blockIdx.x * 256 + threadIdx.x;
   if (i >= total) return;
-  const int T2 = KS * KS, T3 = T2 * KS, NB = NCH * KS;
-  const int j = (int)(i & 7);
-  long q = i >> 3;
-  const int lane = (int)(q & 63); q >>= 6;
-  const int f = (int)(q % (2 * NT)); q /= 2 * NT;
-  const int s = (int)(q % NS); q /= NS;
-  const int half = (int)(q & 1);
-  const int cot = (int)(q >> 1);
-  const int rb = f / NT, term = f % NT;
-  const int g = lane >> 4, m = lane & 15;
-  const int T = 4 * s + g;
-  const int bi = T / T2, tp = T % T2;
-  unsigned short t[3] = {0, 0, 0};
-  if (bi < NB) {
-    const int chunk = bi / KS, dz = bi % KS;
-#ifdef NC_S3X_B128
-    const int jj = j;
-#else
-    const int jj = (g & 1) ? ((j + 4) & 7) : j;
-#endif
-    const long co = cot * 64 + half * 32 + rb * 16 + m, ci = chunk * 8 + jj;
-    const int tap = dz * T2 + tp;
-    const float v = w[co * so + ci * si + (flip ? T3 - 1 - tap : tap)];
-    if constexpr (NT == 3) split3(v, t);
-    else h2_split(v * (ci >= split_c ? h2_group_factor(*cell_a, *cell_b) : 1.f) * h2_scale(*amax), t);
-  }
-  wp[i] = t[term];
+  if constexpr (NT == 3) wp[i] = pack_w_s3x_elem<3>(w, i, NCH, KS, NS, so, si, flip, 0u, split_c, 0u, 0u);
+  else wp[i] = pack_w_s3x_elem<2>(w, i, NCH, KS, NS, so, si, flip, *amax, split_c, *cell_a, *cell_b);
 }
 
 __global__ void __launch_bounds__(256) k_absmax_w(const float* __restrict__ w, long n, int T3, int C, int split_c, const unsigned* __restrict__ cell_a,
                                                   const unsigned* __restrict__ cell_b, unsigned* __restrict__ out) {
-  unsigned m = 0;
-  const float gf = split_c < C ? h2_group_factor(*cell_a, *cell_b) : 1.f;
-  for (long i = (long)blockIdx.x * 256 + threadIdx.x; i < n; i += (long)gridDim.x * 256) {
-    const int ci = (int)((i / T3) % C);
-    const unsigned b = __float_as_uint(w[i] * (ci >= split_c ? gf : 1.f)) & 0x7fffffffu;
-    if (b < 0x7f800000u && b > m) m = b;
-  }
-#pragma unroll
-  for (int o = 32; o > 0; o >>= 1) {
-    const unsigned q = (unsigned)__shfl_xor((int)m, o);
-    m = q > m ? q : m;
-  }
   __shared__ unsigned wm[4];
-  if ((threadIdx.x & 63) == 0) wm[threadIdx.x >> 6] = m;
-  __syncthreads();
-  if (threadIdx.x == 0) {
-    unsigned b = wm[0];
-    for (int k = 1; k < 4; ++k) b = wm[k] > b ? wm[k] : b;
-    if (b) atomicMax(out, b);
-  }
+  absmax_w_block(w, n, T3, C, split_c, *cell_a, *cell_b, out, blockIdx.x, gridDim.x, wm);
 }
 
 __global__ void __launch_bounds__(256) k_pack_w_c1k7(const float* __restrict__ w, unsigned short* __restrict__ wp, int NS, long total,
@@ -1175,26 +1133,34 @@
   return x_plan(N, D, H, W, Kout / 64, KS).ok;
 }
 
+int s3x_pack_h2(const float* w, int Cin, int Kout, int KS, long so, long si, int flip, int split_c, const unsigned* cell_a, const unsigned* cell_b,
+                unsigned* wcell, void* wp_ws, hipStream_t s) {
+  const int NCH = Cin / 8, NS = s3x_ksteps(Cin, KS), T3 = KS * KS * KS;
+  if (int e = h2_zero_cells(wcell, 1, s)) return e;
+  const long nw = (long)Kout * Cin * T3;
+  hipLaunchKernelGGL(k_absmax_w, dim3((unsigned)(cdiv(nw, 256 * 8) < 256 ? cdiv(nw, 256 * 8) : 256)), dim3(256), 0, s, w, nw, T3, Cin,
+                     flip ? Cin : split_c, cell_a, cell_b, wcell);
+  const long total = (long)(s3x_packed_bytes(Cin, Kout, KS, 2) / 2);
+  hipLaunchKernelGGL(k_pack_w_s3x<2>, dim3((unsigned)cdiv(total, 256)), dim3(256), 0, s, w, (unsigned short*)wp_ws, NCH, KS, NS, so, si, flip, total,
+                     (const unsigned*)wcell, flip ? Cin : split_c, cell_a, cell_b);
+  return check_launch("conv_s3x_h2 pack");
+}
+
 int conv_s3x_h2(const void* xs, const unsigned* cell_a, const unsigned* cell_b, int split_c, const float* w, const float* bias, float* y, int N,
                 int Cin, int D, int H, int W, int Kout, int KS, long so, long si, int flip, unsigned* wcell, void* wp_ws, hipStream_t s,
-                const unsigned* guard, float* stats_part) {
+                const unsigned* guard, float* stats_part, const S3xPrepared* prep) {
   const bool k32 = Kout == 32;
   if (k32 && (KS != 5 || stats_part || guard)) { set_error("conv_s3x_h2: 32 output channels for unguarded 5^3 launches only"); return NC_ERR_SHAPE; }
   const XPlan pl = x_plan(N, D, H, W, k32 ? 1 : Kout / 64, KS, 2, k32);
   if (!pl.ok) { set_error("conv_s3x_h2: shape not covered"); return NC_ERR_SHAPE; }
   if (split_c < Cin && (flip || !cell_b || split_c % 8)) { set_error("conv_s3x_h2: scale groups only for the forward weight layout"); return NC_ERR_ARG; }
   if (stats_part && KS != 3) { set_error("conv_s3x_h2: epilogue statistics exist for the 3^3 layers only (the layers in front of an InstanceNorm)"); return NC_ERR_ARG; }
-  const int NCH = Cin / 8, NS = s3x_ksteps(Cin, KS), T3 = KS * KS * KS;
+  const int NCH = Cin / 8, NS = s3x_ksteps(Cin, KS);
   if (Cin % 32) { set_error("conv_s3x_h2: channels must be a multiple of 32"); return NC_ERR_SHAPE; }
-  if (int e = h2_zero_cells(wcell, 1, s)) return e;
-  const long nw = (long)Kout * Cin * T3;
   if (!cell_b) cell_b = cell_a;
-  hipLaunchKernelGGL(k_absmax_w, dim3((unsigned)(cdiv(nw, 256 * 8) < 256 ? cdiv(nw, 256 * 8) : 256)), dim3(256), 0, s, w, nw, T3, Cin,
-                     flip ? Cin : split_c, cell_a, cell_b, wcell);
-  const long total = (long)(s3x_packed_bytes(Cin, Kout, KS, 2) / 2);
-  hipLaunchKernelGGL(k_pack_w_s3x<2>, dim3((unsigned)cdiv(total, 256)), dim3(256), 0, s, w, (unsigned short*)wp_ws, NCH, KS, NS, so, si, flip, total,
-                     (const unsigned*)wcell, flip ? Cin : split_c, cell_a, cell_b);
-  if (int e = check_launch("conv_s3x_h2 pack")) return e;
+  if (prep) {
+    wcell = const_cast<unsigned*>(prep->wcell); wp_ws = const_cast<void*>(prep->wp);
+  } else if (int e = s3x_pack_h2(w, Cin, Kout, KS, so, si, flip, split_c, cell_a, cell_b, wcell, wp_ws, s)) return e;
   XParams p{};
   p.xs = (const uint4*)xs; p.wp = (const uint4*)wp_ws; p.bias = bias; p.y = y; p.amax_x = cell_a; p.amax_w = wcell; p.guard = guard;
   p.N = N; p.NCH = NCH; p.D = D; p.H = H; p.W = W; p.K = Kout;
diff --git a/neuroclear_amd/csrc/conv_split.hip b/neuroclear_amd/csrc/conv_split.hip
--- a/neuroclear_amd/csrc/conv_split.hip
+++ b/neuroclear_amd/csrc/conv_split.hip
@@ -438,7 +438,7 @@
 
 int run_s3(const float* x, const void* xs_pre, const float* w, const float* bias, float* y, const ConvDims& d, int Cin, int Kout,
            long so, long si, int flip, void* ws, size_t wsb, hipStream_t s, void* xs_keep = nullptr, bool h2 = false, unsigned* guard_pre = nullptr,
-           float* stats_part = nullptr) {
+           float* stats_part = nullptr, const S3xPrepared* prep = nullptr) {
   const int KS = d.kd;
   const SPlan pl = s_plan(d.H, d.W, KS);
   const long S = (long)d.D * d.H * d.W;
@@ -466,7 +466,7 @@
     }
     if (stats_part && dual) { set_error("conv_s3 (two-term): epilogue statistics need an operand that cannot fall back"); return NC_ERR_ARG; }
     if (int e = conv_s3x_h2(xs, cells, cells + 1, flip ? Cin : Cin / 2, w, bias, y, d.N, Cin, d.D, d.H, d.W, Kout, KS, so, si, flip, gw + 16,
-                            (char*)ws + xb + 256, s, dual ? guard : nullptr, stats_part)) return e;
+                            (char*)ws + xb + 256, s, dual ? guard : nullptr, stats_part, prep)) return e;
     if (dual) return conv_s3x(xs, w, bias, y, d.N, Cin, d.D, d.H, d.W, Kout, KS, so, si, flip, (char*)ws + xb + 256, s, guard);
     return NC_OK;
   }
@@ -1372,7 +1372,7 @@
 }
 unsigned* conv_bwd_guard_words(void* ws, int N, int K, long S) { return (unsigned*)((char*)ws + align256((size_t)N * K * S * 6)); }
 int conv_bwd_s3(const float* x, const float* dy, const float* w, float* dx, float* dw, const ConvDims& d, void* ws, size_t wsb,
-                hipStream_t s, int phase, const void* xs, bool dy_guarded) {
+                hipStream_t s, int phase, const void* xs, bool dy_guarded, const S3xPrepared* prep) {
   const long S = (long)d.D * d.H * d.W;
   const size_t A = align256((size_t)d.N * d.K * S * 6) + 256;
   if (!ws || wsb < s3_bwd_ws_bytes(d)) { set_error("conv_bwd_s3: workspace too small"); return NC_ERR_WS; }
@@ -1397,7 +1397,8 @@
     ConvDims t = d;
     t.C = d.K; t.K = d.C;
     const int T3 = d.kd * d.kh * d.kw;
-    return run_s3(dy, ws, w, nullptr, dx, t, d.K, d.C, T3, (long)d.C * T3, 1, (char*)ws + A, wsb - A, s, nullptr, h2, guarded ? yg : nullptr);
+    return run_s3(dy, ws, w, nullptr, dx, t, d.K, d.C, T3, (long)d.C * T3, 1, (char*)ws + A, wsb - A, s, nullptr, h2, guarded ? yg : nullptr, nullptr,
+                  h2 ? prep : nullptr);
   }
   return run_ws(x, xs, dy, ws, dw, d, (char*)ws + A, wsb - A, s, guarded ? yg : nullptr);
 }
@@ -1463,9 +1464,10 @@
 ForceThreeTerm::~ForceThreeTerm() { --tl_force3; }
 
 int conv_fwd_s3(const float* x, const void* xs, const float* w, const float* b, float* y, const ConvDims& d, void* ws, size_t wsb,
-                hipStream_t s, void* xs_keep, float* stats_part) {
+                hipStream_t s, void* xs_keep, float* stats_part, const S3xPrepared* prep) {
   const int T3 = d.kd * d.kh * d.kw;
-  return run_s3(x, xs, w, b, y, d, d.C, d.K, (long)d.C * T3, T3, 0, ws, wsb, s, xs_keep, s3_layer_h2(d), nullptr, stats_part);
+  return run_s3(x, xs, w, b, y, d, d.C, d.K, (long)d.C * T3, T3, 0, ws, wsb, s, xs_keep, s3_layer_h2(d), nullptr, stats_part,
+                s3_layer_h2(d) ? prep : nullptr);
 }
 
 int conv_dgrad_s3(const float* dy, const void* dys, const float* w, float* dx, const ConvDims& d, void* ws, size_t wsb, hipStream_t s) {
diff --git a/neuroclear_amd/csrc/convt_s3.hip b/neuroclear_amd/csrc/convt_s3.hip
--- a/neuroclear_amd/csrc/convt_s3.hip
+++ b/neuroclear_amd/csrc/convt_s3.hip
@@ -2,6 +2,7 @@
 
 #include "common.hpp"
 #include "s3_common.hpp"
+#include "w_prep.hpp"
 
 namespace nc {
 namespace {
@@ -183,25 +184,7 @@
                                                      unsigned* __restrict__ cell) {
   __shared__ float part[4][64];
   __shared__ float red[64];
-  const int col = threadIdx.x & 63, sl = threadIdx.x >> 6;
-  const int kq = blockIdx.x * 64 + col;
-  float sabs = 0.f;
-  if (kq < K * 8) {
-#pragma unroll 8
-    for (int ci = sl; ci < C; ci += 4) sabs += fabsf(w[(long)ci * K * 8 + kq]);
-  }
-  part[sl][col] = sabs;
-  __syncthreads();
-  if (sl == 0) {
-    const float t = (part[0][col] + part[1][col]) + (part[2][col] + part[3][col]);
-    red[col] = kq < K * 8 ? t * in_bound + (bias ? fabsf(bias[kq >> 3]) : 0.f) : 0.f;
-  }
-  __syncthreads();
-  for (int o = 32; o > 0; o >>= 1) {
-    if ((int)threadIdx.x < o) red[threadIdx.x] = red[threadIdx.x + o] > red[threadIdx.x] ? red[threadIdx.x + o] : red[threadIdx.x];
-    __syncthreads();
-  }
-  if (threadIdx.x == 0) atomicMax(cell, __float_as_uint(red[0] * 1.001f) & 0x7fffffffu);
+  convT_bound_block(w, bias, C, K, in_bound, cell, (int)blockIdx.x, part, red);
 }
 
 int qn_for(int C) { return (C / 32) * 8 * 3 * 1024 <= 128 * 1024 ? 8 : 4; }
diff --git a/neuroclear_amd/csrc/gen_nets.hip b/neuroclear_amd/csrc/gen_nets.hip
--- a/neuroclear_amd/csrc/gen_nets.hip
+++ b/neuroclear_amd/csrc/gen_nets.hip
@@ -27,11 +27,23 @@
 const UBlock kUB[10] = {{1, 64, 0},    {64, 64, 0},    {64, 128, 1},  {128, 128, 1}, {128, 256, 2},
                         {256, 256, 2}, {256, 256, 2}, {256, 128, 1}, {128, 128, 1}, {128, 64, 0}};
 
+std::atomic<int> g_unet_wprep{getenv("NC_UNET_WPREP") ? (atoi(getenv("NC_UNET_WPREP")) != 0) : 1};
+constexpr unsigned kKeptWPrep = 1u << 15;
+void wprep_segs(WPrepSeg (&sg)[18]) {
+  for (int i = 1; i < 10; ++i) {
+    sg[2 * (i - 1)] = WPrepSeg{nullptr, kUB[i].C, kUB[i].K, 0, 0u, -1, nullptr};
+    sg[2 * (i - 1) + 1] = WPrepSeg{nullptr, kUB[i].K, kUB[i].C, 1, 0u, -1, nullptr};
+  }
+}
+unsigned f32_bits(float f) { unsigned b; __builtin_memcpy(&b, &f, 4); return b; }
+
+
 struct UPlan {
   int N, d[3][3];
   long S[3];
   size_t a1, cat1, p1, a2, cat2, p2, b1, b2, b3, e2a, e2b, e1, t1, raw[10], mean[10], rstd[10], saved;
   size_t xs3[10];
+  size_t wprep;
   size_t G1, G2, G3, H1, H2, H3, Q1, Q2, s1, s2, T, grads;
   size_t conv_ws, in_ws, convT_ws;
 };
@@ -57,6 +69,12 @@
     p.rstd[i] = take(n * kUB[i].K);
   }
   for (int i = 1; i < 10; ++i) { p.xs3[i] = off; off += s3_floats(n * kUB[i].C * (size_t)p.S[kUB[i].lvl]); }
+  {
+    WPrepSeg sg[18];
+    wprep_segs(sg);
+    p.wprep = off;
+    off += up64((wprep_bytes(sg, 18) + 3) / 4);
+  }
   p.saved = off;
   off = 0;
   p.G1 = take(n * 64 * S); p.G2 = take(n * 64 * S); p.G3 = take(n * 128 * S);
@@ -115,10 +133,39 @@
 
 extern "C" {
 
+void nc_set_unet_wprep(int on) { g_unet_wprep.store(on != 0, std::memory_order_relaxed); }
+int nc_get_unet_wprep(void) { return g_unet_wprep.load(std::memory_order_relaxed); }
 void nc_set_unet_lean(int on) { g_unet_lean.store(on != 0, std::memory_order_relaxed); }
 int nc_get_unet_lean(void) { return g_unet_lean.load(std::memory_order_relaxed); }
 
 size_t nc_unet_deconv_param_floats(void) { return u_offsets().total; }
+
+int nc_unet_wprep_layout(int N, int S0, int S1, int S2, int block, int form, size_t* pack_off, size_t* pack_bytes, size_t* cell_off,
+                         size_t* bound_off) {
+  UPlan p;
+  if (!u_plan(p, N, S0, S1, S2) || block < 1 || block > 9 || form < 0 || form > 1) { set_error("unet_wprep_layout: bad argument"); return NC_ERR_ARG; }
+  WPrepSeg sg[18];
+  wprep_segs(sg);
+  const int k = 2 * (block - 1) + form;
+  size_t off = kWPrepCellBytes;
+  for (int j = 0; j < k; ++j) off += s3x_packed_bytes(sg[j].Cin, sg[j].Kout, 3, 2);
+  if (pack_off) *pack_off = p.wprep * 4 + off;
+  if (pack_bytes) *pack_bytes = s3x_packed_bytes(sg[k].Cin, sg[k].Kout, 3, 2);
+  if (cell_off) *cell_off = p.wprep * 4 + (size_t)k * 4;
+  if (bound_off) *bound_off = block == 7 ? p.wprep * 4 + (size_t)kWPrepBoundCell0 * 4 : block == 9 ? p.wprep * 4 + (size_t)(kWPrepBoundCell0 + 1) * 4 : 0;
+  return NC_OK;
+}
+int nc_s3x_pack_h2_debug(const float* w, int C, int K, int form, const unsigned* cell_a, const unsigned* cell_b, void* wp, unsigned* wcell,
+                         void* stream) {
+  if (!w || !cell_a || !cell_b || !wp || !wcell || C % 64 || K % 64) { set_error("s3x_pack_h2_debug: bad argument"); return NC_ERR_ARG; }
+  if (form) return s3x_pack_h2(w, K, C, 3, 27, (long)C * 27, 1, K, cell_a, cell_a, wcell, wp, (hipStream_t)stream);
+  return s3x_pack_h2(w, C, K, 3, (long)C * 27, 27, 0, C / 2, cell_a, cell_b, wcell, wp, (hipStream_t)stream);
+}
+int nc_convT_h2_bound_debug(const float* w, const float* bias, int C, int K, float in_bound, unsigned* cell, void* stream) {
+  if (!w || !cell) { set_error("convT_h2_bound_debug: null pointer"); return NC_ERR_ARG; }
+  NC_TRY(h2_zero_cells(cell, 1, (hipStream_t)stream));
+  return convT_h2_bound(w, bias, C, K, in_bound, cell, (hipStream_t)stream);
+}
 
 size_t nc_unet_deconv_saved_floats(int N, int S0, int S1, int S2) {
   UPlan p;
@@ -158,7 +205,50 @@
     pre[i] = false;
     h2l[i] = make_dims(cd[i], N, b.C, d[0], d[1], d[2], b.K, 3, 3, 3, 1, 1) && use[i] && conv_layer_h2(cd[i]);
   }
+  const long S = p.S[0], Sh = p.S[1], Sq = p.S[2];
+  const int *d0 = p.d[0], *d1 = p.d[1], *d2 = p.d[2];
+  const bool ct2 = nc_convT_k2s2_split_active(1, 256, d2[0], d2[1], d2[2], 128) &&
+                   p.conv_ws >= nc_convT_k2s2_split_ws_bytes(1, 256, d2[0], d2[1], d2[2], 128);
+  static const bool ct_h2 = !(getenv("NC_CONVT_H2") && atoi(getenv("NC_CONVT_H2")) == 0);
+  const bool ct2h = ct2 && h2l[7] && ct_h2;
+  const bool ct1 = nc_convT_k2s2_split_active(1, 128, d1[0], d1[1], d1[2], 64) &&
+                   p.conv_ws >= nc_convT_k2s2_split_ws_bytes(1, 128, d1[0], d1[1], d1[2], 64);
+  const bool ct1h = ct1 && h2l[9] && ct_h2;
+  unsigned* cell7 = h2_cells_of(V + p.xs3[7], (size_t)N * 256 * Sh) + 1;
+  unsigned* cell9 = h2_cells_of(V + p.xs3[9], (size_t)N * 128 * S) + 1;
   unsigned kept_mask = 0;
+  S3xPrepared prep[18] = {};
+  bool bound7 = false, bound9 = false;
+  if (g_unet_wprep.load(std::memory_order_relaxed) != 0) {
+    WPrepSeg sg[18];
+    wprep_segs(sg);
+    WPrepBound wb[2];
+    int nb = 0, any = 0;
+    for (int i = 1; i < 10; ++i) {
+      if (!h2l[i]) continue;
+      WPrepSeg& f = sg[2 * (i - 1)];
+      f.a_bits = f32_bits(sqrtf((float)p.S[kUB[i].lvl]));
+      f.w = P + o.w[i];
+      if (i == 7 || i == 9) {
+        if (i == 7 ? ct2h : ct1h) {
+          f.b_cell = kWPrepBoundCell0 + nb;
+          f.ext_cell = i == 7 ? cell7 : cell9;
+          wb[nb++] = i == 7 ? WPrepBound{P + o.w[10], P + o.b[10], 256, 128, sqrtf((float)Sq), 0}
+                            : WPrepBound{P + o.w[11], P + o.b[11], 128, 64, sqrtf((float)Sh), 0};
+          (i == 7 ? bound7 : bound9) = true;
+        } else {
+          f.w = nullptr;
+        }
+      }
+      sg[2 * (i - 1) + 1].w = P + o.w[i];
+      any = 1;
+    }
+    if (any) {
+      NC_TRY(wprep_run(sg, 18, wb, nb, V + p.wprep, prep, hs));
+      kept_mask |= kKeptWPrep;
+    }
+  }
+  auto prep_of = [&](int seg) -> const S3xPrepared* { return prep[seg].wp ? &prep[seg] : nullptr; };
   auto block = [&](int i, const float* in, float* out, size_t out_stride, int to, int to_ctot) -> int {
     const UBlock& b = kUB[i];
     const int* d = p.d[b.lvl];
@@ -166,13 +256,13 @@
     const bool epi = pre[i] && h2l[i] && epi_stats_mode() == 2 && s3x_stats_bytes(N, d[0], d[1], d[2], b.K, 3) && s3x_stats_bytes(N, d[0], d[1], d[2], b.K, 3) <= p.in_ws;
     if (pre[i]) {
       NC_TRY(conv_fwd_pre(V + p.xs3[i], P + o.w[i], P + o.b[i], V + p.raw[i], N, b.C, d[0], d[1], d[2], b.K, 3, cws, p.conv_ws, stream,
-                          epi ? (float*)iws : nullptr));
+                          epi ? (float*)iws : nullptr, i >= 1 ? prep_of(2 * (i - 1)) : nullptr));
       kept_mask |= 1u << i;
       if (h2l[i]) kept_mask |= 1u << (16 + i);
     } else {
       bool kept1 = false;
       NC_TRY(conv_fwd_keep(in, P + o.w[i], P + o.b[i], V + p.raw[i], N, b.C, d[0], d[1], d[2], b.K, 3, cws, p.conv_ws, stream,
-                           i >= 1 ? (void*)(V + p.xs3[i]) : nullptr, &kept1));
+                           i >= 1 ? (void*)(V + p.xs3[i]) : nullptr, &kept1, i >= 1 ? prep_of(2 * (i - 1)) : nullptr));
       if (kept1) kept_mask |= 1u << i;
       if (kept1 && i >= 1 && conv_layer_h2(cd[i])) kept_mask |= 1u << (16 + i);
     }
@@ -192,8 +282,6 @@
                                  out + n * out_stride, b.K, S, stream));
     return NC_OK;
   };
-  const long S = p.S[0], Sh = p.S[1], Sq = p.S[2];
-  const int *d0 = p.d[0], *d1 = p.d[1], *d2 = p.d[2];
   NC_TRY(block(0, x, V + p.a1, (size_t)64 * S, 1, 64));
   NC_TRY(block(1, V + p.a1, V + p.cat1, (size_t)128 * S, 9, 128));
   for (int n = 0; n < N; ++n)
@@ -205,12 +293,7 @@
   NC_TRY(block(4, V + p.p2, V + p.b1, (size_t)256 * Sq, 5, 256));
   NC_TRY(block(5, V + p.b1, V + p.b2, (size_t)256 * Sq, 6, 256));
   NC_TRY(block(6, V + p.b2, V + p.b3, (size_t)256 * Sq, -1, 0));
-  const bool ct2 = nc_convT_k2s2_split_active(1, 256, d2[0], d2[1], d2[2], 128) &&
-                   p.conv_ws >= nc_convT_k2s2_split_ws_bytes(1, 256, d2[0], d2[1], d2[2], 128);
-  static const bool ct_h2 = !(getenv("NC_CONVT_H2") && atoi(getenv("NC_CONVT_H2")) == 0);
-  const bool ct2h = ct2 && h2l[7] && ct_h2;
-  unsigned* cell7 = h2_cells_of(V + p.xs3[7], (size_t)N * 256 * Sh) + 1;
-  if (ct2h) {
+  if (ct2h && !bound7) {
     NC_TRY(h2_zero_cells(cell7, 1, hs));
     NC_TRY(convT_h2_bound(P + o.w[10], P + o.b[10], 256, 128, sqrtf((float)Sq), cell7, hs));
   }
@@ -232,12 +315,8 @@
   }
   NC_TRY(block(7, V + p.cat2, V + p.e2a, (size_t)128 * Sh, 8, 128));
   NC_TRY(block(8, V + p.e2a, V + p.e2b, (size_t)128 * Sh, -1, 0));
-  const bool ct1 = nc_convT_k2s2_split_active(1, 128, d1[0], d1[1], d1[2], 64) &&
-                   p.conv_ws >= nc_convT_k2s2_split_ws_bytes(1, 128, d1[0], d1[1], d1[2], 64);
   const bool ct_s3 = use[9] && !h2l[9] && (ct1 || convT_fwd_s3_supported(1, 128, d1[0], d1[1], d1[2], 64));
-  const bool ct1h = ct1 && h2l[9] && ct_h2;
-  unsigned* cell9 = h2_cells_of(V + p.xs3[9], (size_t)N * 128 * S) + 1;
-  if (ct1h) {
+  if (ct1h && !bound9) {
     NC_TRY(h2_zero_cells(cell9, 1, hs));
     NC_TRY(convT_h2_bound(P + o.w[11], P + o.b[11], 128, 64, sqrtf((float)Sh), cell9, hs));
   }
@@ -288,6 +367,18 @@
   const unsigned kept_mask = kept;
   static const bool fuse_bwd = !(getenv("NC_S3_TRAIN_FUSE") && atoi(getenv("NC_S3_TRAIN_FUSE")) == 0) &&
                                true;
+  const bool wprep_now = g_unet_wprep.load(std::memory_order_relaxed) != 0;
+  S3xPrepared prepd[10] = {};
+  {
+    WPrepSeg sg[18];
+    wprep_segs(sg);
+    const char* region = (const char*)(V + p.wprep);
+    size_t off = kWPrepCellBytes;
+    for (int k = 0; k < 18; ++k) {
+      if (k & 1) prepd[k / 2 + 1] = S3xPrepared{region + off, (const unsigned*)region + k};
+      off += s3x_packed_bytes(sg[k].Cin, sg[k].Kout, 3, 2);
+    }
+  }
   auto block_bwd = [&](int i, const float* g, const float* in, float* draw, float* gin, bool r1 = false) -> int {
     const UBlock& b = kUB[i];
     const int* d = p.d[b.lvl];
@@ -295,6 +386,7 @@
     ConvDims cdk;
     const bool now_h2 = make_dims(cdk, N, b.C, d[0], d[1], d[2], b.K, 3, 3, 3, 1, 1) && conv_layer_h2(cdk);
     const void* xs = ((kept_mask >> i) & 1) && (((kept_mask >> (16 + i)) & 1) != 0) == now_h2 ? (const void*)(V + p.xs3[i]) : nullptr;
+    const S3xPrepared* pd = i >= 1 && gin && now_h2 && (kept_mask & kKeptWPrep) && ((kept_mask >> (16 + i)) & 1) && wprep_now ? &prepd[i] : nullptr;
     const int lj = lean_index(i);
     if (lj >= 0 && ((kept_mask >> (kLeanBit0 + lj)) & 1) &&
         !(xs && !h2_guard_can_flip() && conv_bwd_pre_supported(N, b.C, d[0], d[1], d[2], b.K, 3, gin != nullptr, p.conv_ws))) {
@@ -304,7 +396,7 @@
     if (r1) {
       NC_TRY(instnorm_act_bwd_dbias_h2_rank1(g, P + o.w[12], V + p.raw[i], V + p.mean[i], V + p.rstd[i], 0.f, cws, DP + o.b[i], b.K, Sl, iws, p.in_ws,
                                              stream, conv_bwd_guard_words(cws, N, b.K, Sl)));
-      return conv_bwd_pre(in, xs, P + o.w[i], gin, DP + o.w[i], N, b.C, d[0], d[1], d[2], b.K, 3, cws, p.conv_ws, stream, h2_guard_can_flip());
+      return conv_bwd_pre(in, xs, P + o.w[i], gin, DP + o.w[i], N, b.C, d[0], d[1], d[2], b.K, 3, cws, p.conv_ws, stream, h2_guard_can_flip(), pd);
     }
     if (fuse_bwd && i >= 1 && conv_bwd_pre_supported(N, b.C, d[0], d[1], d[2], b.K, 3, gin != nullptr, p.conv_ws) &&
         instnorm_bwd_s3_supported(N, b.K, Sl)) {
@@ -313,7 +405,7 @@
                                          conv_bwd_guard_words(cws, N, b.K, Sl)));
       else
         NC_TRY(instnorm_act_bwd_dbias_s3(g, V + p.raw[i], V + p.mean[i], V + p.rstd[i], 0.f, cws, DP + o.b[i], N, b.K, Sl, iws, p.in_ws, stream));
-      return conv_bwd_pre(in, xs, P + o.w[i], gin, DP + o.w[i], N, b.C, d[0], d[1], d[2], b.K, 3, cws, p.conv_ws, stream, now_h2 && h2_guard_can_flip());
+      return conv_bwd_pre(in, xs, P + o.w[i], gin, DP + o.w[i], N, b.C, d[0], d[1], d[2], b.K, 3, cws, p.conv_ws, stream, now_h2 && h2_guard_can_flip(), pd);
     }
     NC_TRY(nc_instnorm_act_bwd_dbias(g, V + p.raw[i], V + p.mean[i], V + p.rstd[i], 0.f, draw, DP + o.b[i], N, b.K, Sl, iws,
                                      p.in_ws, stream));
diff --git a/neuroclear_amd/csrc/w_prep.hip b/neuroclear_amd/csrc/w_prep.hip
--- /dev/null
+++ b/neuroclear_amd/csrc/w_prep.hip
@@ -0,0 +1,108 @@
+#include "common.hpp"
+#include "w_prep.hpp"
+
+namespace nc {
+namespace {
+
+struct WPrepDevSeg {
+  const float* w;
+  unsigned short* wp;
+  unsigned* ext_cell;
+  long total, so, si;
+  long nw;
+  int Cin, NS, flip, split_c;
+  int b_cell;
+  unsigned a_bits;
+};
+struct WPrepDevTable {
+  WPrepDevSeg seg[kWPrepMaxSegs];
+  unsigned blk0[kWPrepMaxSegs + 1];
+  int nseg;
+};
+struct WPrepDevBounds {
+  WPrepBound b[kWPrepMaxBounds];
+  int n;
+};
+
+__global__ void __launch_bounds__(256) k_wprep_bounds(const WPrepDevBounds t, unsigned* __restrict__ cells) {
+  __shared__ float part[4][64];
+  __shared__ float red[64];
+  const WPrepBound& b = t.b[blockIdx.y];
+  if ((int)blockIdx.x * 64 >= b.K * 8) return;
+  convT_bound_block(b.w, b.bias, b.C, b.K, b.in_bound, cells + b.cell, (int)blockIdx.x, part, red);
+}
+
+__global__ void __launch_bounds__(256) k_wprep_absmax(const WPrepDevTable t, unsigned* __restrict__ cells) {
+  __shared__ unsigned wm[4];
+  const WPrepDevSeg& g = t.seg[blockIdx.y];
+  if (!g.w) return;
+  const unsigned ca = g.a_bits, cb = g.b_cell >= 0 ? cells[g.b_cell] : ca;
+  absmax_w_block(g.w, g.nw, 27, g.Cin, g.split_c, ca, cb, cells + blockIdx.y, blockIdx.x, gridDim.x, wm);
+}
+
+__global__ void __launch_bounds__(256) k_wprep_pack(const WPrepDevTable t, const unsigned* __restrict__ cells) {
+  int k = 0;
+  while (k + 1 < t.nseg && blockIdx.x >= t.blk0[k + 1]) ++k;
+  const WPrepDevSeg& g = t.seg[k];
+  const unsigned ca = g.a_bits, cb = g.b_cell >= 0 ? cells[g.b_cell] : ca;
+  const long i = (long)(blockIdx.x - t.blk0[k]) * 256 + threadIdx.x;
+  if (i == 0 && g.ext_cell) *g.ext_cell = cb;
+  if (i >= g.total) return;
+  g.wp[i] = pack_w_s3x_elem<2>(g.w, i, g.Cin / 8, 3, g.NS, g.so, g.si, g.flip, cells[k], g.split_c, ca, cb);
+}
+
+}
+
+size_t wprep_bytes(const WPrepSeg* segs, int n) {
+  size_t b = kWPrepCellBytes;
+  for (int i = 0; i < n; ++i) b += s3x_packed_bytes(segs[i].Cin, segs[i].Kout, 3, 2);
+  return b;
+}
+
+int wprep_run(const WPrepSeg* segs, int n, const WPrepBound* bounds, int nb, void* region, S3xPrepared* out, hipStream_t s) {
+  if (n < 0 || n > kWPrepMaxSegs || nb < 0 || nb > kWPrepMaxBounds || !region) { set_error("wprep_run: bad table"); return NC_ERR_ARG; }
+  unsigned* cells = (unsigned*)region;
+  char* packs = (char*)region + kWPrepCellBytes;
+  WPrepDevTable t{};
+  WPrepDevBounds tb{};
+  t.nseg = n;
+  size_t off = 0;
+  unsigned blk = 0;
+  for (int k = 0; k < n; ++k) {
+    const WPrepSeg& h = segs[k];
+    t.blk0[k] = blk;
+    if (out) out[k] = S3xPrepared{nullptr, nullptr};
+    if (!h.w) { off += s3x_packed_bytes(h.Cin, h.Kout, 3, 2); continue; }
+    if (h.Cin % 64 || h.Kout % 64 || (!h.flip && h.b_cell >= 0 && (h.b_cell < kWPrepBoundCell0 || h.b_cell >= kWPrepBoundCell0 + nb)) ||
+        (h.flip && h.b_cell >= 0)) {
+      set_error("wprep_run: segment %d not covered", k);
+      return NC_ERR_SHAPE;
+    }
+    WPrepDevSeg& g = t.seg[k];
+    const size_t bytes = s3x_packed_bytes(h.Cin, h.Kout, 3, 2);
+    g.w = h.w; g.wp = (unsigned short*)(packs + off); g.ext_cell = h.ext_cell;
+    g.total = (long)(bytes / 2); g.nw = (long)h.Cin * h.Kout * 27;
+    g.Cin = h.Cin; g.NS = s3x_ksteps(h.Cin, 3); g.flip = h.flip;
+    g.so = h.flip ? 27 : (long)h.Cin * 27; g.si = h.flip ? (long)h.Kout * 27 : 27;
+    g.split_c = h.flip ? h.Cin : h.Cin / 2;
+    g.b_cell = h.b_cell; g.a_bits = h.a_bits;
+    blk += (unsigned)cdiv(g.total, 256);
+    if (out) { out[k].wp = packs + off; out[k].wcell = cells + k; }
+    off += bytes;
+  }
+  t.blk0[n] = blk;
+  int kmax = 0;
+  for (int j = 0; j < nb; ++j) {
+    tb.b[j] = bounds[j];
+    tb.b[j].cell = kWPrepBoundCell0 + j;
+    if (bounds[j].K > kmax) kmax = bounds[j].K;
+  }
+  tb.n = nb;
+  if (int e = h2_zero_cells(cells, kWPrepBoundCell0 + kWPrepMaxBounds, s)) return e;
+  if (nb) hipLaunchKernelGGL(k_wprep_bounds, dim3((unsigned)cdiv((long)kmax * 8, 64), (unsigned)nb), dim3(256), 0, s, tb, cells);
+  if (n) hipLaunchKernelGGL(k_wprep_absmax, dim3(256, (unsigned)n), dim3(256), 0, s, t, cells);
+  if (blk) hipLaunchKernelGGL(k_wprep_pack, dim3(blk), dim3(256), 0, s, t, (const unsigned*)cells);
+  return check_launch("wprep_run");
+}
+
+}
diff --git a/neuroclear_amd/csrc/w_prep.hpp b/neuroclear_amd/csrc/w_prep.hpp
--- /dev/null
+++ b/neuroclear_amd/csrc/w_prep.hpp
@@ -0,0 +1,86 @@
+#pragma once
+#include <hip/hip_runtime.h>
+
+#include "s3_common.hpp"
+
+namespace nc {
+
+__device__ __forceinline__ void absmax_w_block(const float* __restrict__ w, long n, int T3, int C, int split_c, unsigned cell_a, unsigned cell_b,
+                                               unsigned* __restrict__ out, long bid, long nblocks, unsigned* wm) {
+  unsigned m = 0;
+  const float gf = split_c < C ? h2_group_factor(cell_a, cell_b) : 1.f;
+  for (long i = bid * 256 + threadIdx.x; i < n; i += nblocks * 256) {
+    const int ci = (int)((i / T3) % C);
+    const unsigned b = __float_as_uint(w[i] * (ci >= split_c ? gf : 1.f)) & 0x7fffffffu;
+    if (b < 0x7f800000u && b > m) m = b;
+  }
+#pragma unroll
+  for (int o = 32; o > 0; o >>= 1) {
+    const unsigned q = (unsigned)__shfl_xor((int)m, o);
+    m = q > m ? q : m;
+  }
+  if ((threadIdx.x & 63) == 0) wm[threadIdx.x >> 6] = m;
+  __syncthreads();
+  if (threadIdx.x == 0) {
+    unsigned b = wm[0];
+    for (int k = 1; k < 4; ++k) b = wm[k] > b ? wm[k] : b;
+    if (b) atomicMax(out, b);
+  }
+}
+
+template <int NT>
+__device__ __forceinline__ unsigned short pack_w_s3x_elem(const float* __restrict__ w, long i, int NCH, int KS, int NS, long so, long si, int flip,
+                                                          unsigned amax, int split_c, unsigned cell_a, unsigned cell_b) {
+  const int T2 = KS * KS, T3 = T2 * KS, NB = NCH * KS;
+  const int j = (int)(i & 7);
+  long q = i >> 3;
+  const int lane = (int)(q & 63); q >>= 6;
+  const int f = (int)(q % (2 * NT)); q /= 2 * NT;
+  const int s = (int)(q % NS); q /= NS;
+  const int half = (int)(q & 1);
+  const int cot = (int)(q >> 1);
+  const int rb = f / NT, term = f % NT;
+  const int g = lane >> 4, m = lane & 15;
+  const int T = 4 * s + g;
+  const int bi = T / T2, tp = T % T2;
+  unsigned short t[3] = {0, 0, 0};
+  if (bi < NB) {
+    const int chunk = bi / KS, dz = bi % KS;
+#ifdef NC_S3X_B128
+    const int jj = j;
+#else
+    const int jj = (g & 1) ? ((j + 4) & 7) : j;
+#endif
+    const long co = cot * 64 + half * 32 + rb * 16 + m, ci = chunk * 8 + jj;
+    const int tap = dz * T2 + tp;
+    const float v = w[co * so + ci * si + (flip ? T3 - 1 - tap : tap)];
+    if constexpr (NT == 3) s3_split(v, t);
+    else h2_split(v * (ci >= split_c ? h2_group_factor(cell_a, cell_b) : 1.f) * h2_scale(amax), t);
+  }
+  return t[term];
+}
+
+__device__ __forceinline__ void convT_bound_block(const float* __restrict__ w, const float* __restrict__ bias, int C, int K, float in_bound,
+                                                  unsigned* __restrict__ cell, int bid, float (*part)[64], float* red) {
+  const int col = threadIdx.x & 63, sl = threadIdx.x >> 6;
+  const int kq = bid * 64 + col;
+  float sabs = 0.f;
+  if (kq < K * 8) {
+#pragma unroll 8
+    for (int ci = sl; ci < C; ci += 4) sabs += fabsf(w[(long)ci * K * 8 + kq]);
+  }
+  part[sl][col] = sabs;
+  __syncthreads();
+  if (sl == 0) {
+    const float t = (part[0][col] + part[1][col]) + (part[2][col] + part[3][col]);
+    red[col] = kq < K * 8 ? t * in_bound + (bias ? fabsf(bias[kq >> 3]) : 0.f) : 0.f;
+  }
+  __syncthreads();
+  for (int o = 32; o > 0; o >>= 1) {
+    if ((int)threadIdx.x < o) red[threadIdx.x] = red[threadIdx.x + o] > red[threadIdx.x] ? red[threadIdx.x + o] : red[threadIdx.x];
+    __syncthreads();
+  }
+  if (threadIdx.x == 0) atomicMax(cell, __float_as_uint(red[0] * 1.001f) & 0x7fffffffu);
+}
+
+}
diff --git a/neuroclear_amd/ops.py b/neuroclear_amd/ops.py
--- a/neuroclear_amd/ops.py
+++ b/neuroclear_amd/ops.py
@@ -900,11 +900,18 @@
     return _param_gen.get(t.untyped_storage().data_ptr(), 0)
 
 
+def _param_versions(packed):
+    flat = _flat_bufs.get(packed.untyped_storage().data_ptr())
+    return packed._version, (flat._version if flat is not None else None)
+
+
 _flat_grads = {}
+_flat_bufs = {}
 
 
 def register_flat_grad(flat, grad):
     _flat_grads[flat.untyped_storage().data_ptr()] = [grad, set()]
+    _flat_bufs[flat.untyped_storage().data_ptr()] = flat
 
 
 def flat_grad_step_begin(flat):
@@ -1321,13 +1328,14 @@
         ctx.save_for_backward(x, y, saved)
         ctx.packed = packed
         ctx.packed_gen = _param_generation(packed)
+        ctx.packed_version = _param_versions(packed)
         ctx.shapes = [tuple(p.shape) for p in params]
         return y
 
     @staticmethod
     def backward(ctx, dy):
         x, y, saved = ctx.saved_tensors
-        if _param_generation(ctx.packed) != ctx.packed_gen:
+        if _param_generation(ctx.packed) != ctx.packed_gen or _param_versions(ctx.packed) != ctx.packed_version:
             raise _lib.NcError('fused Unet_deconv: the parameters were updated between this forward and its backward')
         dy = dy.contiguous()
         N, _, S0, S1, S2 = x.shape
```
